# Gadersd/whisper-burn

Hardware: AMD Instinct MI355X
Metric: real-time factor (audio-sec/wall-sec) (higher is better)
Workload: dtype f32; 1 GPU; tiny.en, 30 s of 16 kHz audio per GPU per step, reference windowing (3 windows <= 14.9 s, 3 s overlap), HIP mel + encoder + KV-cached decode, greedy (beam_size 1), max_depth 100; windows=3, beam_size=1, max_depth=100, encoder_gemm_after_the_run=f16x3, parallelism=windows sharded over 1 GPU(s), 1 token all-gather

## Files before the change

profiles/ps_timeline.py:

```python
#!/usr/bin/env python3
import sys

import numpy as np

raw = np.fromfile(sys.argv[1], dtype=np.uint8)
n_steps, n_roles, grid, ns = [int(x) for x in raw[:16].view(np.int32)]
kinds = raw[16:16 + 4 * n_roles].view(np.int32)
n_st = 8 * n_steps * n_roles * ns
st = raw[16 + 4 * n_roles:16 + 4 * n_roles + n_st].view(np.uint64).reshape(n_steps, n_roles, ns).astype(np.float64)
tail = raw[16 + 4 * n_roles + n_st:]
block = None
if len(tail) >= 4 * (grid + 2) and int(tail[:4].view(np.int32)[0]) == 0x66664f52:
    role_off = tail[4:4 * (grid + 2)].view(np.int32)
    block = np.searchsorted(role_off, np.arange(n_roles), side="right") - 1
st[st == 0] = np.nan
names = {0: "attn", 1: "cross", 2: "mlp", 3: "logits", 4: "merge", 5: "finln"}
kind, layer, row = kinds & 0xff, (kinds >> 8) & 0xff, kinds >> 16
ran = ~np.isnan(st[:, :, 6])
last = int(np.nonzero(ran.any(1))[0].max()) + 1 if ran.any() else 0
lo = int(sys.argv[2]) if len(sys.argv) > 2 else min(8, max(last - 1, 0))
hi = int(sys.argv[3]) if len(sys.argv) > 3 else last
live_row = int(sys.argv[4]) if len(sys.argv) > 4 else 0
tick = 0.01
print(f"steps stamped {last} of {n_steps}, roles/step {n_roles}, grid {grid}; statistics over steps [{lo}, {hi}), attention roles of row {live_row}")
sel = st[lo:hi]
merge_done = sel[:, kind == 4, 7]
step_end = np.nanmax(merge_done, axis=1)
step_start = np.concatenate([[np.nan], step_end[:-1]])
hdr = f"{'role':<10}{'n':>4}{'wait':>8}{'w->p2':>8}{'p2->p3':>8}{'p3->p4':>8}{'p4->p5':>8}{'p5->done':>9}{'arrive':>8}{'run':>8}{'done@':>9}{'arrived@':>9}"
print(hdr)
spread = []
for k in (0, 1, 2, 5, 3, 4):
    for l in sorted(set(layer[kind == k])):
        cols = (kind == k) & (layer == l)
        if k in (0, 1, 5):
            cols &= row == live_row
        if not cols.any():
            continue
        s = sel[:, cols, :]
        def d(a, b):
            x = (s[:, :, b] - s[:, :, a]) * tick
            return np.nanmean(x) if np.isfinite(x).any() else float("nan")
        rel_done = np.nanmean((np.nanmax(s[:, :, 6], axis=1) - step_start) * tick)
        rel_arr = np.nanmean((np.nanmax(s[:, :, 7], axis=1) - step_start) * tick)
        nm = names[k] + (f" L{l}" if k < 3 else "")
        if k in (0, 1, 3, 4, 5):
            wp = np.nanmean((s[:, :, 1] - step_start[:, None]) * tick, axis=0)
            dn = np.nanmean((s[:, :, 6] - step_start[:, None]) * tick, axis=0)
            spread.append((nm, wp, dn, block[cols] if block is not None else None))
        print(f"{nm:<10}{int(cols.sum()):>4}{d(0,1):>8.2f}{d(1,2):>8.2f}{d(2,3):>8.2f}{d(3,4):>8.2f}{d(4,5):>8.2f}{d(5,6):>9.2f}{d(6,7):>8.2f}{d(1,6):>8.2f}{rel_done:>9.2f}{rel_arr:>9.2f}")
dd = np.diff(step_end) * tick
print(f"step time (merge arrived -> next merge arrived): mean {np.nanmean(dd):.2f} us, median {np.nanmedian(dd):.2f}, min {np.nanmin(dd):.2f}, max {np.nanmax(dd):.2f}")
a0 = (kind == 0) & (layer == 0) & (row == live_row)
if a0.any() and (kind == 3).any() and hi - lo > 1:
    lg_done = np.nanmax(st[lo:hi - 1][:, kind == 3, 6], axis=1)
    for nm, red in (("first", np.nanmin), ("last", np.nanmax)):
        edge = (red(st[lo + 1:hi][:, a0, 2], axis=1) - lg_done) * tick
        print(f"last logits done -> attn L0 p2 ({nm} block of row {live_row}): mean {np.nanmean(edge):.2f} us, median {np.nanmedian(edge):.2f}, min {np.nanmin(edge):.2f}, max {np.nanmax(edge):.2f}")
print("over the roles of a kind (each role: mean over the steps), us after the step start (merge: of its own step's start):")
print(f"{'role':<10}{'n':>4}  {'wait passed @  min / median / max':<36}{'done @  min / median / max':<34}")
for nm, wp, dn, blk in spread:
    f3 = lambda v: f"{np.nanmin(v):8.2f} /{np.nanmedian(v):8.2f} /{np.nanmax(v):8.2f}"
    print(f"{nm:<10}{len(wp):>4}  {f3(wp):<36}{f3(dn):<34}")
    if nm == "logits" and blk is not None:
        late = np.argsort(-np.nan_to_num(dn))[:12]
        def held(b):
            o = [names[kind[i]] + f" L{layer[i]}" for i in np.nonzero(block == b)[0] if kind[i] < 3]
            return "+".join(o) if o else "-"
        print(f"{'':<10}last to finish (block [its layer roles]: wait passed @ / done @)  " +
              "  ".join(f"b{blk[i]}[{held(blk[i])}]:{wp[i]:.2f}/{dn[i]:.2f}" for i in late))
        behind = np.array([held(b) != "-" for b in blk])
        for lab, m in (("behind a layer role", behind), ("on blocks without one", ~behind)):
            if m.any():
                print(f"{'':<10}{lab}: n {int(m.sum())}, done @ min / median / max {np.nanmin(dn[m]):.2f} / {np.nanmedian(dn[m]):.2f} / {np.nanmax(dn[m]):.2f}")
    if nm in ("attn L0", "merge", "finln"):
        per = "  ".join((f"b{blk[i]}:" if blk is not None else f"#{i}:") + f"{wp[i]:.2f}/{dn[i]:.2f}" for i in range(len(wp)))
        print(f"{'':<10}per role (block: wait passed @ / done @)  {per}")
```

whisper-burn_amd/csrc/decode.h:

```cpp
#pragma once
#include <hip/hip_runtime.h>
#include <hip/hip_ext.h>
#include <stdint.h>

#include <algorithm>
#include <vector>

#include "kernels.h"
#include "wb_internal.h"

namespace wb {

constexpr int MAX_BEAMS = 8;
constexpr int TOPK_MAX = 8;
constexpr int CA_STRIDE = 66;
constexpr int CA_NCH_MAX = 12;
constexpr int TS_STRIDE = 2 + 2 * TOPK_MAX;
constexpr int GV_CT = 128;
constexpr int GV_CT_LOGITS = 128;
constexpr int KS_MAX = 16;

enum { ST_N = 0, ST_STEP = 1, ST_HDR = 4 };
enum { GC_STEP = 0, GC_NDONE = 1, GC_ALLDONE = 2, GC_BAD = 3, GC_HDR = 4 };
struct StepLayout {
  int S = 0, W = 0;
  int tok = 0, parent = 0, len = 0, win = 0;
  int dead = 0;
  int win_nb = 0, win_slots = 0;
  int total = 0;
};
inline StepLayout make_step_layout(int S, int W) {
  StepLayout l;
  l.S = S; l.W = W;
  l.tok = ST_HDR; l.parent = l.tok + S; l.len = l.parent + S; l.win = l.len + S; l.dead = l.win + S;
  l.win_nb = l.dead + S; l.win_slots = l.win_nb + W; l.total = l.win_slots + W * MAX_BEAMS;
  return l;
}

enum { PRO_PLAIN = 0, PRO_GELU = 1, PRO_ATTN = 2, PRO_LN = 3 };
struct GemvArgs {
  const float* W = nullptr; int ldw = 0;
  int K = 0, N = 0, KS = 1, KSL = 0;
  int pro = PRO_PLAIN;
  const float* src = nullptr; int ld_src = 0;
  const float* pend = nullptr; const float* pbias = nullptr; int KSp = 0;
  float* x_out = nullptr;
  const float* ln_g = nullptr; const float* ln_b = nullptr; float ln_eps = 0.f; int ln_inside = 0;
  int n_head = 0, n_chunks = 0;
  float* P = nullptr;
  float* h_tmp = nullptr;
  const float* mask = nullptr; int use_mask = 0, topk = 0; float* tstats = nullptr;
  const int* st = nullptr; int S = 0;
  int ct = 0;
};

void gemv_plan(int K, int N, int* KS, int* KSL);
int cross_attn_chunk();

void launch_dec_prepare(hipStream_t st, const int* state_host_mapped, int* state_dev, const StepLayout& lay, int n,
                        int* tabs, int Lmax, const float* E, const float* pos, int d, float* x, const int* gctl);
void launch_dec_resolve_ln(hipStream_t st, const int* state, int n_max, const float* x_in, float* x_out,
                           const float* P, int KS, int S, const float* bias, int d, const LayerNormW& ln,
                           int eps_inside_sqrt, float* h);
void launch_dec_gemv(hipStream_t st, const GemvArgs& a, int n_rows_hint, bool stats);
bool dec_logits_two_launches(const GemvArgs& a, int n_rows_hint);
void launch_dec_self_attn(hipStream_t st, const int* state, const StepLayout& lay, int n_max, int n_head,
                          const float* Pqkv, int KS, const float* bqkv, int d, float* Kc, float* Vc, const int* tab,
                          int Lmax, float scale, float* att);
struct CaFuse {
  const float* x_in = nullptr;
  const float* pend = nullptr; int KSp = 0; const float* pbias = nullptr;
  float* x_out = nullptr;
  const float* ln_g = nullptr; const float* ln_b = nullptr; float ln_eps = 0.f; int ln_inside = 0;
  const float* Wq = nullptr;
  const float* Wo = nullptr;
  float* rec = nullptr;
};
bool cross_attn_can_fuse_q(int d);
void launch_dec_cross_attn(hipStream_t st, const int* state, const StepLayout& lay, int n_windows, int n_head,
                           int n_chunks, const float* Pq, int KS, const float* bq, int d, const float* ckv, int ldkv,
                           int koff, const int* win_row0, const int* win_C, float scale, float* ca, int max_nb,
                           const CaFuse* fuse = nullptr);
constexpr int CSF_MAX_D = 1280;
struct CaStreamFuse {
  const float* x_in = nullptr; float* x_out = nullptr;
  const float* pend = nullptr; int KSp = 0; const float* pbias = nullptr;
  const float* ln_g = nullptr; const float* ln_b = nullptr; float ln_eps = 0.f; int ln_inside = 0;
  const float* Wq = nullptr;
};
bool cross_stream_can_fuse(int d);
void launch_dec_cross_attn_stream_fused(hipStream_t st, const int* state, const StepLayout& lay, int n_windows, int n_head,
                                        const float* bq, int d, const float* ckv, int ldkv, int koff, const int* win_row0,
                                        const int* win_C, float scale, float* att, const CaStreamFuse& fz);
void launch_dec_cross_attn_stream(hipStream_t st, const int* state, const StepLayout& lay, int n_windows, int n_head,
                                  const float* Pq, int KS, const float* bq, int d, const float* ckv, int ldkv, int koff,
                                  const int* win_row0, const int* win_C, float scale, float* att);
struct NextPrep {
  float* x = nullptr;
  const float* E = nullptr;
  const float* pos = nullptr;
  int* tabs = nullptr;
  int d = 0;
  int* hflags = nullptr;
};
void launch_dec_topk_merge(hipStream_t st, int* state, int n_max, const float* tstats, int n_tiles, int k,
                           int32_t* out_id, float* out_lp, float* row_stats, const StepLayout& lay, int* gctl, int* gtok,
                           int Lmax, int eot, const NextPrep& nx);
void launch_dec_gelu_fold(hipStream_t st, const int* state, int n_max, const float* P, int KS, int S, int K,
                          const float* bias, float* out);
void launch_dec_attn_combine(hipStream_t st, const int* state, int n_max, const float* ca, int n_head, int n_chunks,
                             float* out);
void launch_dec_topk_rows(hipStream_t st, int* state, int n_max, const float* logits, int V, const float* mask,
                          int use_mask, int k, int32_t* out_id, float* out_lp, float* row_stats, const StepLayout& lay,
                          int* gctl, int* gtok, int Lmax, int eot);
void launch_dec_logprob_row(hipStream_t st, const float* x, int KS, int64_t plane, int V, const float* mask,
                            int use_mask, const float* stats, float* out);

constexpr int BEAM_KB = 2 * TOPK_MAX;
enum { BC_DEPTH = 0, BC_ALLDONE = 1, BC_ERR = 2, BC_NLIVE = 3, BC_HDR = 8 };
struct BeamChainLayout {
  int W = 0, max_depth = 0;
  int nb = 0, done = 0, node = 0, fin = 0, prev_slot = 0, slot_now = 0, lp = 0, nodes = 0, total_ints = 0;
};
inline BeamChainLayout make_beam_layout(int W, int max_depth) {
  BeamChainLayout b;
  b.W = W; b.max_depth = max_depth;
  b.nb = BC_HDR; b.done = b.nb + W; b.node = b.done + W; b.fin = b.node + W * BEAM_KB; b.prev_slot = b.fin + W * BEAM_KB;
  b.slot_now = b.prev_slot + W * BEAM_KB;
  b.lp = (b.slot_now + W * BEAM_KB + 1) & ~1;
  b.nodes = b.lp + 2 * W * BEAM_KB;
  b.total_ints = b.nodes + 2 * (max_depth + 1) * W * BEAM_KB;
  return b;
}
struct BeamChainArgs {
  int* ctl = nullptr; BeamChainLayout bl;
  const int32_t* topk_id = nullptr; const float* topk_lp = nullptr;
  int* state_out = nullptr; StepLayout lay;
  int k = 0, eot = 0, first = 0;
  int V = 0;
  int step_pos = 0;
  int* done_flag_host = nullptr;
  int* tabs = nullptr; int Lmax = 0; const float* E = nullptr; const float* pos = nullptr; int d = 0; float* x = nullptr;
};
void launch_dec_beam_update(hipStream_t st, const BeamChainArgs& a);

enum { SC_NDONE = 0, SC_ALLDONE = 1, SC_ERR = 2, SC_NROWS = 3, SC_BEST_OF = 4, SC_ATTEMPT = 5, SC_SEED_LO = 6, SC_SEED_HI = 7,
       SC_INVT = 8, SC_HDR = 16 };
struct SampleChainLayout {
  int S = 0, W = 0, max_depth = 0;
  int stream = 0, fin = 0, ngen = 0, win_fin = 0, sum = 0, tokens = 0, total_ints = 0;
};
inline SampleChainLayout make_sample_layout(int S, int W, int max_depth) {
  SampleChainLayout b;
  b.S = S; b.W = W; b.max_depth = max_depth;
  b.stream = SC_HDR; b.fin = b.stream + S; b.ngen = b.fin + S; b.win_fin = b.ngen + S;
  b.sum = (b.win_fin + W + 1) & ~1;
  b.tokens = b.sum + 2 * S;
  b.total_ints = b.tokens + S * max_depth;
  return b;
}
struct SampleChainArgs {
  int* ctl = nullptr; SampleChainLayout sl;
  const float* logits = nullptr; int V = 0;
  const float* mask = nullptr; int use_mask = 0;
  const float* row_stats = nullptr;
  int* state = nullptr; StepLayout lay;
  int eot = 0;
  int* tabs = nullptr; int Lmax = 0; const float* E = nullptr; const float* pos = nullptr; int d = 0; float* x = nullptr;
};
void launch_dec_sample_update(hipStream_t st, const SampleChainArgs& a, int n_rows);
struct SampleRowsArgs {
  const float* logits = nullptr; int R = 0, ld = 0, V = 0;
  const float* mask = nullptr; const uint8_t* row_masked = nullptr;
  const float* row_stats = nullptr;
  float inv_t = 1.f; uint32_t seed_lo = 0, seed_hi = 0, attempt = 0;
  const int32_t* stream = nullptr; const int32_t* position = nullptr;
  int eot = 0;
  int32_t* out_token = nullptr; float* out_logprob = nullptr; int32_t* out_err = nullptr;
};
void launch_sample_rows(hipStream_t st, const SampleRowsArgs& a);

enum { TC_NDONE = 0, TC_ALLDONE = 1, TC_ERR = 2, TC_NROWS = 3, TC_BEST_OF = 4, TC_ATTEMPT = 5, TC_SEED_LO = 6, TC_SEED_HI = 7,
       TC_INVT = 8,
       TC_TB = 9, TC_NTS = 10, TC_MAX_INIT = 11, TC_MAX_TS = 12, TC_HDR = 16 };
struct TsChainLayout {
  int S = 0, W = 0, max_depth = 0;
  int stream = 0, fin = 0, ngen = 0, last_was = 0, penult_was = 0, last_ts = 0, win_fin = 0, sum = 0, tokens = 0, total_ints = 0;
};
inline TsChainLayout make_ts_layout(int S, int W, int max_depth) {
  TsChainLayout b;
  b.S = S; b.W = W; b.max_depth = max_depth;
  b.stream = TC_HDR; b.fin = b.stream + S; b.ngen = b.fin + S; b.last_was = b.ngen + S; b.penult_was = b.last_was + S;
  b.last_ts = b.penult_was + S; b.win_fin = b.last_ts + S;
  b.sum = (b.win_fin + W + 1) & ~1;
  b.tokens = b.sum + 2 * S;
  b.total_ints = b.tokens + S * max_depth;
  return b;
}
struct TsRowState {
  int n_gen = 0;
  int last_was = 0, penult_was = 0;
  int last_ts = -1;
};
struct TsRules { int tb = 0, n_ts = 0, max_init = -1, max_ts = -1, eot = 0; };
struct TsChainArgs {
  int* ctl = nullptr; TsChainLayout tl;
  const float* logits = nullptr; int V = 0;
  const uint32_t* sup = nullptr; const uint32_t* sup_first = nullptr;
  const float* row_stats = nullptr;
  int* state = nullptr; StepLayout lay;
  int eot = 0;
  int* tabs = nullptr; int Lmax = 0; const float* E = nullptr; const float* pos = nullptr; int d = 0; float* x = nullptr;
};
void launch_dec_ts_update(hipStream_t st, const TsChainArgs& a, int n_rows);
struct TsRowsArgs {
  const float* logits = nullptr; int R = 0, ld = 0, V = 0;
  const uint32_t* sup = nullptr; const uint32_t* sup_first = nullptr;
  const float* row_max = nullptr;
  TsRules rules;
  float inv_t = 0.f; uint32_t seed_lo = 0, seed_hi = 0, attempt = 0;
  const int32_t* n_gen = nullptr; const int32_t* prev1 = nullptr; const int32_t* prev2 = nullptr; const int32_t* last_ts = nullptr;
  const int32_t* stream = nullptr; const int32_t* position = nullptr;
  int32_t* out_token = nullptr; float* out_logprob = nullptr; int32_t* out_forced = nullptr; float* out_stats = nullptr;
  int32_t* out_err = nullptr;
};
void launch_ts_rows(hipStream_t st, const TsRowsArgs& a);

enum { TB_DEPTH = 0, TB_ALLDONE = 1, TB_ERR = 2, TB_NENDED = 3, TB_NWIN = 4, TB_B = 5, TB_C = 6, TB_TB = 7, TB_NTS = 8,
       TB_MAX_INIT = 9, TB_MAX_TS = 10, TB_NLIVE = 11, TB_HDR = 16 };
struct TsBeamLayout {
  int S = 0, W = 0, max_depth = 0;
  int nb = 0, ended = 0, nfin = 0, slot = 0, node = 0, last_was = 0, penult_was = 0, last_ts = 0, fin_node = 0, row_beam = 0,
      tr_n = 0, tr_fin = 0, score = 0, fin_score = 0, tr_score = 0, nodes = 0, total_ints = 0;
};
inline TsBeamLayout make_tsbeam_layout(int S, int W, int max_depth) {
  TsBeamLayout b;
  b.S = S; b.W = W; b.max_depth = max_depth;
  const int WB = W * MAX_BEAMS, DW = max_depth * W;
  b.nb = TB_HDR; b.ended = b.nb + W; b.nfin = b.ended + W; b.slot = b.nfin + W; b.node = b.slot + WB; b.last_was = b.node + WB;
  b.penult_was = b.last_was + WB; b.last_ts = b.penult_was + WB; b.fin_node = b.last_ts + WB; b.row_beam = b.fin_node + W * BEAM_KB;
  b.tr_n = b.row_beam + S; b.tr_fin = b.tr_n + DW;
  b.score = (b.tr_fin + DW + 1) & ~1;
  b.fin_score = b.score + 2 * WB; b.tr_score = b.fin_score + 2 * W * BEAM_KB;
  b.nodes = b.tr_score + 2 * DW * MAX_BEAMS;
  b.total_ints = b.nodes + 2 * DW * MAX_BEAMS;
  return b;
}
enum { TBR_COUNT = 0, TBR_FORCED = 1, TBR_TS_LSE = 2, TBR_MN = 3, TBR_STRIDE = 4 };
struct TsBeamRowsArgs {
  int* ctl = nullptr; TsBeamLayout bl;
  const float* logits = nullptr; int V = 0;
  const uint32_t* sup = nullptr; const uint32_t* sup_first = nullptr;
  const int* state = nullptr; StepLayout lay;
  int eot = 0;
  int32_t* topk_id = nullptr; float* topk_lp = nullptr; int* row_out = nullptr;
};
struct TsBeamUpdateArgs {
  int* ctl = nullptr; TsBeamLayout bl;
  const int32_t* topk_id = nullptr; const float* topk_lp = nullptr; const int* row_out = nullptr;
  int* state = nullptr; StepLayout lay;
  int eot = 0, V = 0;
  int step_pos = 0;
  int* tabs = nullptr; int Lmax = 0; const float* E = nullptr; const float* pos = nullptr; int d = 0; float* x = nullptr;
};
void launch_dec_tsbeam_rows(hipStream_t st, const TsBeamRowsArgs& a, int n_rows);
void launch_dec_tsbeam_update(hipStream_t st, const TsBeamUpdateArgs& a);
struct TsBeamRowsHookArgs {
  const float* logits = nullptr; int R = 0, ld = 0, V = 0, k = 0;
  const uint32_t* sup = nullptr; const uint32_t* sup_first = nullptr;
  TsRules rules;
  const int32_t* n_gen = nullptr; const int32_t* prev1 = nullptr; const int32_t* prev2 = nullptr; const int32_t* last_ts = nullptr;
  int32_t* out_id = nullptr; float* out_lp = nullptr;
  int32_t* out_count = nullptr; int32_t* out_forced = nullptr; float* out_stats = nullptr; int32_t* out_err = nullptr;
};
void launch_tsbeam_rows_hook(hipStream_t st, const TsBeamRowsHookArgs& a);

struct MlpFusedArgs {
  const int* st = nullptr; int S = 0, d = 0;
  const float* x_in = nullptr; const float* pend = nullptr; int KSp = 0; const float* pbias = nullptr; float* x_out = nullptr;
  int n_head = 0, n_chunks = 0;
  const float* ln_g = nullptr; const float* ln_b = nullptr; float ln_eps = 0.f; int ln_inside = 0;
  const float* W1 = nullptr; int ld1 = 0; const float* b1 = nullptr;
  const float* W2 = nullptr;
  float* P = nullptr;
  unsigned long long* stamps = nullptr;
  int row0 = 0;
  const void* g_x_in = nullptr; const void* g_pend = nullptr; void* g_x_out = nullptr; void* g_P = nullptr;
};
struct AttnFusedArgs {
  const int* st = nullptr; StepLayout lay; int S = 0, d = 0, n_head = 0;
  const float* x_in = nullptr; const float* pend = nullptr; int KSp = 0; const float* pbias = nullptr; float* x_out = nullptr;
  const float* ln_g = nullptr; const float* ln_b = nullptr; float ln_eps = 0.f; int ln_inside = 0;
  const float* Wqkv = nullptr; int ldqkv = 0; const float* bqkv = nullptr; float scale = 0.f;
  float* Kc = nullptr; float* Vc = nullptr; const int* tabs = nullptr; int Lmax = 0;
  const float* Wo = nullptr;
  float* P = nullptr;
  unsigned long long* stamps = nullptr;
  const void* g_x_in = nullptr; const void* g_pend = nullptr; void* g_x_out = nullptr; void* g_P = nullptr;
};
struct CrossFusedArgs {
  const int* st = nullptr; StepLayout lay; int S = 0, d = 0, n_head = 0;
  const float* x_in = nullptr; const float* pend = nullptr; int KSp = 0; const float* pbias = nullptr; float* x_out = nullptr;
  const float* ln_g = nullptr; const float* ln_b = nullptr; float ln_eps = 0.f; int ln_inside = 0;
  const float* Wq = nullptr; const float* bq = nullptr; float scale = 0.f;
  const float* ckv = nullptr; int ldkv = 0, koff = 0;
  const int* win_row0 = nullptr; const int* win_C = nullptr;
  int n_pass = 1;
  const float* Wo = nullptr;
  float* P = nullptr;
  unsigned long long* stamps = nullptr;
  const void* g_x_in = nullptr; const void* g_pend = nullptr; void* g_x_out = nullptr; void* g_P = nullptr;
};
struct SkinnyArgs {
  const float* A = nullptr; int lda = 0;
  const float* B = nullptr; int ldb = 0;
  int M = 0, N = 0, K = 0, ksplit = 1;
  float* P = nullptr; int plane = 0;
  const uint16_t* Bh = nullptr; const uint16_t* Bl = nullptr;
  int* range_flag = nullptr;
  const int* st = nullptr;
};
void launch_split_weight_f16_tiles(hipStream_t st, const float* W, int K, int N, uint16_t* hi, uint16_t* lo);
int skinny_ksplit(int K, int N, int max_ks, int max_rows);
bool skinny_supported(int M, int K, int N);
int launch_dec_skinny_gemm(hipStream_t st, const SkinnyArgs& a);

struct PsLayerArgs { AttnFusedArgs attn; CrossFusedArgs cross; MlpFusedArgs mlp; };
enum { PSR_ATTN = 0, PSR_CROSS = 1, PSR_MLP = 2, PSR_LOGITS = 3, PSR_MERGE = 4, PSR_FINLN = 5 };
struct PsRole { int kind, layer, a, b; };
constexpr int PS_MAX_FORCED = 8;
struct PersistArgs {
  const PsLayerArgs* layers = nullptr;
  const PsRole* roles = nullptr; int n_roles = 0;
  const int* role_off = nullptr;
  const int* res_role = nullptr;
  int n_logits_roles = 0;
  int n_layer = 0, n_rows = 0, S = 0, d = 0, n_head = 0, nb_mlp = 0;
  int n_pass = 1;
  int* ctl = nullptr;
  int step0 = 0, n_steps = 0;
  int n_forced = 0; int forced[PS_MAX_FORCED] = {0, 0, 0, 0, 0, 0, 0, 0};
  int mask_until_len = 0;
  const void* x_fin = nullptr; const void* P2 = nullptr; const float* b2_last = nullptr;
  void* g_xn = nullptr;
  unsigned tag_base = 0;
  const float* ln_g = nullptr; const float* ln_b = nullptr; float ln_eps = 0.f; int ln_inside = 0;
  const float* Et = nullptr; int vocab_ld = 0, V = 0; const float* mask = nullptr;
  void* tstats = nullptr; int n_tiles = 0;
  int pick = 1;
  int* gctl = nullptr; int* gtok = nullptr; int Lmax = 0, eot = 0;
  const float* E = nullptr; const float* pos = nullptr; void* x0 = nullptr; int* tabs = nullptr;
  int* dead = nullptr;
  unsigned long long* stamps = nullptr;
};
enum { PS_DEAL_SLACK = 0, PS_DEAL_LEGACY = 1 };
struct PsDeal {
  std::vector<PsRole> roles;
  std::vector<int> role_off;
  std::vector<int> res_role;
  int n_lg = 0, n_res = 0;
};
PsDeal ps_deal_roles(int n_layer, int n_head, int n_rows, int nb_mlp, int n_tiles, int grid, int policy, bool res_on);
int ps_ctl_ints(int S, int n_layer);
bool dec_persist_supported(int d, int n_rows, int max_keys);
int dec_persist_resident_slots(int d, int n_rows, int max_keys);
bool dec_persist_resident_geometry(int d, int n_rows, int max_keys, int out[5]);
int dec_persist_max_grid(int device, int d, int n_rows, int max_keys);
int launch_dec_persist(hipStream_t st, const PersistArgs& a, int grid);
void launch_ps_seed(hipStream_t st, const float* x, int n, void* gx, unsigned tag, int* ctl);
void launch_ps_pick_test(hipStream_t st, const void* rec, int n_tiles, unsigned tag, int* ctl, int* out_id);

#if defined(HIPEMU) && !defined(HIPEMU_PROD_GEOMETRY)
constexpr int CROSS_FUSED_MAX_C = 384;
#else
constexpr int CROSS_FUSED_MAX_C = 768;
#endif
constexpr int CROSS_FUSED_MAX_PASSES = 2;
void launch_dec_cross_fused(hipStream_t st, const CrossFusedArgs& a, int n_rows_hint);
bool dec_fused_supported(int d);
int dec_mlp_fused_planes(int d);
void launch_dec_mlp_fused(hipStream_t st, const MlpFusedArgs& a, int n_rows_hint);
void launch_dec_attn_fused(hipStream_t st, const AttnFusedArgs& a, int n_rows_hint);
int launch_dec_attn_fused_rounds(hipStream_t st, const AttnFusedArgs& a, int n_rows_hint, int n_reg);

}
```

whisper-burn_amd/csrc/decode_chain.cpp:

```cpp
#include <climits>
#include <cstring>
#include <string>

#include "decode_step.h"
#include "handoff.h"
#include "switches.h"

using namespace wb;

namespace wb {

struct PsPin { size_t seed, err, gctl, tok, total, ctl_ints; };
static PsPin ps_pin_layout(size_t ctl_ints, size_t tok_ints) {
  PsPin p;
  p.seed = 0; p.err = (ctl_ints + 3) & ~(size_t)3; p.gctl = p.err + 4; p.tok = p.gctl + ((ctl_ints + 3) & ~(size_t)3);
  p.total = p.tok + tok_ints; p.ctl_ints = ctl_ints;
  return p;
}
static int ps_pin_ensure(wb_session* s, size_t ints) {
  if (s->ps_pin_ints >= ints) return WB_OK;
  if (s->ps_pin_busy) { WB_HIP(hipStreamSynchronize(s->st)); s->ps_pin_busy = false; }
  if (s->ps_pin) { (void)hipHostFree(s->ps_pin); s->ps_pin = nullptr; s->ps_pin_ints = 0; }
  WB_HIP(hipHostMalloc((void**)&s->ps_pin, ints * 4, hipHostMallocDefault));
  s->ps_pin_ints = ints;
  return WB_OK;
}

PsDeal ps_deal_roles(int NL, int H, int W, int NB, int n_tiles, int grid, int policy, bool res_on) {
  std::vector<PsRole> lr;
  for (int l = 0; l < NL; l++) {
    for (int r = 0; r < W; r++) for (int h = 0; h < H; h++) lr.push_back(PsRole{PSR_ATTN, l, h, r});
    for (int r = 0; r < W; r++) for (int h = 0; h < H; h++) lr.push_back(PsRole{PSR_CROSS, l, h, r});
    for (int j = 0; j < NB; j++) lr.push_back(PsRole{PSR_MLP, l, j, 0});
  }
  std::vector<std::vector<PsRole>> deal(grid);
  for (size_t i = 0; i < lr.size(); i++) deal[i % grid].push_back(lr[i]);
  std::vector<char> early(grid, 0);
  std::vector<int> cand;
  for (int b = 0; b < grid; b++) {
    for (const PsRole& r : deal[b]) early[b] |= r.layer == 0 && (r.kind == PSR_ATTN || r.kind == PSR_CROSS);
    if (!early[b]) cand.push_back(b);
  }
  if ((int)cand.size() * 4 < n_tiles) { cand.clear(); for (int b = 0; b < grid; b++) cand.push_back(b); }
  const bool slack = policy != PS_DEAL_LEGACY;
  auto by_load = [&](std::vector<int>& v) {
    std::stable_sort(v.begin(), v.end(), [&](int x, int y) {
      if (slack && early[x] != early[y]) return early[x] < early[y];
      return deal[x].size() < deal[y].size();
    });
  };
  std::vector<int> fin_block(W, 0);
  std::vector<char> is_fin(grid, 0);
  {
    std::vector<int> order(grid);
    for (int b = 0; b < grid; b++) order[b] = b;
    by_load(order);
    for (int r = 0; r < W; r++) { fin_block[r] = order[r % grid]; deal[fin_block[r]].push_back(PsRole{PSR_FINLN, 0, 0, r}); is_fin[fin_block[r]] = 1; }
  }
  if ((int)cand.size() > 2 * W) cand.erase(std::remove_if(cand.begin(), cand.end(), [&](int b) { return is_fin[b] != 0; }), cand.end());
  std::stable_sort(cand.begin(), cand.end(), [&](int x, int y) { return deal[x].size() < deal[y].size(); });
  const int tpb = (n_tiles + (int)cand.size() - 1) / (int)cand.size();
  const int n_lg = (n_tiles + tpb - 1) / tpb;
  std::vector<char> has_lg(grid, 0);
  for (int q = 0; q < n_lg; q++) {
    deal[cand[q]].push_back(PsRole{PSR_LOGITS, q, q * tpb, std::min(tpb, n_tiles - q * tpb)});
    has_lg[cand[q]] = 1;
  }
  {
    std::vector<int> order;
    if (slack) {
      for (int b = 0; b < grid; b++) if (!early[b] && !has_lg[b]) order.push_back(b);
      if (order.empty()) for (int b = 0; b < grid; b++) if (!early[b]) order.push_back(b);
    }
    if (order.empty()) for (int b = 0; b < grid; b++) order.push_back(b);
    by_load(order);
    for (int r = 0; r < W; r++) {
      const int b = slack && !early[fin_block[r]] ? fin_block[r] : order[r % (int)order.size()];
      deal[b].push_back(PsRole{PSR_MERGE, 0, 0, r});
    }
  }
  PsDeal out;
  out.n_lg = n_lg;
  out.role_off.assign(grid + 1, 0);
  for (int b = 0; b < grid; b++) {
    out.role_off[b] = (int)out.roles.size();
    out.roles.insert(out.roles.end(), deal[b].begin(), deal[b].end());
  }
  out.role_off[grid] = (int)out.roles.size();
  out.res_role.assign(grid, -1);
  if (res_on)
    for (int b = 0; b < grid; b++) {
      int n_lr = 0, at = -1;
      for (int i = out.role_off[b]; i < out.role_off[b + 1]; i++)
        if (out.roles[i].kind <= PSR_MLP) { n_lr++; at = i; }
      if (n_lr == 1 && out.roles[at].kind != PSR_MLP) { out.res_role[b] = at; out.n_res++; }
    }
  return out;
}

static void ps_deal_log(const PsDeal& deal, int grid) {
  std::string where[2];
  int n_lg_blocks = 0;
  for (int b = 0; b < grid; b++) {
    bool lg = false;
    for (int i = deal.role_off[b]; i < deal.role_off[b + 1]; i++) {
      const int k = deal.roles[i].kind;
      lg |= k == PSR_LOGITS;
      if (k == PSR_MERGE || k == PSR_FINLN) {
        std::string& w = where[k == PSR_FINLN];
        w += (w.empty() ? "" : ",") + std::to_string(b);
      }
    }
    n_lg_blocks += lg;
  }
  fprintf(stderr, "persist deal: merge on blocks %s; finln on %s; logits blocks %d\n", where[0].c_str(), where[1].c_str(), n_lg_blocks);
}

static int ps_setup_ensure(wb_session* s, bool res_on, bool* built) {
  wb_model* m = s->m;
  const wb_dims& D = m->dims;
  const int d = D.n_text_state, H = D.n_text_head, NL = D.n_text_layer, V = D.n_vocab, S = s->S, W = s->W;
  const StepLayout& L = s->lay;
  hipStream_t st = s->st;
  const int NB = dec_mlp_fused_planes(d);
  const int n_tiles = (V + 127) / 128;
  const size_t pool = (size_t)s->Lmax * S;
  const int ldkv = 2 * d;
  const int n_pass = s->maxC > CROSS_FUSED_MAX_C ? 2 : 1;
  const int n_layer_roles = NL * (2 * W * H + NB);
  const int grid = std::max(1, std::min(s->ps_grid, n_layer_roles + n_tiles + 2 * W));
  const char* deal_sw = sw::persist_deal();
  const int policy = deal_sw && !strcmp(deal_sw, "legacy") ? PS_DEAL_LEGACY : PS_DEAL_SLACK;
  auto up = [](const void* p) { return (uint64_t)reinterpret_cast<uintptr_t>(p); };
  const std::vector<uint64_t> key = {
      s->model_uid, (uint64_t)W, (uint64_t)S, (uint64_t)s->Lmax, (uint64_t)grid, (uint64_t)n_tiles, (uint64_t)n_pass,
      (uint64_t)s->enc_rows, (uint64_t)res_on, (uint64_t)m->ln_eps_inside_sqrt, up(s->state.p), up(s->x.p), up(s->P2.p),
      up(s->Pa.p), up(s->Pc.p), up(s->kc.p), up(s->vc.p), up(s->tabs.p), up(s->ckv.p), up(s->win_meta.p), up(s->ps_gx.p),
      up(s->ps_gpa.p), up(s->ps_gpc.p), up(s->ps_gp2.p), up(s->ps_gxn.p), (uint64_t)policy};
  const char* sw_setup = sw::persist_setup();
  const bool cache_on = !(sw_setup && sw_setup[0] == '0');
  *built = !(cache_on && !s->ps_setup_key.empty() && s->ps_setup_key == key);
  if (sw_setup && strstr(sw_setup, "log")) fprintf(stderr, "persist setup: %s\n", *built ? "built" : "reused");
  if (!*built) return WB_OK;
  s->ps_setup_key.clear();
  char* gxb[2] = {static_cast<char*>(s->ps_gx.p), static_cast<char*>(s->ps_gx.p) + (size_t)S * d * 8};
  std::vector<PsLayerArgs> la(NL);
  float* xb[2] = {s->x.as<float>(), s->x.as<float>() + (size_t)S * d};
  int xi = 0;
  for (int l = 0; l < NL; l++) {
    const DecBlockW& b = m->dec[l];
    AttnFusedArgs& fa = la[l].attn;
    fa.st = s->state.as<int>(); fa.lay = L; fa.S = S; fa.d = d; fa.n_head = H;
    fa.x_in = xb[xi]; fa.pend = l == 0 ? nullptr : s->P2.as<float>(); fa.KSp = l == 0 ? 0 : NB;
    fa.pbias = l == 0 ? nullptr : m->dec[l - 1].mlp2.b; fa.x_out = xb[xi ^ 1];
    fa.ln_g = b.ln1.g; fa.ln_b = b.ln1.b; fa.ln_eps = b.ln1.eps; fa.ln_inside = m->ln_eps_inside_sqrt;
    fa.Wqkv = b.qkv.w; fa.ldqkv = b.qkv.n; fa.bqkv = b.qkv.b; fa.scale = m->qk_scale;
    fa.Kc = s->kc.as<float>() + (size_t)l * pool * d; fa.Vc = s->vc.as<float>() + (size_t)l * pool * d;
    fa.tabs = s->tabs.as<int>(); fa.Lmax = s->Lmax; fa.Wo = b.out.w; fa.P = s->Pa.as<float>();
    fa.g_x_in = gxb[xi]; fa.g_pend = l == 0 ? nullptr : s->ps_gp2.p; fa.g_x_out = gxb[xi ^ 1]; fa.g_P = s->ps_gpa.p;
    xi ^= 1;
    CrossFusedArgs& ca = la[l].cross;
    ca.st = s->state.as<int>(); ca.lay = L; ca.S = S; ca.d = d; ca.n_head = H;
    ca.x_in = xb[xi]; ca.pend = s->Pa.as<float>(); ca.KSp = H; ca.pbias = b.out.b; ca.x_out = xb[xi ^ 1];
    ca.ln_g = b.ln2.g; ca.ln_b = b.ln2.b; ca.ln_eps = b.ln2.eps; ca.ln_inside = m->ln_eps_inside_sqrt;
    ca.Wq = b.cq.w; ca.bq = b.cq.b; ca.scale = m->qk_scale;
    ca.ckv = s->ckv.as<float>() + (size_t)l * s->enc_rows * 2 * d; ca.ldkv = ldkv; ca.koff = 0;
    ca.win_row0 = s->win_meta.as<int>(); ca.win_C = s->win_meta.as<int>() + W;
    ca.Wo = b.cout.w; ca.P = s->Pc.as<float>();
    ca.n_pass = n_pass;
    ca.g_x_in = gxb[xi]; ca.g_pend = s->ps_gpa.p; ca.g_x_out = gxb[xi ^ 1]; ca.g_P = s->ps_gpc.p;
    xi ^= 1;
    MlpFusedArgs& ma = la[l].mlp;
    ma.st = s->state.as<int>(); ma.S = S; ma.d = d;
    ma.x_in = xb[xi]; ma.pend = s->Pc.as<float>(); ma.KSp = H; ma.pbias = b.cout.b; ma.x_out = xb[xi ^ 1];
    ma.ln_g = b.ln3.g; ma.ln_b = b.ln3.b; ma.ln_eps = b.ln3.eps; ma.ln_inside = m->ln_eps_inside_sqrt;
    ma.W1 = b.mlp1.w; ma.ld1 = b.mlp1.n; ma.b1 = b.mlp1.b; ma.W2 = b.mlp2.w; ma.P = s->P2.as<float>();
    ma.g_x_in = gxb[xi]; ma.g_pend = s->ps_gpc.p; ma.g_x_out = gxb[xi ^ 1]; ma.g_P = s->ps_gp2.p;
    xi ^= 1;
  }
  PsDeal deal = ps_deal_roles(NL, H, W, NB, n_tiles, grid, policy, res_on);
  if (deal_sw && !strcmp(deal_sw, "log")) ps_deal_log(deal, grid);
  std::vector<PsRole>& roles = deal.roles;
  const std::vector<int>&role_off = deal.role_off, &res_role = deal.res_role;
  const int n_lg = deal.n_lg, n_res = deal.n_res;
  WB_TRY(s->ps_layers.ensure(la.size() * sizeof(PsLayerArgs)));
  WB_TRY(s->ps_roles.ensure(roles.size() * sizeof(PsRole) + (role_off.size() + res_role.size()) * 4));
  WB_HIP(hipMemcpyAsync(s->ps_layers.p, la.data(), la.size() * sizeof(PsLayerArgs), hipMemcpyHostToDevice, st));
  WB_HIP(hipMemcpyAsync(s->ps_roles.p, roles.data(), roles.size() * sizeof(PsRole), hipMemcpyHostToDevice, st));
  WB_HIP(hipMemcpyAsync(static_cast<char*>(s->ps_roles.p) + roles.size() * sizeof(PsRole), role_off.data(), role_off.size() * 4,
                        hipMemcpyHostToDevice, st));
  WB_HIP(hipMemcpyAsync(static_cast<char*>(s->ps_roles.p) + roles.size() * sizeof(PsRole) + role_off.size() * 4, res_role.data(),
                        res_role.size() * 4, hipMemcpyHostToDevice, st));
  WB_HIP(hipStreamSynchronize(st));
  s->ps_pin_busy = false;
  s->ps_roles_host.swap(roles);
  s->ps_role_off_host = role_off;
  s->ps_setup_grid = grid; s->ps_setup_n_lg = n_lg; s->ps_setup_n_res = n_res;
  s->ps_setup_key = key;
  return WB_OK;
}

static int run_persistent_chain(wb_session* s, int eot, int max_depth, int mask_until_len, const int32_t* forced, int n_forced,
                                const PsPin& pin, int* steps_done, bool* fell_back) {
  *fell_back = false;
  WB_REQUIRE(n_forced >= 0 && n_forced <= PS_MAX_FORCED, WB_ERR_ARG, "persistent decode: %d prompt steps", n_forced);
  const char* inject = sw::persist_inject_fail();
  wb_model* m = s->m;
  const wb_dims& D = m->dims;
  const int d = D.n_text_state, H = D.n_text_head, NL = D.n_text_layer, V = D.n_vocab, S = s->S, W = s->W;
  const StepLayout& L = s->lay;
  hipStream_t st = s->st;
  const int NB = dec_mlp_fused_planes(d);
  const int n_tiles = (V + 127) / 128;
  WB_REQUIRE(NB <= 32 && H <= 8, WB_ERR_SHAPE, "persistent decode: more planes than its folds hold");
  WB_TRY(s->ps_gx.ensure_zeroed(((size_t)2 * S + 8) * d * 8, st));
  WB_TRY(s->ps_gpa.ensure_zeroed(((size_t)H * S + 8) * d * 8, st));
  WB_TRY(s->ps_gpc.ensure_zeroed(((size_t)H * S + 8) * d * 8, st));
  WB_TRY(s->ps_gp2.ensure_zeroed(((size_t)NB * S + 8) * d * 8, st));
  WB_TRY(s->ps_gxn.ensure_zeroed(((size_t)S + 8) * d * 8, st));
  WB_TRY(s->ps_tstats.ensure_zeroed((size_t)2 * S * n_tiles * 16, st));
  if (((s->ps_launches + 1) & 0xffffu) == 0) {
    for (DevMem* b : {&s->ps_gx, &s->ps_gpa, &s->ps_gpc, &s->ps_gp2, &s->ps_gxn, &s->ps_tstats}) WB_HIP(hipMemsetAsync(b->p, 0, b->bytes, st));
    s->ps_launches++;
  }
  const unsigned tag_base = ((++s->ps_launches) & 0xffffu) << 16;
  char* gxb[2] = {static_cast<char*>(s->ps_gx.p), static_cast<char*>(s->ps_gx.p) + (size_t)S * d * 8};
  const char* res_sw = sw::persist_resident();
  const bool res_on = !(res_sw && res_sw[0] == '0') && dec_persist_resident_slots(d, W, s->maxC) > 0;
  bool built = false;
  WB_TRY(ps_setup_ensure(s, res_on, &built));
  const std::vector<PsRole>& roles = s->ps_roles_host;
  const int grid = s->ps_setup_grid, n_res = s->ps_setup_n_res;
  if (res_sw && !strcmp(res_sw, "log")) fprintf(stderr, "persist resident blocks: %d of %d\n", n_res, grid);
  const int n_ctl = ps_ctl_ints(S, NL);
  WB_TRY(s->ps_ctl.ensure((size_t)n_ctl * 4));
  WB_TRY(s->ps_dead.ensure((size_t)S * 4));
  WB_HIP(hipMemsetAsync(s->ps_ctl.p, 0, (size_t)n_ctl * 4, st));
  WB_HIP(hipMemsetAsync(s->ps_dead.p, 0, (size_t)S * 4, st));
  PersistArgs a;
  a.layers = s->ps_layers.as<PsLayerArgs>(); a.roles = s->ps_roles.as<PsRole>(); a.n_roles = (int)roles.size();
  a.role_off = reinterpret_cast<const int*>(static_cast<char*>(s->ps_roles.p) + roles.size() * sizeof(PsRole));
  if (n_res > 0) a.res_role = a.role_off + (grid + 1);
  a.n_logits_roles = s->ps_setup_n_lg;
  a.n_layer = NL; a.n_rows = W; a.S = S; a.d = d; a.n_head = H; a.nb_mlp = NB;
  a.n_pass = s->maxC > CROSS_FUSED_MAX_C ? 2 : 1;
  a.ctl = s->ps_ctl.as<int>(); a.step0 = s->step; a.n_steps = n_forced + max_depth; a.mask_until_len = mask_until_len;
  a.n_forced = n_forced;
  for (int i = 0; i < n_forced; i++) a.forced[i] = forced[i];
  a.g_xn = s->ps_gxn.p;
  a.x_fin = gxb[(3 * NL) & 1]; a.P2 = s->ps_gp2.p; a.b2_last = m->dec[NL - 1].mlp2.b; a.tag_base = tag_base;
  a.ln_g = m->ln_dec.g; a.ln_b = m->ln_dec.b; a.ln_eps = m->ln_dec.eps; a.ln_inside = m->ln_eps_inside_sqrt;
  a.Et = m->tok_emb_t; a.vocab_ld = m->vocab_ld; a.V = V; a.mask = s->mask.as<float>();
  a.tstats = s->ps_tstats.p; a.n_tiles = n_tiles;
  const char* pick_sw = sw::persist_pick();
  a.pick = pick_sw && !strcmp(pick_sw, "merge") ? 0 : 1;
  a.gctl = s->gctl.as<int>(); a.gtok = s->gtok.as<int>(); a.Lmax = s->Lmax; a.eot = eot;
  a.E = m->tok_emb; a.pos = m->dec_pos; a.x0 = gxb[0]; a.tabs = s->tabs.as<int>(); a.dead = s->ps_dead.as<int>();
  const char* stamps_path = sw::ps_stamps();
  const size_t n_stamps = stamps_path ? (size_t)(n_forced + max_depth) * roles.size() * 8 : 0;
  if (n_stamps) {
    WB_TRY(s->ps_stamps.ensure(n_stamps * 8));
    WB_HIP(hipMemsetAsync(s->ps_stamps.p, 0, n_stamps * 8, st));
    a.stamps = s->ps_stamps.as<unsigned long long>();
  }
  WB_REQUIRE(3 * NL * (n_forced + max_depth + 1) + 4 < 0x10000, WB_ERR_SHAPE,
             "persistent decode: %d layers x %d steps do not fit the 16-bit granule tags", NL, max_depth);
  launch_dec_prepare(st, reinterpret_cast<const int*>(s->host_block_dev), s->state.as<int>(), L, W, s->tabs.as<int>(),
                     s->Lmax, m->tok_emb, m->dec_pos, d, s->x.as<float>(), s->gctl.as<int>());
  launch_ps_seed(st, s->x.as<float>(), W * d, gxb[0], tag_base + 1u, s->ps_ctl.as<int>());
  hipEvent_t e0 = nullptr, e1 = nullptr;
  prof_tag(KC_PERSIST, 0.0);
  const bool timed = prof_take_events(&e0, &e1);
  if (timed) WB_HIP(hipEventRecord(e0, st));
  const bool refused = (inject && !strcmp(inject, "launch")) || launch_dec_persist(st, a, grid) != 0;
  if (timed) WB_HIP(hipEventRecord(e1, st));
  if (refused) {
    (void)hipGetLastError();
    s->ps_grid = 0;
    *fell_back = true;
    *steps_done = 0;
    return WB_OK;
  }
  int* hp = s->ps_pin;
  s->ps_pin_busy = true;
  WB_HIP(hipMemcpyAsync(hp + pin.err, s->ps_ctl.as<int>() + HX_ERR, 4, hipMemcpyDeviceToHost, st));
  WB_HIP(hipMemcpyAsync(hp + pin.gctl, s->gctl.p, pin.ctl_ints * 4, hipMemcpyDeviceToHost, st));
  WB_HIP(hipMemcpyAsync(hp + pin.tok, s->gtok.p, (pin.total - pin.tok) * 4, hipMemcpyDeviceToHost, st));
  WB_HIP(hipStreamSynchronize(st));
  s->ps_pin_busy = false;
  const int err = hp[pin.err], gstep = hp[pin.gctl + GC_STEP];
  if (err != 0 && gstep == s->step) {
    s->ps_grid = 0;
    *fell_back = true;
    *steps_done = 0;
    return WB_OK;
  }
  WB_REQUIRE(err == 0, WB_ERR_HIP, "persistent decode: a wait gave up (counter %d) at step %d", err - 1, gstep);
  if (n_stamps) {
    std::vector<unsigned long long> hs(n_stamps);
    WB_HIP(hipMemcpy(hs.data(), s->ps_stamps.p, n_stamps * 8, hipMemcpyDeviceToHost));
    if (FILE* f = fopen(stamps_path, "wb")) {
      const int hdr[4] = {n_forced + max_depth, (int)roles.size(), grid, 8};
      fwrite(hdr, 4, 4, f);
      std::vector<int> kinds(roles.size());
      for (size_t i = 0; i < roles.size(); i++)
        kinds[i] = roles[i].kind | ((roles[i].kind <= PSR_MLP ? roles[i].layer : 0) << 8) |
                   ((roles[i].kind == PSR_LOGITS ? 0 : roles[i].b) << 16);
      fwrite(kinds.data(), 4, kinds.size(), f);
      fwrite(hs.data(), 8, hs.size(), f);
      const int marker = 0x66664f52;
      fwrite(&marker, 4, 1, f);
      fwrite(s->ps_role_off_host.data(), 4, s->ps_role_off_host.size(), f);
      fclose(f);
    }
  }
  *steps_done = std::max(0, std::min(n_forced + max_depth, gstep - s->step));
  return WB_OK;
}

int session_greedy_chain(wb_session* s, const int32_t* prompt, int eot, int max_depth, int mask_until_len, int prompt_len,
                         int32_t* out_tokens, int32_t row_stride, int32_t* out_lens) {
  wb_model* m = s->m;
  const int S = s->S, W = s->W;
  WB_REQUIRE(S == W, WB_ERR_STATE, "chained greedy decode needs max_beams == 1");
  WB_REQUIRE(prompt && prompt_len >= 1, WB_ERR_ARG, "chained greedy decode: empty prompt");
  WB_REQUIRE(s->step == 0 || (s->prev_n == W && s->step == prompt_len - 1), WB_ERR_STATE,
             "chained greedy decode: the session is neither fresh nor prefilled");
  const int n_forced_max = prompt_len - 1;
  auto host_prefill = [&]() -> int {
    std::vector<int32_t> tok(W), par(W), win(W);
    for (int t = s->step; t < prompt_len - 1; t++) {
      for (int w = 0; w < W; w++) { tok[w] = prompt[t]; par[w] = t == 0 ? -1 : w; win[w] = w; }
      WB_TRY(wb_session_step(s, tok.data(), par.data(), win.data(), W, 0, 0, nullptr, nullptr));
    }
    return WB_OK;
  };
  WB_REQUIRE(s->has_mask || mask_until_len < prompt_len || max_depth == 0, WB_ERR_STATE,
             "wb_session_decode: special mask not set");
  const int asked_depth = max_depth;
  max_depth = std::min(max_depth, s->Lmax - (prompt_len - 1));
  WB_HIP(hipSetDevice(m->device));
  hipStream_t st = s->st;
  const size_t ctl_ints = GC_HDR + 3 * (size_t)S;
  WB_TRY(s->gctl.ensure(ctl_ints * 4));
  WB_TRY(s->gtok.ensure(((size_t)S * s->Lmax + 1) * 4));
  std::vector<int> ctl(ctl_ints, 0);
  const PsPin pin = ps_pin_layout(ctl_ints, (size_t)S * s->Lmax + 1);
  WB_TRY(ps_pin_ensure(s, pin.total));
  auto seed_ctl = [&](bool wait) -> int {
    if (s->ps_pin_busy) { WB_HIP(hipStreamSynchronize(st)); s->ps_pin_busy = false; }
    int* seed = s->ps_pin + pin.seed;
    std::fill(seed, seed + ctl_ints, 0);
    seed[GC_STEP] = s->step;
    for (int i = 0; i < W; i++) seed[GC_HDR + i] = prompt[s->step];
    s->ps_pin_busy = true;
    WB_HIP(hipMemcpyAsync(s->gctl.p, seed, ctl_ints * 4, hipMemcpyHostToDevice, st));
    if (wait) { WB_HIP(hipStreamSynchronize(st)); s->ps_pin_busy = false; }
    return WB_OK;
  };
  const StepPlan plan = plan_step(s, W, false);
  const int n_launch = plan.n_launch;
  const bool fuse_ln = plan.fuse_ln;
  const int chunk = 16;
  int depth = 0;
  bool persist = plan.persist && max_depth > 0;
  if (persist) {
    if (s->ps_grid < 0) s->ps_grid = dec_persist_max_grid(m->device, m->dims.n_text_state, W, s->maxC);
    persist = s->ps_grid > 0;
  }
  int n_forced = 0;
  if (s->step == 0 && s->prefill_mode == 1 && sw::prefill_pass() && prompt_len > 1) {
    std::vector<int> win(W);
    for (int w = 0; w < W; w++) win[w] = w;
    WB_TRY(session_prefill(s, prompt, prompt_len - 1, win.data(), W));
  }
  if (persist && sw::persist_prefill() && s->step == 0 && n_forced_max <= PS_MAX_FORCED && s->has_mask) n_forced = n_forced_max;
  if (n_forced == 0) WB_TRY(host_prefill());
  WB_TRY(seed_ctl(!persist));
  ScopedTimer tm(st, 3);
  if (persist) {
    bool fell_back = false;
    WB_TRY(run_persistent_chain(s, eot, max_depth, mask_until_len, prompt + s->step + 1, n_forced, pin, &depth, &fell_back));
    if (fell_back) {
      persist = false;
      depth = 0;
      WB_TRY(host_prefill());
      WB_TRY(seed_ctl(true));
      n_forced = 0;
    } else {
      if (profile().on) profile().ms[4] += depth;
      depth -= n_forced;
      s->step += n_forced;
      s->prev_n = W;
      s->prev_win.resize(W);
      for (int w = 0; w < W; w++) s->prev_win[w] = w;
    }
  }
  if (!persist) {
  if (fuse_ln)
    launch_dec_prepare(st, reinterpret_cast<const int*>(s->host_block_dev), s->state.as<int>(), s->lay, n_launch,
                       s->tabs.as<int>(), s->Lmax, m->tok_emb, m->dec_pos, m->dims.n_text_state, s->x.as<float>(),
                       s->gctl.as<int>());
  const bool speculate = fuse_ln && sw::speculate();
  if (speculate && !s->st2) {
    WB_HIP(hipStreamCreateWithFlags(&s->st2, hipStreamNonBlocking));
    WB_HIP(hipEventCreateWithFlags(&s->ev_seg, hipEventDisableTiming));
  }
  auto enqueue_segment = [&](int* enq) -> int {
    int n = 0;
    while (depth + n < max_depth && n < chunk) {
      const int d0 = depth + n;
      const int use_mask = (prompt_len + d0) <= mask_until_len ? 1 : 0;
      const int run = (!use_mask && max_depth - d0 >= chunk) ? chunk : 1;
      StepCall call;
      call.k = 1; call.use_mask = use_mask; call.chained = true; call.eot = eot; call.reps = run;
      WB_TRY(launch_step(s, plan, call));
      if (profile().on) profile().ms[4] += run;
      n += run;
    }
    *enq = n;
    return WB_OK;
  };
  auto read_flags = [&](bool behind_event) -> int {
    if (behind_event) {
      WB_HIP(hipStreamWaitEvent(s->st2, s->ev_seg, 0));
      WB_HIP(hipMemcpyAsync(ctl.data(), s->gctl.p, ctl_ints * 4, hipMemcpyDeviceToHost, s->st2));
      WB_HIP(hipStreamSynchronize(s->st2));
    } else {
      WB_HIP(hipMemcpyAsync(ctl.data(), s->gctl.p, ctl_ints * 4, hipMemcpyDeviceToHost, st));
      WB_HIP(hipStreamSynchronize(st));
    }
    return WB_OK;
  };
  auto all_done = [&]() {
    bool d = true;
    for (int i = 0; i < W; i++) d = d && ctl[GC_HDR + S + i] != 0;
    return d;
  };
  const bool poll = fuse_ln && sw::poll() && !profile().on;
  volatile int* hfl = reinterpret_cast<volatile int*>(s->host_block + s->chain_flags_off);
  if (poll) for (int i = 0; i < 2 * S; i++) hfl[i] = 0;
  auto wait_flags = [&](int want_step, bool* done) -> int {
    for (long spins = 0;; spins++) {
      bool ready = true;
      for (int i = 0; i < W && ready; i++) ready = hfl[2 * i] >= want_step;
      if (ready) break;
      bool fin = true;
      for (int i = 0; i < W && fin; i++) fin = hfl[2 * i + 1] != 0;
      if (fin) break;
      if ((spins & 0xfff) == 0xfff) {
        const hipError_t q = hipStreamQuery(st);
        if (q == hipSuccess) {
          bool r2 = true;
          for (int i = 0; i < W && r2; i++) r2 = hfl[2 * i] >= want_step;
          if (r2) break;
          bool all = true;
          for (int i = 0; i < W; i++) all = all && hfl[2 * i + 1] != 0;
          if (all) break;
          set_error("chained decode: the device stopped at step %d of %d", (int)hfl[0], want_step);
          return WB_ERR_HIP;
        }
        if (q != hipErrorNotReady) { set_error("chained decode: %s", hipGetErrorString(q)); return WB_ERR_HIP; }
      }
    }
    __atomic_thread_fence(__ATOMIC_ACQUIRE);
    bool all = true;
    for (int i = 0; i < W; i++) all = all && hfl[2 * i + 1] != 0;
    *done = all;
    return WB_OK;
  };
  if (!speculate) {
    while (depth < max_depth) {
      int n = 0;
      WB_TRY(enqueue_segment(&n));
      depth += n;
      if (poll) {
        bool done = false;
        WB_TRY(wait_flags(s->step + depth, &done));
        if (done) break;
      } else {
        WB_TRY(read_flags(false));
        if (all_done()) break;
      }
    }
  } else {
    int n_cur = 0;
    WB_TRY(enqueue_segment(&n_cur));
    depth += n_cur;
    while (true) {
      WB_HIP(hipEventRecord(s->ev_seg, st));
      int n_next = 0;
      if (depth < max_depth) { WB_TRY(enqueue_segment(&n_next)); depth += n_next; }
      WB_TRY(read_flags(true));
      if (all_done() || n_next == 0) break;
    }
    WB_HIP(hipStreamSynchronize(st));
  }
  }
  tm.stop();
  std::vector<int> toks_chain;
  const int* toks = s->ps_pin + pin.tok;
  if (persist) {
    std::copy(s->ps_pin + pin.gctl, s->ps_pin + pin.gctl + ctl_ints, ctl.begin());
  } else {
    toks_chain.resize((size_t)S * s->Lmax + 1);
    WB_HIP(hipMemcpyAsync(ctl.data(), s->gctl.p, ctl_ints * 4, hipMemcpyDeviceToHost, st));
    WB_HIP(hipMemcpyAsync(toks_chain.data(), s->gtok.p, toks_chain.size() * 4, hipMemcpyDeviceToHost, st));
    WB_HIP(hipStreamSynchronize(st));
    s->ps_pin_busy = false;
    toks = toks_chain.data();
  }
  tm.collect();
  WB_TRY(dec_split_check(s));
  WB_REQUIRE(ctl[GC_BAD] == 0, WB_ERR_STATE, "a decode step produced a row without a finite log-prob (NaN logits: non-finite "
             "weights or activations); its window was ended on <|endoftext|> on the device and the rows of this call are invalid");
  for (int w = 0; w < W; w++) {
    int len = ctl[GC_HDR + 2 * S + w];
    if (len < prompt_len) len = prompt_len;
    len = std::min(len, prompt_len + max_depth);
    WB_REQUIRE(len <= row_stride, WB_ERR_ARG, "row_stride too small");
    for (int p = prompt_len; p < len; p++) out_tokens[(size_t)w * row_stride + p] = toks[(size_t)w * s->Lmax + p];
    out_lens[w] = len;
  }
  if (profile().on && !persist && s->prof_cls_cross >= 0 && s->prof_cls_self >= 0) {
    const int dm = m->dims.n_text_state, NL = m->dims.n_text_layer;
    double dead_ckv = 0, dead_self = 0;
    for (int w = 0; w < W; w++) {
      const int live = std::max(0, std::min(out_lens[w] - prompt_len, depth));
      for (int t = live; t < depth; t++) { dead_ckv += 8.0 * s->C[w] * dm; dead_self += 8.0 * (s->step + t + 1) * dm; }
    }
    prof_adjust_bytes(s->prof_cls_cross, -(double)NL * dead_ckv);
    prof_adjust_bytes(s->prof_cls_self, -(double)NL * dead_self);
  }
  if (profile().on && persist) {
    const double dm = m->dims.n_text_state, NL = m->dims.n_text_layer;
    double bytes = (double)(depth + n_forced) * 4.0 * NL * 14.0 * dm * dm + (double)depth * 4.0 * (double)m->dims.n_vocab * dm;
    for (int w = 0; w < W; w++)
      for (int t = 0; t < n_forced; t++) bytes += NL * (8.0 * s->C[w] * dm + 8.0 * (t + 1) * dm);
    for (int w = 0; w < W; w++) {
      const int live = std::max(0, std::min(out_lens[w] - prompt_len, depth));
      for (int t = 0; t < live; t++) bytes += NL * (8.0 * s->C[w] * dm + 8.0 * (s->step + t + 1) * dm);
    }
    prof_adjust_bytes(KC_PERSIST, bytes);
  }
  s->prof_step_off = 0;
  s->step += depth;
  s->prev_len.assign(W, s->step);
  s->last_had_logits = 0;
  if (max_depth < asked_depth)
    for (int w = 0; w < W; w++)
      WB_REQUIRE(ctl[GC_HDR + S + w] != 0, WB_ERR_SHAPE, "Token sequence length %d must not exceed %d.", s->Lmax + 1,
                 s->Lmax);
  return WB_OK;
}
}
```

whisper-burn_amd/csrc/decode_fused_bodies.h:

```cpp
#pragma once
#include <hip/hip_runtime.h>

#include "decode.h"
#include "handoff.h"
#include "wave_ops.h"

namespace wb {
namespace fused {

struct PsStep {
  const unsigned* ctr = nullptr; unsigned target = 0; int ctr_index = 0;
  const int* ctl = nullptr;
  int step = 0;
  int n_rows = 0;
  const int* dead = nullptr;
  int* lds_flag = nullptr;
  unsigned long long* stamp = nullptr;
  int n_ctr = 1;
  unsigned tag_in = 0, tag_out = 0;
  bool known_dead = false;
  mutable bool saw_dead = false;
  const void* pk_rec = nullptr; int pk_n_tiles = 0; unsigned pk_tag = 0;
  const unsigned* pk_go = nullptr; unsigned pk_go_target = 0;
  const float* pk_E = nullptr; const float* pk_pos = nullptr; int pk_eot = 0;
  bool cross_early = false;
};
constexpr int PS_STAMPS = 8;
__device__ __forceinline__ void ps_stamp(const PsStep& ps, int k) {
#ifdef WB_EXP_FINE
  if (k == 4 || k == 5) return;
#endif
  if (ps.stamp && threadIdx.x == 0) ps.stamp[k] = wall_clock64();
}
__device__ __forceinline__ void ps_stamp_fine(const PsStep& ps, int k) {
#ifdef WB_EXP_FINE
  if (ps.stamp && threadIdx.x == 0) ps.stamp[k] = wall_clock64();
#endif
}
__device__ __forceinline__ bool ps_wait(const PsStep& ps) {
  const bool ok = ps.n_ctr > 1 ? hx_wait_same(ps.ctr, ps.target, ps.n_ctr, ps.ctl, ps.step, ps.ctr_index, ps.lds_flag)
                               : hx_wait(ps.ctr, ps.target, ps.ctl, ps.step, ps.ctr_index, ps.lds_flag);
  ps_stamp(ps, 1);
  return ok;
}
__device__ __forceinline__ bool ps_sweep_retry(unsigned& sweeps, const PsStep& ps) {
  if ((sweeps & 31u) == 31u &&
      (__hip_atomic_load(ps.ctl + HX_STOP, __ATOMIC_RELAXED, __HIP_MEMORY_SCOPE_AGENT) <= ps.step ||
       __hip_atomic_load(ps.ctl + HX_ERR, __ATOMIC_RELAXED, __HIP_MEMORY_SCOPE_AGENT) != 0)) return true;
  if (++sweeps > HX_SWEEP_LIMIT) {
    __hip_atomic_store(const_cast<int*>(ps.ctl) + HX_ERR, 5000 + ps.ctr_index, __ATOMIC_RELAXED, __HIP_MEMORY_SCOPE_AGENT);
    return true;
  }
  __builtin_amdgcn_s_sleep(1);
  return false;
}
__device__ __forceinline__ bool ps_sweeps_ok(const PsStep& ps) { return *ps.lds_flag != 0; }
template <int UNITS>
__device__ __forceinline__ void ps_nap() {
#if !defined(WB_PS_DRY) || defined(WB_PS_DRY_NAPS)
#ifndef WB_PS_NAP_ADJ
#define WB_PS_NAP_ADJ 0
#endif
#pragma unroll
  for (int i = 0; i < UNITS + (WB_PS_NAP_ADJ); i++) __builtin_amdgcn_s_sleep(64);
#endif
}

constexpr int PS_PICK_NONE = 0x7fffffff;
#ifdef WB_PS_PICK_NOINLINE
__device__ __attribute__((noinline)) int ps_pick_token(
#else
__device__ __forceinline__ int ps_pick_token(
#endif
const void* rec, const int n_tiles, const unsigned tag, const PsStep& ps,
                                             float* xch, const int tid) {
  const Buf16 rb(rec);
  float bv = -INFINITY; int bi = PS_PICK_NONE;
  unsigned sweeps = 0;
  for (int t = tid; t < n_tiles;) {
    const Rec q = ld_rec(rb, (uint32_t)t);
    if (q.t0 == tag && q.t1 == tag) {
      if (better(q.v, q.id, bv, bi)) { bv = q.v; bi = q.id; }
      t += 512;
    } else if (ps_sweep_retry(sweeps, ps)) {
      *ps.lds_flag = 0;
      break;
    }
  }
  wave_argmax(bv, bi);
  int* xid = reinterpret_cast<int*>(xch) + 8;
  if ((tid & 63) == 0) { xch[tid >> 6] = bv; xid[tid >> 6] = bi; }
  __syncthreads();
  float gv = xch[0]; int gi = xid[0];
#pragma unroll
  for (int j = 1; j < 8; j++)
    if (better(xch[j], xid[j], gv, gi)) { gv = xch[j]; gi = xid[j]; }
  return gi;
}
#ifndef WB_PS_PICK_NAP
#define WB_PS_PICK_NAP 6
#endif
#ifndef WB_PS_CROSS0_NAP
#define WB_PS_CROSS0_NAP 1
#endif

#ifdef WB_STAMPS
#define WB_STAMP_DECL unsigned long long stamp_buf[16];
#define WB_STAMP(i) do { if (threadIdx.x == 0 && blockIdx.x == 0 && blockIdx.y == 0) sm.stamp_buf[i] = wall_clock64(); } while (0)
#define WB_STAMP_FLUSH(a, n) do { if (threadIdx.x == 0 && blockIdx.x == 0 && blockIdx.y == 0 && (a).stamps) for (int _i = 0; _i < (n); _i++) (a).stamps[_i] = sm.stamp_buf[_i]; } while (0)
#else
#define WB_STAMP_DECL
#define WB_STAMP(i) do {} while (0)
#define WB_STAMP_FLUSH(a, n) do {} while (0)
#endif

constexpr int FD_MAX = 512;
constexpr int FA_MAXPOS = 448;


constexpr int ROLE_NT = 512;
template <int MR, int DPL, bool REC>
struct MlpLds {
  static constexpr int d = 64 * DPL, HS = 64, G = d / 4 <= 32 ? 8 : 4;
  alignas(16) float hs[MR][d];
  alignas(16) float red[8][MR][HS];
  alignas(16) float hid[MR][HS];
  alignas(16) float obuf[(G - 1) * MR * d];
  float mlb[REC ? MR : 1][48][2];
  float coef[REC ? MR : 1][48];
  WB_STAMP_DECL
};
template <int DPL>
struct AttnLds {
  static constexpr int d = 64 * DPL, G = d / 4 <= 32 ? 8 : 4;
  static constexpr int RED = (8 * 192 > (G - 1) * d) ? 8 * 192 : (G - 1) * d;
  alignas(16) float hs[d];
  alignas(16) float red[RED];
  alignas(16) float qkv[192];
  int tbs[FA_MAXPOS];
  float sc[FA_MAXPOS];
  alignas(16) float part[32][64];
  alignas(16) float att[64];
  WB_STAMP_DECL
};
template <int DPL, int NP>
struct CrossLds {
  static constexpr int d = 64 * DPL, G = d / 4 <= 32 ? 8 : 4, CMAX = NP * CROSS_FUSED_MAX_C;
  alignas(16) float hs[d];
  alignas(16) float red[8][64];
  alignas(16) float qv[64];
  float sc[CMAX];
  float pbuf[CMAX];
  alignas(16) float part[32][64];
  alignas(16) float att[64];
  alignas(16) float wmax[8];
  alignas(16) float obuf[(G - 1) * d];
};

template <int DPL, int NP, int RS>
struct ResGeom {
  static constexpr int d = 64 * DPL, G = d / 4 <= 32 ? 8 : 4, RPG = 64 / G;
  static constexpr int KW = d / 8, RK = DPL >= 6 ? 8 : 16, NIT = KW / RK;
  static constexpr int CAP = RS * ROLE_NT;
  static constexpr int QL = 8 * 48;
  static constexpr int WL = G * (d / 4) < ROLE_NT ? G * (d / 4) : ROLE_NT;
  static constexpr int NRND_MAX = DPL == 6 ? 2 : 1;
  static constexpr int NRND_FIT = CAP / (RK * QL) < NIT - 2 ? CAP / (RK * QL) : NIT - 2;
  static constexpr int NRND = NRND_FIT <= 0 ? 0 : (NRND_FIT < NRND_MAX ? NRND_FIT : NRND_MAX);
  static constexpr int WO_A = NRND * RK * QL;
  static constexpr int NWO_A = (CAP - WO_A) / WL < RPG ? (CAP - WO_A) / WL : RPG;
  static constexpr int SL = 4, NTILE = CROSS_FUSED_MAX_C / 128;
  static constexpr int NVT = NP > 1 ? 0 : (RS / SL < NTILE ? RS / SL : NTILE);
  static constexpr int WO_X = NVT * SL * ROLE_NT;
  static constexpr int NWO_X = NP > 1 ? 0 : ((CAP - WO_X) / WL < RPG ? (CAP - WO_X) / WL : RPG);
  static_assert(RS >= 0 && WO_A + NWO_A * WL <= CAP && WO_X + NWO_X * WL <= CAP, "resident region");
  static __device__ __forceinline__ int q_holder(int wave, int lane) { return wave * 48 + (lane < 47 ? lane : 47); }
  static __device__ __forceinline__ int wo_holder(int tid) { return tid < WL - 1 ? tid : WL - 1; }
};
__device__ __forceinline__ float4 res_ld(const float4* res, int base, int NH, int slot, int k) { return res[base + slot * NH + k]; }
__device__ __forceinline__ void res_st(float4* res, int base, int NH, int slot, int k, const float4& v) { res[base + slot * NH + k] = v; }

__device__ __forceinline__ float gelu_erf_f(float x) {
  return 0.5f * x * (1.0f + erff(x * 0.70710678118654752440f));
}

template <int DPL>
__device__ __forceinline__ void fold_ln_row(const float* __restrict__ x_in, const float* __restrict__ pend, int KSp,
                                            int64_t plane, const float* __restrict__ pbias, float* __restrict__ x_out,
                                            const float* __restrict__ g, const float* __restrict__ b, float eps,
                                            int eps_inside, int d, int row, int lane, float* __restrict__ out) {
  int co[DPL];
#pragma unroll
  for (int i = 0; i < DPL; i++) co[i] = lane + (64 * i < d ? 64 * i : 0);
  float gv[DPL], bv[DPL], v[DPL];
  const float* xr = x_in + (int64_t)row * d;
#pragma unroll
  for (int i = 0; i < DPL; i++) { gv[i] = g[co[i]]; bv[i] = b[co[i]]; v[i] = xr[co[i]]; }
  if (KSp > 0) {
    float acc[DPL];
#pragma unroll
    for (int i = 0; i < DPL; i++) acc[i] = pbias[co[i]];
    const float* pp = pend + (int64_t)row * d;
    constexpr int CH = DPL <= 6 ? 8 : 4;
    for (int sp = 0; sp < KSp; sp += CH) {
      float t[CH][DPL];
#pragma unroll
      for (int j = 0; j < CH; j++) {
        const float* pj = pp + (int64_t)min(sp + j, KSp - 1) * plane;
#pragma unroll
        for (int i = 0; i < DPL; i++) t[j][i] = pj[co[i]];
      }
#pragma unroll
      for (int j = 0; j < CH; j++) {
        const bool live = sp + j < KSp;
#pragma unroll
        for (int i = 0; i < DPL; i++) acc[i] += live ? t[j][i] : 0.f;
      }
    }
#pragma unroll
    for (int i = 0; i < DPL; i++) v[i] = v[i] + acc[i];
  }
  float s = 0.f;
#pragma unroll
  for (int i = 0; i < DPL; i++) {
    if (64 * i < d) { s += v[i]; if (x_out) x_out[(int64_t)row * d + co[i]] = v[i]; }
  }
  const float mean = wave_sum(s) / (float)d;
  float q = 0.f;
#pragma unroll
  for (int i = 0; i < DPL; i++) {
    if (64 * i < d) { const float t = v[i] - mean; q += t * t; }
  }
  const float var = wave_sum(q) / (float)d;
  const float denom = eps_inside ? sqrtf(var + eps) : (sqrtf(var) + eps);
#pragma unroll
  for (int i = 0; i < DPL; i++) {
    const int c = lane + 64 * i;
    if (c < d) out[c] = (v[i] - mean) / denom * gv[i] + bv[i];
  }
}

template <int NT, int MR, int EPT, int PCH>
__device__ __forceinline__ void fold_rows(const float* __restrict__ x_in, const float* __restrict__ pend, int KSp,
                                          int64_t plane, const float* __restrict__ pbias, int d, int tid,
                                          float (&v)[EPT]) {
  int off[EPT], col[EPT];
#pragma unroll
  for (int i = 0; i < EPT; i++) {
    int e = tid + NT * i;
    if (e >= MR * d) e = tid;
    off[i] = e; col[i] = e % d;
  }
#pragma unroll
  for (int i = 0; i < EPT; i++) v[i] = x_in[off[i]];
  if (KSp > 0) {
    float acc[EPT];
#pragma unroll
    for (int i = 0; i < EPT; i++) acc[i] = pbias[col[i]];
    for (int sp = 0; sp < KSp; sp += PCH) {
      float t[PCH][EPT];
#pragma unroll
      for (int j = 0; j < PCH; j++) {
        const float* pj = pend + (int64_t)min(sp + j, KSp - 1) * plane;
#pragma unroll
        for (int i = 0; i < EPT; i++) t[j][i] = pj[off[i]];
      }
#pragma unroll
      for (int j = 0; j < PCH; j++) {
        const bool live = sp + j < KSp;
#pragma unroll
        for (int i = 0; i < EPT; i++) acc[i] += live ? t[j][i] : 0.f;
      }
    }
#pragma unroll
    for (int i = 0; i < EPT; i++) v[i] = v[i] + acc[i];
  }
}

template <int DPL>
__device__ __forceinline__ void ln_row_lds(float* __restrict__ row, int d, int lane, const float (&gv)[DPL],
                                           const float (&bv)[DPL], float eps, int eps_inside) {
  float v[DPL];
  float s = 0.f;
#pragma unroll
  for (int i = 0; i < DPL; i++) { v[i] = row[lane + 64 * i]; s += v[i]; }
  const float mean = wave_sum(s) / (float)d;
  float q = 0.f;
#pragma unroll
  for (int i = 0; i < DPL; i++) { const float t = v[i] - mean; q += t * t; }
  const float var = wave_sum(q) / (float)d;
  const float denom = eps_inside ? sqrtf(var + eps) : (sqrtf(var) + eps);
#pragma unroll
  for (int i = 0; i < DPL; i++) row[lane + 64 * i] = (v[i] - mean) / denom * gv[i] + bv[i];
}

template <int DPL>
__device__ __forceinline__ void ln_stats_lds(const float* __restrict__ row, int d, int lane, float eps, int eps_inside,
                                             float& mean, float& denom) {
  float v[DPL];
  float s = 0.f;
#pragma unroll
  for (int i = 0; i < DPL; i++) { v[i] = row[lane + 64 * i]; s += v[i]; }
  mean = wave_sum(s) / (float)d;
  float q = 0.f;
#pragma unroll
  for (int i = 0; i < DPL; i++) { const float t = v[i] - mean; q += t * t; }
  const float var = wave_sum(q) / (float)d;
  denom = eps_inside ? sqrtf(var + eps) : (sqrtf(var) + eps);
}
__device__ __forceinline__ float lane_get(float v, int src) { return __shfl(v, src, 64); }

template <int MR, int DPL, bool REC, bool PS>
__device__ __forceinline__ bool dec_mlp_body(const MlpFusedArgs& a, const int jblk, const PsStep& ps, MlpLds<MR, DPL, REC>& sm) {
  constexpr int HS = 64, NT = 512;
  constexpr int d = 64 * DPL;
  constexpr int CF = d / 4;
  constexpr int G = CF <= 32 ? 8 : 4;
  constexpr int RPG = HS / G;
  constexpr int EPT = (MR * d + NT - 1) / NT;
  constexpr int PCH = EPT <= 3 ? 8 : EPT <= 6 ? 6 : 3;
  static_assert(G == MlpLds<MR, DPL, REC>::G, "LDS struct geometry");
  auto& hs = sm.hs; auto& red = sm.red; auto& hid = sm.hid; auto& obuf = sm.obuf; auto& mlb = sm.mlb; auto& coef = sm.coef;
  WB_STAMP(0);
  const int tid = role_tid<PS>(), lane = tid & 63, wave = tid >> 6;
  const int j0 = jblk * HS;
  const int rg = tid >> 4, c4 = (tid & 15) * 4;
  float xv_fold[EPT];
  constexpr int NW1 = d / 32;
  float4 w1[NW1];
  const int cf = tid % CF, jg = tid / CF;
  const bool p2 = jg < G;
  const int jb = (p2 ? jg : 0) * RPG;
  float4 w2[RPG];
  constexpr int NOWN = 4 * NW1;
  const int own_col = 4 * wave + (lane & 3) + 32 * ((lane < NOWN ? lane : 0) >> 2);
  float g_own = 0.f, b_own = 0.f;
  float b1v;
  int deadm = 0;
  {
    int off[EPT], col[EPT];
#pragma unroll
    for (int i = 0; i < EPT; i++) {
      int e = tid + NT * i;
      if (e >= MR * d) e = tid;
      off[i] = e; col[i] = e % d;
    }
    float acc0[EPT];
    constexpr bool rec = REC;
    const int64_t plane = rec ? (int64_t)a.S * (d + 2) : (int64_t)a.S * d;
    int poff[EPT];
#pragma unroll
    for (int i = 0; i < EPT; i++) poff[i] = rec ? (off[i] / d) * (d + 2) + 2 + col[i] : off[i];
    constexpr int PCHR = EPT <= 3 ? 18 : EPT <= 4 ? 16 : EPT <= 6 ? 12 : 8;
    constexpr int PC = REC ? PCHR : PCH;
    float t[PC][EPT];
    const int npl = a.KSp;
    const int ch = rec ? PCHR : PCH;
    auto load_weights = [&]() {
      g_own = gld(a.ln_g + own_col); b_own = gld(a.ln_b + own_col);
      b1v = gld(a.b1 + j0 + (tid & 63));
      {
        const float* wp = a.W1 + (int64_t)rg * a.ld1 + j0 + c4;
#pragma unroll
        for (int i = 0; i < NW1; i++) w1[i] = ld_w4(wp + (int64_t)(32 * i) * a.ld1);
      }
      {
        const float* wp = a.W2 + (int64_t)(j0 + jb) * d + cf * 4;
#pragma unroll
        for (int i = 0; i < RPG; i++) w2[i] = ld_w4(wp + (int64_t)i * d);
      }
    };
    if constexpr (PS) {
#if !defined(WB_PS_DRY)
      load_weights();
#endif
      if (!ps_wait(ps)) return false;
#pragma unroll
      for (int r = 0; r < MR; r++)
        if (r >= ps.n_rows || ld_i<true>(ps.dead + min(r, ps.n_rows - 1)) != 0) deadm |= 1 << r;
      const Buf16 xgb(a.g_x_in), pgb(a.g_pend);
      const int iplane = a.S * d;
      ps_nap<3>();
      bool rdead[EPT];
#pragma unroll
      for (int i = 0; i < EPT; i++) { rdead[i] = ((deadm >> (off[i] / d)) & 1) != 0; acc0[i] = gld(a.pbias + col[i]); xv_fold[i] = 0.f; }
      constexpr int GP = EPT <= 3 ? 8 : 4;
      unsigned sweeps = 0;
      bool bad = false;
      for (int sp = 0; sp < npl && !bad; sp += GP) {
        Gran gx[EPT], g[GP][EPT];
#pragma unroll
        for (int i = 0; i < EPT; i++) {
          gx[i] = Gran{0u, 0.f};
#pragma unroll
          for (int j = 0; j < GP; j++) g[j][i] = Gran{0u, 0.f};
        }
        for (;;) {
          if (sp == 0) {
#pragma unroll
            for (int i = 0; i < EPT; i++)
              if (!rdead[i] && gx[i].tag != ps.tag_in) gx[i] = ld_gran(xgb, (uint32_t)off[i], 0u);
          }
#pragma unroll
          for (int j = 0; j < GP; j++)
#pragma unroll
            for (int i = 0; i < EPT; i++)
              if (!rdead[i] && sp + j < npl && g[j][i].tag != ps.tag_in)
                g[j][i] = ld_gran(pgb, (uint32_t)off[i], (uint32_t)((sp + j) * iplane));
          bool ok = true;
#pragma unroll
          for (int i = 0; i < EPT; i++) {
            if (sp == 0) ok &= rdead[i] || gx[i].tag == ps.tag_in;
#pragma unroll
            for (int j = 0; j < GP; j++) ok &= rdead[i] || sp + j >= npl || g[j][i].tag == ps.tag_in;
          }
          if (ok) {
#pragma unroll
            for (int i = 0; i < EPT; i++) {
              if (sp == 0) xv_fold[i] = gx[i].v;
#pragma unroll
              for (int j = 0; j < GP; j++) acc0[i] += (sp + j < npl) ? g[j][i].v : 0.f;
            }
            break;
          }
          if (ps_sweep_retry(sweeps, ps)) { *ps.lds_flag = 0; bad = true; break; }
        }
      }
#pragma unroll
      for (int i = 0; i < EPT; i++) {
        xv_fold[i] = rdead[i] ? 0.f : xv_fold[i] + acc0[i];
        const int e = tid + NT * i;
        if (e < MR * d) (&hs[0][0])[e] = xv_fold[i];
      }
    } else {
#pragma unroll
    for (int i = 0; i < EPT; i++) { xv_fold[i] = a.x_in[off[i]]; acc0[i] = npl > 0 ? gld(a.pbias + col[i]) : 0.f; }
    float mlv0 = -1.0e30f, mlv1 = 0.f;
    if (rec && tid < MR * npl) {
      const float* rp = a.pend + (int64_t)(tid % npl) * plane + (int64_t)(tid / npl) * (d + 2);
      mlv0 = rp[0]; mlv1 = rp[1];
    }
    if (npl > 0) {
#pragma unroll
      for (int j = 0; j < PC; j++)
        if (j < ch) {
#pragma unroll
          for (int i = 0; i < EPT; i++) t[j][i] = a.pend[(int64_t)min(j, npl - 1) * plane + poff[i]];
        }
    }
    load_weights();
    if constexpr (REC) {
      if (tid < MR * npl) { mlb[tid / npl][tid % npl][0] = mlv0; mlb[tid / npl][tid % npl][1] = mlv1; }
      __syncthreads();
      if (tid < MR * a.n_head) {
        const int r = tid / a.n_head, hh = tid % a.n_head;
        float M = -1.0e30f;
        for (int c = 0; c < a.n_chunks; c++) M = fmaxf(M, mlb[r][hh * a.n_chunks + c][0]);
        float den = 0.f;
        for (int c = 0; c < a.n_chunks; c++) den += expf(mlb[r][hh * a.n_chunks + c][0] - M) * mlb[r][hh * a.n_chunks + c][1];
        for (int c = 0; c < a.n_chunks; c++)
          coef[r][hh * a.n_chunks + c] = den > 0.f ? expf(mlb[r][hh * a.n_chunks + c][0] - M) / den : 0.f;
      }
      __syncthreads();
    }
    if (npl > 0) {
      int rowi[EPT];
#pragma unroll
      for (int i = 0; i < EPT; i++) rowi[i] = off[i] / d;
      for (int sp = 0; sp < npl; sp += ch) {
        if (sp > 0) {
#pragma unroll
          for (int j = 0; j < PC; j++)
            if (j < ch) {
#pragma unroll
              for (int i = 0; i < EPT; i++) t[j][i] = a.pend[(int64_t)min(sp + j, npl - 1) * plane + poff[i]];
            }
        }
#pragma unroll
        for (int j = 0; j < PC; j++)
          if (j < ch) {
#pragma unroll
            for (int i = 0; i < EPT; i++) {
              const bool live = sp + j < npl;
              float wgt = 1.f;
              if constexpr (REC) wgt = coef[rowi[i]][min(sp + j, npl - 1)];
              acc0[i] += live ? wgt * t[j][i] : 0.f;
            }
          }
      }
#pragma unroll
      for (int i = 0; i < EPT; i++) xv_fold[i] += acc0[i];
    }
#pragma unroll
    for (int i = 0; i < EPT; i++) {
      const int e = tid + NT * i;
      if (e < MR * d) (&hs[0][0])[e] = xv_fold[i];
    }
    }
  }
  int n_rows;
  if constexpr (PS) n_rows = ps.n_rows; else n_rows = min(MR, a.st[ST_N] - a.row0);
  if (n_rows <= 0) return true;
  WB_STAMP(1);
  __syncthreads();
  if constexpr (PS) { if (!ps_sweeps_ok(ps)) return false; }
#if defined(WB_PS_DRY)
  if constexpr (PS) {
    if (jg == 0) {
      const Buf16 pgo(a.g_P);
#pragma unroll
      for (int r = 0; r < MR; r++)
        if (r < n_rows && !((deadm >> r) & 1)) st_gran4(pgo, (uint32_t)((jblk * a.S + r) * d + cf * 4), ps.tag_out, make_float4(0.f, 0.f, 0.f, 0.f));
    }
    if (jblk == 0) {
      const Buf16 xgo(a.g_x_out);
#pragma unroll
      for (int i = 0; i < EPT; i++) {
        const int e = tid + NT * i;
        if (e < n_rows * d && !((deadm >> (e / d)) & 1)) st_gran(xgo, (uint32_t)e, ps.tag_out, xv_fold[i]);
      }
    }
    return true;
  }
#endif
  float xn_own[MR];
#pragma unroll
  for (int r = 0; r < MR; r++) {
    xn_own[r] = 0.f;
    bool skip = r >= n_rows;
    if constexpr (PS) skip = skip || ((deadm >> r) & 1);
    if (skip) continue;
    float mean, denom;
    ln_stats_lds<DPL>(hs[r], d, lane, a.ln_eps, a.ln_inside, mean, denom);
    xn_own[r] = (hs[r][own_col] - mean) / denom * g_own + b_own;
  }
  WB_STAMP(2);
  float acc[MR][4];
#pragma unroll
  for (int r = 0; r < MR; r++) { acc[r][0] = acc[r][1] = acc[r][2] = acc[r][3] = 0.f; }
  {
    const int q4 = lane >> 4;
#pragma unroll
    for (int r = 0; r < MR; r++) {
      bool skip = r >= n_rows;
      if constexpr (PS) skip = skip || ((deadm >> r) & 1);
      if (skip) continue;
#pragma unroll
      for (int i = 0; i < NW1; i++) {
        const float xv = lane_get(xn_own[r], 4 * i + q4);
        acc[r][0] += xv * w1[i].x; acc[r][1] += xv * w1[i].y; acc[r][2] += xv * w1[i].z; acc[r][3] += xv * w1[i].w;
      }
    }
  }
#pragma unroll
  for (int r = 0; r < MR; r++)
#pragma unroll
    for (int c = 0; c < 4; c++) { acc[r][c] = xor16_sum(acc[r][c]); acc[r][c] = xor32_sum(acc[r][c]); }
  if (lane < 16) {
#pragma unroll
    for (int r = 0; r < MR; r++)
      *reinterpret_cast<float4*>(&red[wave][r][c4]) = make_float4(acc[r][0], acc[r][1], acc[r][2], acc[r][3]);
  }
  __syncthreads();
  if (tid < MR * HS) {
    const int r = tid >> 6, c = tid & 63;
    float v = 0.f;
#pragma unroll
    for (int w8 = 0; w8 < 8; w8++) v += red[w8][r][c];
    hid[r][c] = gelu_erf_f(v + b1v);
  }
  __syncthreads();
  WB_STAMP(3);
  float o[MR][4];
#pragma unroll
  for (int r = 0; r < MR; r++) { o[r][0] = o[r][1] = o[r][2] = o[r][3] = 0.f; }
  if constexpr (PS) {
#pragma unroll
    for (int r = 0; r < MR; r++) {
      if ((deadm >> r) & 1) continue;
#pragma unroll
      for (int i = 0; i < RPG; i++) {
        const float hv = hid[r][jb + i];
        o[r][0] += hv * w2[i].x; o[r][1] += hv * w2[i].y; o[r][2] += hv * w2[i].z; o[r][3] += hv * w2[i].w;
      }
    }
  } else {
#pragma unroll
  for (int i = 0; i < RPG; i++) {
#pragma unroll
    for (int r = 0; r < MR; r++) {
      const float hv = hid[r][jb + i];
      o[r][0] += hv * w2[i].x; o[r][1] += hv * w2[i].y; o[r][2] += hv * w2[i].z; o[r][3] += hv * w2[i].w;
    }
  }
  }
  if (p2 && jg > 0) {
#pragma unroll
    for (int r = 0; r < MR; r++)
      *reinterpret_cast<float4*>(&obuf[((jg - 1) * MR + r) * d + cf * 4]) = make_float4(o[r][0], o[r][1], o[r][2], o[r][3]);
  }
  __syncthreads();
  if (jg == 0) {
#pragma unroll
    for (int g2 = 1; g2 < G; g2++) {
#pragma unroll
      for (int r = 0; r < MR; r++) {
        const float4 t = *reinterpret_cast<const float4*>(&obuf[((g2 - 1) * MR + r) * d + cf * 4]);
        o[r][0] += t.x; o[r][1] += t.y; o[r][2] += t.z; o[r][3] += t.w;
      }
    }
    if constexpr (PS) {
      const Buf16 pgo(a.g_P);
#pragma unroll
      for (int r = 0; r < MR; r++)
        if (r < n_rows && !((deadm >> r) & 1))
          st_gran4(pgo, (uint32_t)((jblk * a.S + r) * d + cf * 4), ps.tag_out, make_float4(o[r][0], o[r][1], o[r][2], o[r][3]));
    } else {
#pragma unroll
      for (int r = 0; r < MR; r++)
        if (r < n_rows)
          *reinterpret_cast<float4*>(&a.P[((int64_t)jblk * a.S + r) * d + cf * 4]) = make_float4(o[r][0], o[r][1], o[r][2], o[r][3]);
    }
  }
  if (jblk == 0) {
    if constexpr (PS) {
      const Buf16 xgo(a.g_x_out);
#pragma unroll
      for (int i = 0; i < EPT; i++) {
        const int e = tid + NT * i;
        if (e < n_rows * d && !((deadm >> (e / d)) & 1)) st_gran(xgo, (uint32_t)e, ps.tag_out, xv_fold[i]);
      }
    } else {
#pragma unroll
      for (int i = 0; i < EPT; i++) {
        const int e = tid + NT * i;
        if (e < n_rows * d) a.x_out[e] = xv_fold[i];
      }
    }
  }
  WB_STAMP(4);
  WB_STAMP_FLUSH(a, 5);
  return true;
}

#ifndef WB_ATTN_NREG_PS6
#define WB_ATTN_NREG_PS6 4
#endif
template <int DPL, bool PS, int RS>
constexpr int attn_nreg() { return (PS && DPL == 6 && RS > 0) ? (WB_ATTN_NREG_PS6) : 2; }
template <int DPL, bool PS, int RS = 0, int NREG = attn_nreg<DPL, PS, RS>()>
__device__ __forceinline__ bool dec_attn_body(const AttnFusedArgs& a, const int h, const int r, const PsStep& ps, AttnLds<DPL>& sm,
                                              const float4* res = nullptr) {
  constexpr int NT = 512;
  constexpr int d = 64 * DPL;
  constexpr int KW = d / 8;
  constexpr int RK = DPL >= 6 ? 8 : 16;
  constexpr int NIT = KW / RK;
  constexpr int CF = d / 4;
  constexpr int G = CF <= 32 ? 8 : 4;
  constexpr int RPG = 64 / G;
  constexpr int PT = 128, PSL = PT * 16 / NT;
  using RG = ResGeom<DPL, 1, PS ? RS : 0>;
  static_assert(G == AttnLds<DPL>::G && RG::RK == RK && RG::NIT == NIT && RG::RPG == RPG && NT == ROLE_NT, "LDS struct / resident geometry");
  auto& hs = sm.hs; auto& red = sm.red; auto& qkv = sm.qkv; auto& tbs = sm.tbs; auto& sc = sm.sc; auto& part = sm.part; auto& att = sm.att;
  WB_STAMP(0);
  const int tid = role_tid<PS>(), lane = tid & 63, wave = tid >> 6;
  if (h >= a.n_head) return true;
  int n_rows, len, step_par, dead;
  if constexpr (PS) { n_rows = ps.n_rows; len = ps.step + 1; step_par = 0; dead = 0; }
  else {
    n_rows = a.st[ST_N]; len = a.st[a.lay.len + r]; step_par = a.st[ST_STEP] & 1;
    dead = a.st[a.lay.dead + r];
  }
  const int seg = lane >> 4, c4 = (lane & 15) * 4;
  const bool seg_ok = seg < 3;
  const float* wq = a.Wqkv + (int64_t)(wave * KW) * a.ldqkv + (seg_ok ? seg : 0) * d + h * 64 + c4;
  static_assert(NREG == 2 || (NREG == 4 && NIT == 6 && (RG::NRND == 0 || RG::NRND == 2)), "register rounds: 2, or 4 of the 6 at d = 384");
  float4 wr[NREG][RK];
  auto load_round =[&](float4 (&w)[RK], int it) {
#pragma unroll
    for (int j = 0; j < RK; j++) w[j] = ld_w4(wq + (int64_t)(RK * it + j) * a.ldqkv);
  };
  float xfold;
  const int own_col = wave * KW + (lane < KW ? lane : 0);
  float g_own = 0.f, b_own = 0.f;
  float qbias = 0.f;
  const int npast = len - 1;
  const int rg = tid >> 4, pq4 = (tid & 15) * 4;
  const int* tb = a.tabs + (size_t)step_par * a.lay.S * a.Lmax + r * a.Lmax;
  auto slot_of = [&](int p) { if constexpr (PS) return p * a.lay.S + r; else return tb[p]; };
  int slot_new = 0;
  const Buf16 kbuf(a.Kc), vbuf(a.Vc);
  float4 kc[PSL], vc[PSL];
  auto load_cache_tile = [&]() {
    int slot[PSL];
#pragma unroll
    for (int i = 0; i < PSL; i++) slot[i] = slot_of(rg + 32 * i < npast ? rg + 32 * i : 0);
    slot_new = slot_of(npast);
    if constexpr (!PS) {
      if (npast > PT)
        for (int p = tid; p < npast; p += NT) tbs[p] = tb[p];
    }
#pragma unroll
    for (int i = 0; i < PSL; i++) kc[i] = ld_f4<PS>(a.Kc, kbuf, (uint32_t)(slot[i] * d + h * 64 + pq4));
#pragma unroll
    for (int i = 0; i < PSL; i++) vc[i] = ld_f4<PS>(a.Vc, vbuf, (uint32_t)(slot[i] * d + h * 64 + pq4));
  };
  {
    const int c = tid < d ? tid : 0;
    const float* pp = a.pend + (int64_t)r * d + c;
    const int64_t plane = (int64_t)a.S * d;
    auto load_weights = [&]() {
      g_own = gld(a.ln_g + own_col); b_own = gld(a.ln_b + own_col);
      load_round(wr[0], 0);
      if (NIT > 1) load_round(wr[1], 1);
      if constexpr (NREG == 4) {
        const int it2 = (RG::NRND > 0 && res != nullptr) ? 2 + RG::NRND : 2;
        load_round(wr[2], it2);
        load_round(wr[3], it2 + 1);
      }
      if constexpr (PS && NREG == 2) { if (tid < 192) qbias = gld(a.bqkv + (tid >> 6) * d + h * 64 + (tid & 63)); }
    };
    if constexpr (PS) {
#if !defined(WB_PS_DRY)
      if (!ps.known_dead) {
        load_weights();
        if constexpr (NREG == 2) load_cache_tile();
      }
#endif
      float v = 0.f;
      bool picked = false;
      if (ps.pk_rec != nullptr && !ps.known_dead) {
        const int go = hx_wait_two(ps.pk_go, ps.pk_go_target, ps.ctr, ps.target - 1u, ps.ctl, ps.step, ps.ctr_index, ps.lds_flag,
                                   ps.dead + (r < n_rows ? r : 0));
        if (go == 0) return false;
        ps_stamp(ps, 1);
        if (r < n_rows && go == 1) {
          ps_nap<WB_PS_PICK_NAP>();
          const int tok = ps_pick_token(ps.pk_rec, ps.pk_n_tiles, ps.pk_tag, ps, red, tid);
          if (!ps_sweeps_ok(ps)) return false;
          if (tok != PS_PICK_NONE && tok != ps.pk_eot) {
            v = gld(ps.pk_E + (int64_t)tok * d + c) + gld(ps.pk_pos + c);
            picked = true;
          }
        }
      }
      if (!picked) {
      if (!ps_wait(ps)) return false;
      dead = ps.known_dead ? 1 : ld_i<true>(ps.dead + r);
      if (r >= n_rows || dead) { ps.saw_dead = true; return true; }
      const Buf16 xgb(a.g_x_in), pgb(a.g_pend);
      const uint32_t pvo = (uint32_t)(r * d + c);
      const int iplane = a.S * d;
      if (a.KSp > 0) ps_nap<2>();
      constexpr int FP = 4 * DPL;
      float accp = a.KSp > 0 ? gld(a.pbias + c) : 0.f;
      unsigned sweeps = 0;
      Gran gx{0u, 0.f}, g[FP];
#pragma unroll
      for (int j = 0; j < FP; j++) g[j] = Gran{0u, 0.f};
      for (;;) {
        if (gx.tag != ps.tag_in) gx = ld_gran(xgb, pvo, 0u);
        if (a.KSp > 0) {
#pragma unroll
          for (int j = 0; j < FP; j++)
            if (j < a.KSp && g[j].tag != ps.tag_in) g[j] = ld_gran(pgb, pvo, (uint32_t)(j * iplane));
        }
        bool ok = gx.tag == ps.tag_in;
        if (a.KSp > 0) {
#pragma unroll
          for (int j = 0; j < FP; j++) ok &= (j >= a.KSp) || g[j].tag == ps.tag_in;
        }
        if (ok) {
          v = gx.v;
          if (a.KSp > 0) {
#pragma unroll
            for (int j = 0; j < FP; j++) accp += (j < a.KSp) ? g[j].v : 0.f;
            v += accp;
          }
          break;
        }
        if (ps_sweep_retry(sweeps, ps)) { *ps.lds_flag = 0; break; }
      }
      }
      xfold = v;
      if (tid < d) hs[tid] = v;
#if !defined(WB_PS_DRY)
      if constexpr (NREG == 4) {
        load_cache_tile();
        if (tid < 192) qbias = gld(a.bqkv + (tid >> 6) * d + h * 64 + (tid & 63));
      }
#endif
    } else {
    float v = a.x_in[(int64_t)r * d + c];
    constexpr int FP = 32;
    float t[FP];
    float accp = 0.f;
    if (a.KSp > 0) {
      accp = gld(a.pbias + c);
#pragma unroll
      for (int j = 0; j < FP; j++) t[j] = pp[(int64_t)min(j, a.KSp - 1) * plane];
    }
    load_weights();
    if (r >= n_rows || dead) return true;
    if (a.KSp > 0) {
#pragma unroll
      for (int j = 0; j < FP; j++) accp += (j < a.KSp) ? t[j] : 0.f;
      for (int sp = FP; sp < a.KSp; sp += FP) {
#pragma unroll
        for (int j = 0; j < FP; j++) t[j] = pp[(int64_t)min(sp + j, a.KSp - 1) * plane];
#pragma unroll
        for (int j = 0; j < FP; j++) accp += (sp + j < a.KSp) ? t[j] : 0.f;
      }
      v += accp;
    }
    xfold = v;
    if (tid < d) hs[tid] = v;
    }
  }
  if constexpr (!PS) qbias = tid < 192 ? a.bqkv[(tid >> 6) * d + h * 64 + (tid & 63)] : 0.f;
  if constexpr (!PS) load_cache_tile();
  WB_STAMP(1);
  if constexpr (PS) ps_stamp(ps, 2);
  __syncthreads();
  if constexpr (PS) { if (!ps_sweeps_ok(ps)) return false; }
#if defined(WB_PS_DRY)
  if constexpr (PS) {
    if (tid < d / 4) { const Buf16 pgo(a.g_P); st_gran4(pgo, (uint32_t)((h * a.S + r) * d + tid * 4), ps.tag_out, make_float4(0.f, 0.f, 0.f, 0.f)); }
    if (h == 0 && tid < d) { const Buf16 xgo(a.g_x_out); st_gran(xgo, (uint32_t)(r * d + tid), ps.tag_out, xfold); }
    return true;
  }
#endif
  float xn_own;
  {
    float mean, denom;
    ln_stats_lds<DPL>(hs, d, lane, a.ln_eps, a.ln_inside, mean, denom);
    xn_own = (hs[own_col] - mean) / denom * g_own + b_own;
  }
  if constexpr (PS) ps_stamp_fine(ps, 4);
  WB_STAMP(2);
  const int nres = (RG::NRND > 0 && res != nullptr) ? RG::NRND : 0;
  const int nreg = NIT - nres;
  float acc[4] = {0.f, 0.f, 0.f, 0.f};
  if constexpr (NREG == 4) {
    auto fma_round = [&](const float4 (&w)[RK], const int kb) {
#pragma unroll
      for (int j = 0; j < RK; j++) {
        const float xv = __int_as_float(__builtin_amdgcn_readlane(__float_as_int(xn_own), kb + j));
        acc[0] += xv * w[j].x; acc[1] += xv * w[j].y; acc[2] += xv * w[j].z; acc[3] += xv * w[j].w;
      }
    };
    fma_round(wr[0], 0);
    if (nres == 0) load_round(wr[0], 4);
    fma_round(wr[1], RK);
    if (nres == 0) load_round(wr[1], 5);
    if (nres > 0) {
      if constexpr (RG::NRND > 0) {
#pragma unroll 1
        for (int q = 0; q < RG::NRND; q++) {
          float4 wl[RK];
#pragma unroll
          for (int j = 0; j < RK; j++) wl[j] = res_ld(res, 0, RG::QL, q * RK + j, RG::q_holder(wave, lane));
          fma_round(wl, RK * (2 + q));
        }
      }
      fma_round(wr[2], 4 * RK);
      fma_round(wr[3], 5 * RK);
    } else {
      fma_round(wr[2], 2 * RK);
      fma_round(wr[3], 3 * RK);
      fma_round(wr[0], 4 * RK);
      fma_round(wr[1], 5 * RK);
    }
  } else {
#pragma unroll 1
  for (int n = 0; n < nreg; n += 2) {
#pragma unroll
    for (int b = 0; b < 2; b++) {
      if (n + b < nreg) {
        const int kb = RK * (n + b < 2 ? n + b : n + b + nres);
#pragma unroll
        for (int j = 0; j < RK; j++) {
          const float xv = __int_as_float(__builtin_amdgcn_readlane(__float_as_int(xn_own), kb + j));
          acc[0] += xv * wr[b][j].x; acc[1] += xv * wr[b][j].y; acc[2] += xv * wr[b][j].z; acc[3] += xv * wr[b][j].w;
        }
        if (n + b + 2 < nreg) load_round(wr[b], n + b + 2 + nres);
      }
      if constexpr (RG::NRND > 0) {
        if (b == 1 && n == 0 && nres > 0) {
#pragma unroll 1
          for (int q = 0; q < RG::NRND; q++) {
            float4 wl[RK];
#pragma unroll
            for (int j = 0; j < RK; j++) wl[j] = res_ld(res, 0, RG::QL, q * RK + j, RG::q_holder(wave, lane));
            const int kb = RK * (2 + q);
#pragma unroll
            for (int j = 0; j < RK; j++) {
              const float xv = __int_as_float(__builtin_amdgcn_readlane(__float_as_int(xn_own), kb + j));
              acc[0] += xv * wl[j].x; acc[1] += xv * wl[j].y; acc[2] += xv * wl[j].z; acc[3] += xv * wl[j].w;
            }
          }
        }
      }
    }
  }
  }
  WB_STAMP(3);
  if constexpr (PS) ps_stamp(ps, 3);
  __syncthreads();
  const int cf = tid % CF, jg = tid / CF;
  const bool p5 = jg < G;
  const int jb = (p5 ? jg : 0) * RPG;
  float4 wo[RPG];
  {
    const float* wp = a.Wo + (int64_t)(h * 64 + jb) * d + cf * 4;
    if (RG::NWO_A == 0 || res == nullptr) {
#pragma unroll
      for (int i = 0; i < RG::NWO_A; i++) wo[i] = ld_w4(wp + (int64_t)i * d);
    }
#pragma unroll
    for (int i = RG::NWO_A; i < RPG; i++) wo[i] = ld_w4(wp + (int64_t)i * d);
  }
  if (seg_ok) *reinterpret_cast<float4*>(&red[wave * 192 + seg * 64 + c4]) = make_float4(acc[0], acc[1], acc[2], acc[3]);
  __syncthreads();
  if (tid < 192) {
    float v = 0.f;
#pragma unroll
    for (int w8 = 0; w8 < 8; w8++) v += red[w8 * 192 + tid];
    v += qbias;
    if (tid < 128) v *= a.scale;
    qkv[tid] = v;
  }
  __syncthreads();
  if constexpr (PS) ps_stamp_fine(ps, 5);
  WB_STAMP(4);
  {
    const float4 q4 = *reinterpret_cast<const float4*>(&qkv[pq4]);
    auto row_dot = [&](const float4& k4) {
      float s = q4.x * k4.x + q4.y * k4.y + q4.z * k4.z + q4.w * k4.w;
      s += dpp_f<DPP_QUAD_XOR1, 0xF>(0.f, s);
      s += dpp_f<DPP_QUAD_XOR2, 0xF>(0.f, s);
      s += dpp_f<DPP_ROW_HALF_MIRROR, 0xF>(0.f, s);
      s += dpp_f<DPP_ROW_MIRROR, 0xF>(0.f, s);
      return s;
    };
#pragma unroll
    for (int i = 0; i < PSL; i++) {
      const int p = rg + 32 * i;
      const float s = row_dot(kc[i]);
      if ((tid & 15) == 0 && p < npast) sc[p] = s;
    }
    for (int t0 = PT; t0 < npast; t0 += PT) {
      float4 kt[PSL];
#pragma unroll
      for (int i = 0; i < PSL; i++) {
        const int p = min(t0 + rg + 32 * i, npast - 1);
        int sl;
        if constexpr (PS) sl = p * a.lay.S + r; else sl = tbs[p];
        kt[i] = ld_f4<PS>(a.Kc, kbuf, (uint32_t)(sl * d + h * 64 + pq4));
      }
#pragma unroll
      for (int i = 0; i < PSL; i++) {
        const int p = t0 + rg + 32 * i;
        const float s = row_dot(kt[i]);
        if ((tid & 15) == 0 && p < npast) sc[p] = s;
      }
    }
    if (wave == 7) {
      const float s = wave_sum(qkv[lane] * qkv[64 + lane]);
      if (lane == 0) sc[npast] = s;
    }
  }
  __syncthreads();
  WB_STAMP(5);
  if constexpr (PS) ps_stamp(ps, 4);
  float m = -INFINITY;
  for (int p = lane; p < len; p += 64) m = fmaxf(m, sc[p]);
  m = wave_max(m);
  float l = 0.f;
  for (int p = lane; p < len; p += 64) l += expf(sc[p] - m);
  l = wave_sum(l);
  {
    float4 o = make_float4(0.f, 0.f, 0.f, 0.f);
#pragma unroll
    for (int i = 0; i < PSL; i++) {
      const int p = rg + 32 * i;
      const float pk = p < npast ? expf(sc[p] - m) : 0.f;
      o.x += pk * vc[i].x; o.y += pk * vc[i].y; o.z += pk * vc[i].z; o.w += pk * vc[i].w;
    }
    for (int t0 = PT; t0 < npast; t0 += PT) {
      float4 vt[PSL];
#pragma unroll
      for (int i = 0; i < PSL; i++) {
        const int p = min(t0 + rg + 32 * i, npast - 1);
        int sl;
        if constexpr (PS) sl = p * a.lay.S + r; else sl = tbs[p];
        vt[i] = ld_f4<PS>(a.Vc, vbuf, (uint32_t)(sl * d + h * 64 + pq4));
      }
#pragma unroll
      for (int i = 0; i < PSL; i++) {
        const int p = t0 + rg + 32 * i;
        const float pk = p < npast ? expf(sc[p] - m) : 0.f;
        o.x += pk * vt[i].x; o.y += pk * vt[i].y; o.z += pk * vt[i].z; o.w += pk * vt[i].w;
      }
    }
    *reinterpret_cast<float4*>(&part[rg][pq4]) = o;
  }
  __syncthreads();
  if (tid < 64) {
    float v = 0.f;
#pragma unroll
    for (int g2 = 0; g2 < 32; g2++) v += part[g2][tid];
    v += expf(sc[npast] - m) * qkv[128 + tid];
    att[tid] = v / l;
  }
  __syncthreads();
  WB_STAMP(6);
  if constexpr (PS) ps_stamp(ps, 5);
  if constexpr (RG::NWO_A > 0) {
    if (res != nullptr) {
#pragma unroll
      for (int i = 0; i < RG::NWO_A; i++) wo[i] = res_ld(res, RG::WO_A, RG::WL, i, RG::wo_holder(tid));
    }
  }
  float ov[4] = {0.f, 0.f, 0.f, 0.f};
#pragma unroll
  for (int i = 0; i < RPG; i++) {
    const float av = att[jb + i];
    ov[0] += av * wo[i].x; ov[1] += av * wo[i].y; ov[2] += av * wo[i].z; ov[3] += av * wo[i].w;
  }
  if (p5 && jg > 0)
    *reinterpret_cast<float4*>(&red[(jg - 1) * d + cf * 4]) = make_float4(ov[0], ov[1], ov[2], ov[3]);
  __syncthreads();
  if (jg == 0) {
#pragma unroll
    for (int g2 = 1; g2 < G; g2++) {
      const float4 t = *reinterpret_cast<const float4*>(&red[(g2 - 1) * d + cf * 4]);
      ov[0] += t.x; ov[1] += t.y; ov[2] += t.z; ov[3] += t.w;
    }
    if constexpr (PS) {
      const Buf16 pgo(a.g_P);
      st_gran4(pgo, (uint32_t)((h * a.S + r) * d + cf * 4), ps.tag_out, make_float4(ov[0], ov[1], ov[2], ov[3]));
    } else {
      *reinterpret_cast<float4*>(&a.P[((int64_t)h * a.S + r) * d + cf * 4]) = make_float4(ov[0], ov[1], ov[2], ov[3]);
    }
  }
  if (tid >= 64 && tid < 192) {
    float* dst = (tid < 128 ? a.Kc : a.Vc) + (int64_t)slot_new * d + h * 64 + (tid & 63);
    st_f<PS>(dst, qkv[tid]);
  }
  if (h == 0 && tid < d) {
    if constexpr (PS) { const Buf16 xgo(a.g_x_out); st_gran(xgo, (uint32_t)(r * d + tid), ps.tag_out, xfold); }
    else a.x_out[(int64_t)r * d + tid] = xfold;
  }
  WB_STAMP(7);
  WB_STAMP_FLUSH(a, 8);
  return true;
}

template <int DPL, int RS>
__device__ __forceinline__ void dec_attn_res_fill(const AttnFusedArgs& a, const int h, float4* res) {
  using RG = ResGeom<DPL, 1, RS>;
  constexpr int d = 64 * DPL, KW = d / 8, RK = RG::RK, CF = d / 4, G = RG::G, RPG = RG::RPG;
  const int tid = role_tid<true>(), lane = tid & 63, wave = tid >> 6;
  const int seg = lane >> 4, c4 = (lane & 15) * 4;
  const float* wq = a.Wqkv + (int64_t)(wave * KW) * a.ldqkv + (seg < 3 ? seg : 0) * d + h * 64 + c4;
#pragma unroll 1
  for (int q = 0; q < RG::NRND; q++) {
    float4 w[RK];
#pragma unroll
    for (int j = 0; j < RK; j++) w[j] = ld_w4(wq + (int64_t)(RK * (2 + q) + j) * a.ldqkv);
#pragma unroll
    for (int j = 0; j < RK; j++)
      if (seg < 3) res_st(res, 0, RG::QL, q * RK + j, RG::q_holder(wave, lane), w[j]);
  }
  if constexpr (RG::NWO_A > 0) {
    const int cf = tid % CF, jg = tid / CF;
    const int jb = (jg < G ? jg : 0) * RPG;
    const float* wp = a.Wo + (int64_t)(h * 64 + jb) * d + cf * 4;
    float4 w[RG::NWO_A];
#pragma unroll
    for (int i = 0; i < RG::NWO_A; i++) w[i] = ld_w4(wp + (int64_t)i * d);
#pragma unroll
    for (int i = 0; i < RG::NWO_A; i++)
      if (jg < G) res_st(res, RG::WO_A, RG::WL, i, tid, w[i]);
  }
}

template <int DPL, bool PS, int NP = 1, int RS = 0>
__device__ __forceinline__ bool dec_cross_body(const CrossFusedArgs& a, const int h, const int r, const PsStep& ps,
                                               CrossLds<DPL, NP>& sm, const float4* res = nullptr) {
  constexpr int NT = 512;
  constexpr int PASS_C = CROSS_FUSED_MAX_C, CMAX = NP * PASS_C;
  constexpr int d = 64 * DPL;
  constexpr int NWQ = d / 32;
  constexpr int CF = d / 4;
  constexpr int G = CF <= 32 ? 8 : 4;
  constexpr int RPG = 64 / G;
  constexpr int KT = 128, NTILE = CROSS_FUSED_MAX_C / KT, SL = KT * 16 / NT;
  static_assert(CROSS_FUSED_MAX_C % KT == 0 && SL * NT == KT * 16, "tile geometry");
  using RG = ResGeom<DPL, NP, PS ? RS : 0>;
  static_assert(G == CrossLds<DPL, NP>::G && CMAX == CrossLds<DPL, NP>::CMAX && RG::SL == SL && RG::NTILE == NTILE && RG::RPG == RPG &&
                NT == ROLE_NT, "LDS struct / resident geometry");
  auto& hs = sm.hs; auto& red = sm.red; auto& qv = sm.qv; auto& sc = sm.sc; auto& pbuf = sm.pbuf; auto& part = sm.part; auto& att = sm.att;
  auto& obuf = sm.obuf; auto& wmax = sm.wmax;
  const bool res_v = RG::NVT > 0 && res != nullptr;
  const int tid = role_tid<PS>(), lane = tid & 63, wave = tid >> 6;
  if (h >= a.n_head) return true;
  int n_live, w_row, dead;
  if constexpr (PS) { n_live = ps.n_rows; w_row = r; dead = 0; }
  else {
    n_live = a.st[ST_N]; w_row = a.st[a.lay.win + r];
    dead = a.st[a.lay.dead + r];
  }
  const int wi8 = min(lane & 7, a.lay.W - 1);
  const int vC8 = gld(a.win_C + wi8), vR8 = gld(a.win_row0 + wi8);
  float xfold;
  const int rg = tid >> 4, c4 = (tid & 15) * 4;
  constexpr int NOWN = 4 * NWQ;
  const int own_col = 4 * wave + (lane & 3) + 32 * ((lane < NOWN ? lane : 0) >> 2);
  float g_own = 0.f, b_own = 0.f;
  float4 wqr[NWQ];
  float4 kv[NTILE][SL];
  const float* Kh; const float* Vh; int C;
  float qbias = 0.f;
  auto load_weights = [&]() {
    g_own = gld(a.ln_g + own_col); b_own = gld(a.ln_b + own_col);
    if constexpr (PS) { if (tid < 64) qbias = gld(a.bq + h * 64 + tid); }
    {
      const float* wp = a.Wq + (int64_t)rg * d + h * 64 + c4;
#pragma unroll
      for (int i = 0; i < NWQ; i++) wqr[i] = ld_w4(wp + (int64_t)(32 * i) * d);
    }
  };
  auto load_keys = [&]() {
    int C_w, row0_w;
    {
      const int ws = __builtin_amdgcn_readfirstlane(w_row);
      if (ws < 8) { C_w = __builtin_amdgcn_readlane(vC8, ws); row0_w = __builtin_amdgcn_readlane(vR8, ws); }
      else { C_w = gld(a.win_C + ws); row0_w = gld(a.win_row0 + ws); }
    }
    C = min(C_w, CMAX);
    Kh = a.ckv + (int64_t)row0_w * a.ldkv + a.koff + h * 64;
    Vh = Kh + d;
#pragma unroll
    for (int t = 0; t < NTILE; t++)
#pragma unroll
      for (int i = 0; i < SL; i++) {
        const int key = min(t * KT + rg + 32 * i, C - 1);
        kv[t][i] = gld4(Kh + (key * a.ldkv + c4));
      }
  };
  {
    const int c = tid < d ? tid : 0;
    const float* pp = a.pend + (int64_t)r * d + c;
    const int64_t plane = (int64_t)a.S * d;
    if constexpr (PS) {
#if !defined(WB_PS_DRY)
      if (!ps.known_dead) {
        load_weights();
        load_keys();
      }
#endif
      if (!ps_wait(ps)) return false;
      dead = ps.known_dead ? 1 : ld_i<true>(ps.dead + r);
      if (r >= n_live || dead) { ps.saw_dead = true; return true; }
      const Buf16 xgb(a.g_x_in), pgb(a.g_pend);
      const uint32_t pvo = (uint32_t)(r * d + c);
      const int iplane = a.S * d;
      if (ps.cross_early) ps_nap<WB_PS_CROSS0_NAP>(); else ps_nap<4>();
      constexpr int FP = 8;
      float v = 0.f, accp = gld(a.pbias + c);
      unsigned sweeps = 0;
      Gran gx{0u, 0.f}, g[FP];
#pragma unroll
      for (int j = 0; j < FP; j++) g[j] = Gran{0u, 0.f};
      for (;;) {
        if (gx.tag != ps.tag_in) gx = ld_gran(xgb, pvo, 0u);
#pragma unroll
        for (int j = 0; j < FP; j++)
          if (j < a.KSp && g[j].tag != ps.tag_in) g[j] = ld_gran(pgb, pvo, (uint32_t)(j * iplane));
        bool ok = gx.tag == ps.tag_in;
#pragma unroll
        for (int j = 0; j < FP; j++) ok &= (j >= a.KSp) || g[j].tag == ps.tag_in;
        if (ok) {
#pragma unroll
          for (int j = 0; j < FP; j++) accp += (j < a.KSp) ? g[j].v : 0.f;
          v = gx.v + accp;
          break;
        }
        if (ps_sweep_retry(sweeps, ps)) { *ps.lds_flag = 0; break; }
      }
      xfold = v;
      if (tid < d) hs[tid] = v;
    } else {
    float v = a.x_in[(int64_t)r * d + c];
    constexpr int FP = 16;
    float t[FP];
    float accp = 0.f;
    if (a.KSp > 0) {
      accp = gld(a.pbias + c);
#pragma unroll
      for (int j = 0; j < FP; j++) t[j] = pp[(int64_t)min(j, a.KSp - 1) * plane];
    }
    load_weights();
    if (r >= n_live || dead) return true;
    if (a.KSp > 0) {
#pragma unroll
      for (int j = 0; j < FP; j++) accp += (j < a.KSp) ? t[j] : 0.f;
      for (int sp = FP; sp < a.KSp; sp += FP) {
#pragma unroll
        for (int j = 0; j < FP; j++) t[j] = pp[(int64_t)min(sp + j, a.KSp - 1) * plane];
#pragma unroll
        for (int j = 0; j < FP; j++) accp += (sp + j < a.KSp) ? t[j] : 0.f;
      }
      v += accp;
    }
    xfold = v;
    if (tid < d) hs[tid] = v;
    }
  }
  if constexpr (!PS) qbias = tid < 64 ? a.bq[h * 64 + tid] : 0.f;
  if constexpr (!PS) load_keys();
  if constexpr (PS) ps_stamp(ps, 2);
  __syncthreads();
  if constexpr (PS) { if (!ps_sweeps_ok(ps)) return false; }
#if defined(WB_PS_DRY)
  if constexpr (PS) {
    if (tid < d / 4) { const Buf16 pgo(a.g_P); st_gran4(pgo, (uint32_t)((h * a.S + r) * d + tid * 4), ps.tag_out, make_float4(0.f, 0.f, 0.f, 0.f)); }
    if (h == 0 && tid < d) { const Buf16 xgo(a.g_x_out); st_gran(xgo, (uint32_t)(r * d + tid), ps.tag_out, xfold); }
    return true;
  }
#endif
  float xn_own;
  {
    float mean, denom;
    ln_stats_lds<DPL>(hs, d, lane, a.ln_eps, a.ln_inside, mean, denom);
    xn_own = (hs[own_col] - mean) / denom * g_own + b_own;
  }
  if constexpr (PS) ps_stamp_fine(ps, 4);
  {
    float acc[4] = {0.f, 0.f, 0.f, 0.f};
    const int q4 = lane >> 4;
#pragma unroll
    for (int i = 0; i < NWQ; i++) {
      const float xv = lane_get(xn_own, 4 * i + q4);
      acc[0] += xv * wqr[i].x; acc[1] += xv * wqr[i].y; acc[2] += xv * wqr[i].z; acc[3] += xv * wqr[i].w;
    }
#pragma unroll
    for (int c = 0; c < 4; c++) { acc[c] = xor16_sum(acc[c]); acc[c] = xor32_sum(acc[c]); }
    if (lane < 16) *reinterpret_cast<float4*>(&red[wave][c4]) = make_float4(acc[0], acc[1], acc[2], acc[3]);
  }
  __syncthreads();
  if constexpr (PS) ps_stamp_fine(ps, 5);
  const int cf = tid % CF, jg = tid / CF;
  const bool p5 = jg < G;
  const int jb = (p5 ? jg : 0) * RPG;
  float4 wo[RPG];
  {
    const float* wp = a.Wo + (int64_t)(h * 64 + jb) * d + cf * 4;
    if (RG::NWO_X == 0 || res == nullptr) {
#pragma unroll
      for (int i = 0; i < RG::NWO_X; i++) wo[i] = ld_w4(wp + (int64_t)i * d);
    }
#pragma unroll
    for (int i = RG::NWO_X; i < RPG; i++) wo[i] = ld_w4(wp + (int64_t)i * d);
  }
  if (tid < 64) {
    float v = 0.f;
#pragma unroll
    for (int w8 = 0; w8 < 8; w8++) v += red[w8][tid];
    qv[tid] = (v + qbias) * a.scale;
  }
  __syncthreads();
  if constexpr (PS) ps_stamp(ps, 3);
  {
    const float4 q4 = *reinterpret_cast<const float4*>(&qv[c4]);
#pragma unroll
    for (int p = 0; p < NP; p++) {
      const float* nxt = p + 1 < NP ? Kh + (p + 1) * PASS_C * a.ldkv : Vh;
      int rgp = rg;
      if constexpr (NP > 1) WB_LAUNDER_V(rgp);
#pragma unroll
      for (int t = 0; t < NTILE; t++) {
        if constexpr (NP > 1) __builtin_amdgcn_sched_barrier(0);
#pragma unroll
        for (int i = 0; i < SL; i++) {
          const int k0 = t * KT + rgp + 32 * i, key = p * PASS_C + k0;
          float s = q4.x * kv[t][i].x + q4.y * kv[t][i].y + q4.z * kv[t][i].z + q4.w * kv[t][i].w;
          s += dpp_f<DPP_QUAD_XOR1, 0xF>(0.f, s);
          s += dpp_f<DPP_QUAD_XOR2, 0xF>(0.f, s);
          s += dpp_f<DPP_ROW_HALF_MIRROR, 0xF>(0.f, s);
          s += dpp_f<DPP_ROW_MIRROR, 0xF>(0.f, s);
          if ((tid & 15) == 0 && key < C) sc[key] = s;
          const int lim = p + 1 < NP ? max(C - 1 - (p + 1) * PASS_C, -(p + 1) * PASS_C) : C - 1;
          if (t >= RG::NVT || !res_v) kv[t][i] = gld4(nxt + (min(k0, lim) * a.ldkv + c4));
        }
      }
    }
  }
  __syncthreads();
  if constexpr (PS) ps_stamp(ps, 4);
  constexpr int KPT = (CMAX + NT - 1) / NT;
  float m;
  {
    float sv[KPT];
#pragma unroll
    for (int i = 0; i < KPT; i++) sv[i] = sc[min(tid + NT * i, CMAX - 1)];
    float mt = -INFINITY;
#pragma unroll
    for (int i = 0; i < KPT; i++) mt = fmaxf(mt, tid + NT * i < C ? sv[i] : -INFINITY);
    mt = wave_max(mt);
    if (lane == 0) wmax[wave] = mt;
    __syncthreads();
    const float4 m0 = *reinterpret_cast<const float4*>(&wmax[0]), m1 = *reinterpret_cast<const float4*>(&wmax[4]);
    m = fmaxf(fmaxf(fmaxf(m0.x, m0.y), fmaxf(m0.z, m0.w)), fmaxf(fmaxf(m1.x, m1.y), fmaxf(m1.z, m1.w)));
#pragma unroll
    for (int i = 0; i < KPT; i++)
      if (tid + NT * i < C) pbuf[tid + NT * i] = expf(sv[i] - m);
  }
  __syncthreads();
  float l = 0.f;
  if (tid < 64) {
    constexpr int KPL = CMAX / 64;
    float pv[KPL];
#pragma unroll
    for (int i = 0; i < KPL; i++) pv[i] = pbuf[lane + 64 * i];
#pragma unroll
    for (int i = 0; i < KPL; i++) l += lane + 64 * i < C ? pv[i] : 0.f;
    l = wave_sum(l);
  }
  {
    float4 o = make_float4(0.f, 0.f, 0.f, 0.f);
#pragma unroll
    for (int p = 0; p < NP; p++) {
      int rgp = rg;
      if constexpr (NP > 1) WB_LAUNDER_V(rgp);
#pragma unroll
      for (int t = 0; t < NTILE; t++) {
        if constexpr (NP > 1) WB_PIN_F4(o);
#pragma unroll
        for (int i = 0; i < SL; i++) {
          const int k0 = t * KT + rgp + 32 * i, key = p * PASS_C + k0;
          const float pk = key < C ? pbuf[key] : 0.f;
          if (t < RG::NVT) { if (res_v) kv[t][i] = res_ld(res, 0, ROLE_NT, t * SL + i, tid); }
          o.x += pk * kv[t][i].x; o.y += pk * kv[t][i].y; o.z += pk * kv[t][i].z; o.w += pk * kv[t][i].w;
          if (p + 1 < NP)
            kv[t][i] = gld4(Vh + (min(key + PASS_C, C - 1) * a.ldkv + c4));
        }
      }
    }
    *reinterpret_cast<float4*>(&part[rg][c4]) = o;
  }
  __syncthreads();
  if (tid < 64) {
    float v = 0.f;
#pragma unroll
    for (int g2 = 0; g2 < 32; g2++) v += part[g2][tid];
    att[tid] = v / l;
  }
  __syncthreads();
  if constexpr (PS) ps_stamp(ps, 5);
  if constexpr (RG::NWO_X > 0) {
    if (res != nullptr) {
#pragma unroll
      for (int i = 0; i < RG::NWO_X; i++) wo[i] = res_ld(res, RG::WO_X, RG::WL, i, RG::wo_holder(tid));
    }
  }
  float ov[4] = {0.f, 0.f, 0.f, 0.f};
#pragma unroll
  for (int i = 0; i < RPG; i++) {
    const float av = att[jb + i];
    ov[0] += av * wo[i].x; ov[1] += av * wo[i].y; ov[2] += av * wo[i].z; ov[3] += av * wo[i].w;
  }
  if (p5 && jg > 0) *reinterpret_cast<float4*>(&obuf[(jg - 1) * d + cf * 4]) = make_float4(ov[0], ov[1], ov[2], ov[3]);
  __syncthreads();
  if (jg == 0) {
#pragma unroll
    for (int g2 = 1; g2 < G; g2++) {
      const float4 t = *reinterpret_cast<const float4*>(&obuf[(g2 - 1) * d + cf * 4]);
      ov[0] += t.x; ov[1] += t.y; ov[2] += t.z; ov[3] += t.w;
    }
    if constexpr (PS) {
      const Buf16 pgo(a.g_P);
      st_gran4(pgo, (uint32_t)((h * a.S + r) * d + cf * 4), ps.tag_out, make_float4(ov[0], ov[1], ov[2], ov[3]));
    } else {
      *reinterpret_cast<float4*>(&a.P[((int64_t)h * a.S + r) * d + cf * 4]) = make_float4(ov[0], ov[1], ov[2], ov[3]);
    }
  }
  if (h == 0 && tid < d) {
    if constexpr (PS) { const Buf16 xgo(a.g_x_out); st_gran(xgo, (uint32_t)(r * d + tid), ps.tag_out, xfold); }
    else a.x_out[(int64_t)r * d + tid] = xfold;
  }
  return true;
}

template <int DPL, int NP, int RS>
__device__ __forceinline__ void dec_cross_res_fill(const CrossFusedArgs& a, const int h, const int r, float4* res) {
  using RG = ResGeom<DPL, NP, RS>;
  constexpr int d = 64 * DPL, CF = d / 4, G = RG::G, RPG = RG::RPG, KT = 128, SL = RG::SL;
  const int tid = role_tid<true>();
  const int rg = tid >> 4, c4 = (tid & 15) * 4;
  if constexpr (RG::NVT > 0) {
    const int C = min(gld(a.win_C + r), CROSS_FUSED_MAX_C), row0 = gld(a.win_row0 + r);
    const float* Vh = a.ckv + (int64_t)row0 * a.ldkv + a.koff + h * 64 + d;
#pragma unroll 1
    for (int t = 0; t < RG::NVT; t++) {
      float4 v[SL];
#pragma unroll
      for (int i = 0; i < SL; i++) v[i] = gld4(Vh + (min(t * KT + rg + 32 * i, C - 1) * a.ldkv + c4));
#pragma unroll
      for (int i = 0; i < SL; i++) res_st(res, 0, ROLE_NT, t * SL + i, tid, v[i]);
    }
  }
  if constexpr (RG::NWO_X > 0) {
    const int cf = tid % CF, jg = tid / CF;
    const int jb = (jg < G ? jg : 0) * RPG;
    const float* wp = a.Wo + (int64_t)(h * 64 + jb) * d + cf * 4;
    float4 w[RG::NWO_X];
#pragma unroll
    for (int i = 0; i < RG::NWO_X; i++) w[i] = ld_w4(wp + (int64_t)i * d);
#pragma unroll
    for (int i = 0; i < RG::NWO_X; i++)
      if (jg < G) res_st(res, RG::WO_X, RG::WL, i, tid, w[i]);
  }
}


}
}
```

whisper-burn_amd/csrc/decode_persist.hip:

```cpp
#include <hip/hip_runtime.h>

#include <climits>
#include <vector>

#include "decode.h"
#include "decode_fused_bodies.h"
#include "handoff.h"
#include "wave_ops.h"

namespace wb {
namespace {

using namespace fused;

constexpr int PS_NT = 512;
constexpr int PS_CT = 128;
constexpr int PS_NGO = 16;

template <int DPL>
struct FinLnLds { alignas(16) float hs[64 * DPL]; };
template <int DPL>
__device__ __forceinline__ bool ps_finln_role(const PersistArgs& a, const int r, const PsStep& ps, FinLnLds<DPL>& sm) {
  constexpr int d = 64 * DPL, FP = 4 * DPL;
  auto& hs = sm.hs;
  const int tid = role_tid<true>(), lane = tid & 63, wave = tid >> 6;
  const int c = tid < d ? tid : 0;
  const float g_own = a.ln_g[c], b_own = a.ln_b[c];
  float accp = a.b2_last[c];
  if (!ps_wait(ps)) return false;
  if (ld_i<true>(ps.dead + r) != 0) return true;
  ps_nap<2>();
  const Buf16 xgb(a.x_fin), pgb(a.P2);
  const uint32_t pvo = (uint32_t)(r * d + c);
  const int iplane = a.S * d;
  float v = 0.f;
  unsigned sweeps = 0;
  Gran gx{0u, 0.f}, g[FP];
#pragma unroll
  for (int j = 0; j < FP; j++) g[j] = Gran{0u, 0.f};
  for (;;) {
    if (gx.tag != ps.tag_in) gx = ld_gran(xgb, pvo, 0u);
#pragma unroll
    for (int j = 0; j < FP; j++)
      if (j < a.nb_mlp && g[j].tag != ps.tag_in) g[j] = ld_gran(pgb, pvo, (uint32_t)(j * iplane));
    bool ok = gx.tag == ps.tag_in;
#pragma unroll
    for (int j = 0; j < FP; j++) ok &= (j >= a.nb_mlp) || g[j].tag == ps.tag_in;
    if (ok) {
#pragma unroll
      for (int j = 0; j < FP; j++) accp += (j < a.nb_mlp) ? g[j].v : 0.f;
      v = gx.v + accp;
      break;
    }
    if (ps_sweep_retry(sweeps, ps)) { *ps.lds_flag = 0; break; }
  }
  if (tid < d) hs[tid] = v;
  ps_stamp(ps, 2);
  __syncthreads();
  if (!ps_sweeps_ok(ps)) return false;
  if (wave < DPL) {
    float mean, denom;
    ln_stats_lds<DPL>(hs, d, lane, a.ln_eps, a.ln_inside, mean, denom);
    const Buf16 xo(a.g_xn);
    st_gran(xo, (uint32_t)(r * d + tid), ps.tag_out, (v - mean) / denom * g_own + b_own);
  }
  return true;
}

template <int MR, int DPL>
struct LogitsLds {
  alignas(16) float xs[MR][64 * DPL];
  alignas(16) float red[8][MR][PS_CT];
  float tilev[MR][PS_CT];
};
template <int MR, int DPL>
__device__ __forceinline__ bool ps_logits_role(const PersistArgs& a, const int tile0, const int n_t, const PsStep& ps,
                                               const bool forced, const int par, LogitsLds<MR, DPL>& sm) {
  constexpr int d = 64 * DPL, NT = PS_NT, CT = PS_CT;
  constexpr int NR = d / 16;
  constexpr int EPT = (MR * d + NT - 1) / NT;
  constexpr int PCH = EPT <= 3 ? 8 : EPT <= 6 ? 4 : 2;
  constexpr int NQ = MR * CT / NT;
  constexpr bool TWO = DPL <= 6;
  auto& xs = sm.xs; auto& red = sm.red; auto& tilev = sm.tilev;
  const int tid = role_tid<true>(), lane = tid & 63, wave = tid >> 6;
  const int hh = lane >> 5, c4 = (lane & 31) * 4;
  const Buf16 etb(a.Et);
  auto load_tile = [&](float4 (&w)[NR], int tile) {
    const int n0 = tile * CT;
    const bool col_ok = n0 + c4 < a.vocab_ld;
    const uint32_t vo = (uint32_t)((2 * wave + hh) * NR * a.vocab_ld + n0 + (col_ok ? c4 : 0));
#pragma unroll
    for (int i = 0; i < NR; i++) w[i] = ld_f4_plain(etb, vo, (uint32_t)(i * a.vocab_ld));
  };
  float4 w0[NR], w1[TWO ? NR : 1];
  if (!forced) {
#if !defined(WB_PS_DRY)
    load_tile(w0, tile0);
    if constexpr (TWO) { if (n_t > 1) load_tile(w1, tile0 + 1); }
#endif
  }
  const int use_mask = (ps.step + 1 <= a.mask_until_len) ? 1 : 0;
  int deadm = 0;
  if (!ps_wait(ps)) return false;
  {
    int off[EPT];
#pragma unroll
    for (int i = 0; i < EPT; i++) {
      int e = tid + NT * i;
      if (e >= MR * d) e = tid;
      off[i] = e;
    }
#pragma unroll
    for (int r = 0; r < MR; r++)
      if (r >= ps.n_rows || ld_i<true>(ps.dead + min(r, ps.n_rows - 1)) != 0) deadm |= 1 << r;
    const Buf16 xgb(a.g_xn);
    float v[EPT];
    unsigned sweeps = 0;
    for (;;) {
      Gran gx[EPT];
#pragma unroll
      for (int i = 0; i < EPT; i++) gx[i] = ld_gran(xgb, (uint32_t)off[i], 0u);
      bool ok = true;
#pragma unroll
      for (int i = 0; i < EPT; i++) ok &= ((deadm >> (off[i] / d)) & 1) != 0 || gx[i].tag == ps.tag_in;
      if (ok) {
#pragma unroll
        for (int i = 0; i < EPT; i++) v[i] = ((deadm >> (off[i] / d)) & 1) ? 0.f : gx[i].v;
        break;
      }
      if (ps_sweep_retry(sweeps, ps)) { *ps.lds_flag = 0; break; }
    }
#pragma unroll
    for (int i = 0; i < EPT; i++) {
      const int e = tid + NT * i;
      if (e < MR * d) (&xs[0][0])[e] = v[i];
    }
  }
  ps_stamp(ps, 2);
  __syncthreads();
  if (!ps_sweeps_ok(ps)) return false;
  ps_stamp(ps, 3);
  if (forced) return true;
#if defined(WB_PS_DRY)
  for (int t = 0; t < n_t; t++)
    if (wave < MR && !((deadm >> wave) & 1)) {
      const int r_u = __builtin_amdgcn_readfirstlane(wave);
      if (lane == 0) st_rec(Buf16(a.tstats), (uint32_t)((par * a.S + r_u) * a.n_tiles + tile0 + t), ps.tag_in, 0.f, (tile0 + t) * CT);
    }
  return true;
#endif
  auto run_tile = [&](const float4 (&w)[NR], int tile) {
    const int n0 = tile * CT;
    float mk[NQ];
#pragma unroll
    for (int q = 0; q < NQ; q++) {
      const int col = n0 + ((tid + NT * q) & (CT - 1));
      mk[q] = (use_mask && col < a.V) ? a.mask[col] : 0.f;
    }
    float acc[MR][4];
#pragma unroll
    for (int r = 0; r < MR; r++) { acc[r][0] = acc[r][1] = acc[r][2] = acc[r][3] = 0.f; }
#pragma unroll
    for (int r = 0; r < MR; r++) {
      if ((deadm >> r) & 1) continue;
#pragma unroll
      for (int i4 = 0; i4 < NR; i4 += 4) {
        const float4 xv = *reinterpret_cast<const float4*>(&xs[r][(2 * wave + hh) * NR + i4]);
        acc[r][0] += xv.x * w[i4].x; acc[r][1] += xv.x * w[i4].y; acc[r][2] += xv.x * w[i4].z; acc[r][3] += xv.x * w[i4].w;
        acc[r][0] += xv.y * w[i4 + 1].x; acc[r][1] += xv.y * w[i4 + 1].y; acc[r][2] += xv.y * w[i4 + 1].z; acc[r][3] += xv.y * w[i4 + 1].w;
        acc[r][0] += xv.z * w[i4 + 2].x; acc[r][1] += xv.z * w[i4 + 2].y; acc[r][2] += xv.z * w[i4 + 2].z; acc[r][3] += xv.z * w[i4 + 2].w;
        acc[r][0] += xv.w * w[i4 + 3].x; acc[r][1] += xv.w * w[i4 + 3].y; acc[r][2] += xv.w * w[i4 + 3].z; acc[r][3] += xv.w * w[i4 + 3].w;
      }
    }
#pragma unroll
    for (int r = 0; r < MR; r++)
#pragma unroll
      for (int c = 0; c < 4; c++) acc[r][c] = xor32_sum(acc[r][c]);
    __syncthreads();
    if (hh == 0) {
#pragma unroll
      for (int r = 0; r < MR; r++)
        *reinterpret_cast<float4*>(&red[wave][r][c4]) = make_float4(acc[r][0], acc[r][1], acc[r][2], acc[r][3]);
    }
    __syncthreads();
#pragma unroll
    for (int q = 0; q < NQ; q++) {
      const int e = tid + NT * q, r = e / CT, c = e & (CT - 1);
      float v = 0.f;
#pragma unroll
      for (int w8 = 0; w8 < 8; w8++) v += red[w8][r][c];
      v += mk[q];
      if (n0 + c >= a.V) v = -INFINITY;
      tilev[r][c] = v;
    }
    __syncthreads();
    if (wave < MR && !((deadm >> wave) & 1)) {
      const int r = wave;
      const float v0 = tilev[r][lane], v1 = tilev[r][lane + 64];
      float bvv; int bi;
      if (better(v0, lane, v1, lane + 64)) { bvv = v0; bi = lane; } else { bvv = v1; bi = lane + 64; }
      wave_argmax(bvv, bi);
      const int r_u = __builtin_amdgcn_readfirstlane(r);
      if (lane == 0) st_rec(Buf16(a.tstats), (uint32_t)((par * a.S + r_u) * a.n_tiles + tile), ps.tag_in, bvv, n0 + bi);
    }
  };
  run_tile(w0, tile0);
  ps_stamp(ps, 4);
  if constexpr (TWO) {
    if (n_t > 1) run_tile(w1, tile0 + 1);
    ps_stamp(ps, 5);
    for (int t = 2; t < n_t; t++) { load_tile(w0, tile0 + t); run_tile(w0, tile0 + t); }
  } else {
    for (int t = 1; t < n_t; t++) { load_tile(w0, tile0 + t); run_tile(w0, tile0 + t); }
  }
  return true;
}

struct MergeLds { float redv[8]; int redi[8]; unsigned tgt[8]; };
__device__ __forceinline__ bool ps_merge_role(const PersistArgs& a, const int r, const int e, const PsStep& ps0,
                                              const unsigned* clog, const int* n_per_ctr, MergeLds& sm) {
  auto& redv = sm.redv; auto& redi = sm.redi;
  const int tid = role_tid<true>(), lane = tid & 63, wave = tid >> 6;
  const PsStep& ps = ps0;
  {
    auto& tgt = sm.tgt;
    if (tid < 8) tgt[tid] = (unsigned)(e + 1) * (unsigned)n_per_ctr[tid];
    __syncthreads();
    if (!hx_wait_many(clog, tgt, 8, ps.ctl, ps.step, 1000, ps.lds_flag)) return false;
  }
  ps_stamp(ps, 1);
  const int len = ps.step + 1;
  const int fin_now = ld_i<true>(a.dead + r);
  const int tok_prev = ld_i<true>(a.gctl + GC_HDR + r);
  int gi;
  if (e < a.n_forced) {
    gi = a.forced[e];
  } else {
    float bv = -INFINITY; int bi = 0x7fffffff;
    const Buf16 recb(a.tstats);
    for (int t = tid; t < a.n_tiles; t += PS_NT) {
      const Rec q = ld_rec(recb, (uint32_t)(((e & 1) * a.S + r) * a.n_tiles + t));
      if (better(q.v, q.id, bv, bi)) { bv = q.v; bi = q.id; }
    }
    wave_argmax(bv, bi);
    if (lane == 0) { redv[wave] = bv; redi[wave] = bi; }
    __syncthreads();
    float gv = redv[0]; gi = redi[0];
#pragma unroll
    for (int j = 1; j < 8; j++)
      if (better(redv[j], redi[j], gv, gi)) { gv = redv[j]; gi = redi[j]; }
    if ((unsigned)gi >= 0x7fffffffu) { gi = a.eot; if (tid == 0) a.gctl[GC_BAD] = 1; }
  }
  const int finished = fin_now || (gi == a.eot && e >= a.n_forced);
  const int tok_next = fin_now ? tok_prev : gi;
  if (tid == 0 && !fin_now) {
    st_i_sc1(a.gctl + GC_HDR + r, gi);
    a.gtok[r * a.Lmax + len] = gi;
    a.gctl[GC_HDR + 2 * a.S + r] = len + 1;
    if (gi == a.eot && e >= a.n_forced) {
      a.gctl[GC_HDR + a.S + r] = 1;
      st_i_sc1(a.dead + r, 1);
      const unsigned n = __hip_atomic_fetch_add(reinterpret_cast<unsigned*>(a.ctl + HX_NDONE), 1u, __ATOMIC_RELAXED,
                                                __HIP_MEMORY_SCOPE_AGENT) + 1u;
      if ((int)n == ps.n_rows) st_i_sc1(a.ctl + HX_STOP, ps.step + 1);
    }
  }
  if (tid == 0 && r == 0) a.gctl[GC_STEP] = ps.step + 1;
  if (len < a.Lmax) {
    const Buf16 xb(a.x0);
    const float4* ev = reinterpret_cast<const float4*>(a.E + (int64_t)tok_next * a.d);
    const float4* pp = reinterpret_cast<const float4*>(a.pos + (int64_t)len * a.d);
    const unsigned tag_x = a.tag_base + 1u + 3u * (unsigned)((e + 1) * a.n_layer);
    for (int c = tid; c < (a.d >> 2); c += PS_NT) {
      const float4 x = ev[c], y = pp[c];
      st_gran4(xb, (uint32_t)(r * a.d + 4 * c), tag_x, make_float4(x.x + y.x, x.y + y.y, x.z + y.z, x.w + y.w));
    }
    const int nstep = ps.step + 1;
    int* tab_new = a.tabs + (size_t)(nstep & 1) * a.S * a.Lmax;
    for (int p = tid; p <= len; p += PS_NT) tab_new[r * a.Lmax + p] = p * a.S + r;
  }
  (void)finished;
  return true;
}

template <int DPL, int MR, int NP>
union PsRoleLds {
  MlpLds<MR, DPL, false> mlp; AttnLds<DPL> attn; CrossLds<DPL, NP> cross;
  FinLnLds<DPL> finln; LogitsLds<MR, DPL> logits; MergeLds merge;
};
constexpr int PS_LDS_BYTES = 160 * 1024;
constexpr bool ps_resident_instance(int DPL, int MR, int NP) { return !(DPL >= 6 && (MR == 8 || NP == 2)); }
template <int DPL, int MR, int NP>
struct PsArena {
  static constexpr int ROLE_BYTES = (int)((sizeof(PsRoleLds<DPL, MR, NP>) + 15) / 16 * 16);
  static constexpr int FLAG_BYTES = 16;
  static constexpr int RS = ps_resident_instance(DPL, MR, NP) ? (PS_LDS_BYTES - ROLE_BYTES - FLAG_BYTES) / (PS_NT * 16) : 0;
  static constexpr int BYTES = ROLE_BYTES + FLAG_BYTES + RS * PS_NT * 16;
  static_assert(RS >= 0 && BYTES <= PS_LDS_BYTES, "the persistent kernel's LDS arena exceeds 160 KB");
  static constexpr bool USEFUL = ResGeom<DPL, NP, RS>::WO_A + ResGeom<DPL, NP, RS>::NWO_A + ResGeom<DPL, NP, RS>::WO_X +
                                 ResGeom<DPL, NP, RS>::NWO_X > 0;
};
static_assert(PS_NT == ROLE_NT, "block size");
#define WB_PS_INSTANCES(X) X(2, 4, 1) X(2, 8, 1) X(6, 4, 1) X(6, 8, 1) X(8, 4, 1) X(2, 4, 2) X(6, 4, 2) X(8, 4, 2)
#define WB_PS_CHECK(DPL_, MR_, NP_) static_assert(PsArena<DPL_, MR_, NP_>::BYTES <= 160 * 1024, "LDS arena of an instance");
WB_PS_INSTANCES(WB_PS_CHECK)
#undef WB_PS_CHECK

template <int DPL, int MR, int NP>
__global__ __launch_bounds__(PS_NT) void dec_persist_kernel(PersistArgs a) {
  using AR = PsArena<DPL, MR, NP>;
  constexpr int RS = AR::RS;
  __shared__ PsRoleLds<DPL, MR, NP> lds;
  __shared__ __attribute__((aligned(16))) int wait_flag[AR::FLAG_BYTES / 4];
  __shared__ __attribute__((aligned(16))) float4 res_buf[RS > 0 ? RS * PS_NT : 1];
  static_assert(sizeof(lds) <= AR::ROLE_BYTES && sizeof(wait_flag) == AR::FLAG_BYTES && sizeof(res_buf) <= (RS > 0 ? RS : 1) * PS_NT * 16 &&
                AR::BYTES + (RS > 0 ? 0 : 16) <= PS_LDS_BYTES, "the three LDS objects are what PsArena accounts for");
  const int NL = a.n_layer, S = a.S, R = a.n_rows, H = a.n_head, NB = a.nb_mlp;
  auto cptr = [&](int c) { return reinterpret_cast<unsigned*>(a.ctl + HX_HDR + c * HX_LINE); };
  const int C_X = 0, C_ATTN = S, C_CROSS = S + NL * S, C_MLP = C_CROSS + NL, C_LOG = C_MLP + NL, C_GO = C_LOG + 8;
  int n_per_ctr[8];
#pragma unroll
  for (int k = 0; k < 8; k++) n_per_ctr[k] = (a.n_logits_roles + 7 - k) / 8;
  const int i_lo = a.role_off[blockIdx.x], i_hi = a.role_off[blockIdx.x + 1];
#if defined(WB_PS_DRY)
  constexpr bool RES = false;
#else
  constexpr bool RES = RS > 0;
#endif
  int res_i = -1;
  if (RES && a.res_role != nullptr) res_i = a.res_role[blockIdx.x];
  if (res_i >= i_lo && res_i < i_hi) {
    const PsRole role = a.roles[res_i];
    if (role.kind == PSR_ATTN) dec_attn_res_fill<DPL, RS>(a.layers[role.layer].attn, role.a, res_buf);
    else if (role.kind == PSR_CROSS) dec_cross_res_fill<DPL, NP, RS>(a.layers[role.layer].cross, role.a, role.b, res_buf);
  }
  unsigned long long dead_seen = 0;
  for (int e = 0; e < a.n_steps; e++) {
    for (int i = i_lo; i < i_hi; i++) {
      const PsRole role = a.roles[i];
      PsStep ps;
      ps.known_dead = i - i_lo < 64 && ((dead_seen >> (i - i_lo)) & 1ull) != 0;
      ps.ctl = a.ctl; ps.step = a.step0 + e; ps.n_rows = R; ps.dead = a.dead; ps.lds_flag = &wait_flag[0];
      unsigned long long* stp = a.stamps ? a.stamps + ((size_t)e * a.n_roles + i) * PS_STAMPS : nullptr;
      if (stp && threadIdx.x == 0) stp[0] = wall_clock64();
      ps.stamp = stp;
      int out;
      bool ok;
      const unsigned tag_l = a.tag_base + 2u + 3u * (unsigned)(e * NL + (role.kind <= PSR_MLP ? role.layer : NL - 1));
      const bool pick_e = a.pick != 0 && e >= 1 && e - 1 >= a.n_forced && ps.step < a.Lmax;
      if (role.kind == PSR_ATTN) {
        const AttnFusedArgs la = a.layers[role.layer].attn;
        if (role.layer == 0) { ps.ctr_index = C_X + role.b; ps.target = (unsigned)e; }
        else { ps.ctr_index = C_CROSS + role.layer - 1; ps.target = (unsigned)(e + 1) * H * R; }
        ps.ctr = cptr(ps.ctr_index);
        ps.tag_out = tag_l; ps.tag_in = tag_l - 1u;
        if (role.layer == 0 && pick_e) {
          ps.pk_rec = static_cast<const char*>(a.tstats) + ((size_t)((e - 1) & 1) * S + role.b) * a.n_tiles * sizeof(Rec);
          ps.pk_n_tiles = a.n_tiles;
          ps.pk_tag = a.tag_base + 4u + 3u * (unsigned)((e - 1) * NL + NL - 1);
          ps.pk_go = cptr(C_GO + (role.b * H + role.a) % PS_NGO); ps.pk_go_target = (unsigned)e;
          ps.pk_E = a.E; ps.pk_pos = a.pos + (int64_t)ps.step * a.d; ps.pk_eot = a.eot;
        }
        ok = dec_attn_body<DPL, true, RS>(la, role.a, role.b, ps, lds.attn, i == res_i ? res_buf : nullptr);
        out = C_ATTN + role.layer * S + role.b;
      } else if (role.kind == PSR_CROSS) {
        const CrossFusedArgs la = a.layers[role.layer].cross;
        if (role.layer == 0) { ps.ctr_index = C_X + role.b; ps.target = (unsigned)e; }
        else { ps.ctr_index = C_MLP + role.layer - 1; ps.target = (unsigned)(e + 1) * NB; }
        ps.ctr = cptr(ps.ctr_index);
        ps.tag_out = tag_l + 1u; ps.tag_in = tag_l;
        ps.cross_early = role.layer == 0 && pick_e;
        ok = dec_cross_body<DPL, true, NP, RS>(la, role.a, role.b, ps, lds.cross, i == res_i ? res_buf : nullptr);
        out = C_CROSS + role.layer;
      } else if (role.kind == PSR_MLP) {
        const MlpFusedArgs la = a.layers[role.layer].mlp;
        ps.ctr_index = C_ATTN + role.layer * S; ps.target = (unsigned)(e + 1) * H; ps.n_ctr = R;
        ps.ctr = cptr(ps.ctr_index);
        ps.tag_out = tag_l + 2u; ps.tag_in = tag_l + 1u;
        ok = dec_mlp_body<MR, DPL, false, true>(la, role.a, ps, lds.mlp);
        out = C_MLP + role.layer;
      } else if (role.kind == PSR_FINLN) {
        ps.ctr_index = C_CROSS + NL - 1; ps.target = (unsigned)(e + 1) * H * R;
        ps.ctr = cptr(ps.ctr_index);
        ps.tag_in = tag_l + 2u; ps.tag_out = tag_l + 2u;
        ok = ps_finln_role<DPL>(a, role.b, ps, lds.finln);
        out = C_GO + PS_NGO;
      } else if (role.kind == PSR_LOGITS) {
        ps.ctr_index = C_GO + (role.layer % PS_NGO); ps.target = (unsigned)(e + 1);
        ps.ctr = cptr(ps.ctr_index);
        ps.tag_in = tag_l + 2u;
        ok = ps_logits_role<MR, DPL>(a, role.a, role.b, ps, e < a.n_forced, e & 1, lds.logits);
        out = C_LOG + (role.layer & 7);
      } else {
        ok = ps_merge_role(a, role.b, e, ps, cptr(C_LOG), n_per_ctr, lds.merge);
        out = C_X + role.b;
      }
      if (!ok) return;
      if (ps.saw_dead && i - i_lo < 64) dead_seen |= 1ull << (i - i_lo);
      if (stp && threadIdx.x == 0) stp[6] = wall_clock64();
      if (role.kind == PSR_CROSS && role.layer == NL - 1)
        hx_arrive_broadcast(cptr(out), (unsigned)(e + 1) * H * R, cptr(C_GO), PS_NGO, (unsigned)(e + 1));
      else
        hx_arrive(cptr(out));
      if (stp && threadIdx.x == 0) stp[7] = wall_clock64();
    }
  }
}

__global__ void ps_seed_kernel(const float* __restrict__ x, int n, void* gx, unsigned tag, int* ctl) {
  if (blockIdx.x == 0 && threadIdx.x == 0) ctl[HX_STOP] = INT_MAX;
  const Buf16 b(gx);
  for (int i = blockIdx.x * blockDim.x + threadIdx.x; i < n; i += gridDim.x * blockDim.x) st_gran(b, (uint32_t)i, tag, x[i]);
}

__global__ __launch_bounds__(PS_NT) void ps_pick_test_kernel(const void* rec, int n_tiles, unsigned tag, int* ctl, int* out_id) {
  __shared__ float xch[16];
  __shared__ int flag;
  PsStep ps;
  ps.ctl = ctl; ps.step = -1; ps.lds_flag = &flag;
  if (threadIdx.x == 0) flag = 1;
  __syncthreads();
  const int tok = ps_pick_token(rec, n_tiles, tag, ps, xch, role_tid<true>());
  if (threadIdx.x == 0) *out_id = ps_sweeps_ok(ps) ? tok : -1;
}

template <int DPL, int MR, int NP>
int max_blocks_per_cu() {
  int nb = 0;
  if (hipOccupancyMaxActiveBlocksPerMultiprocessor(&nb, (dec_persist_kernel<DPL, MR, NP>), PS_NT, 0) != hipSuccess) return 0;
  return nb;
}

}

int dec_persist_resident_slots(int d, int n_rows, int max_keys) {
  if (!dec_persist_supported(d, n_rows, max_keys)) return 0;
  const int dpl = d / 64, mr = n_rows > 4 ? 8 : 4, np = max_keys > CROSS_FUSED_MAX_C ? 2 : 1;
#define WB_PS_SLOTS(DPL_, MR_, NP_) \
  if (dpl == DPL_ && mr == MR_ && np == NP_) return PsArena<DPL_, MR_, NP_>::USEFUL ? PsArena<DPL_, MR_, NP_>::RS : 0;
  WB_PS_INSTANCES(WB_PS_SLOTS)
#undef WB_PS_SLOTS
  return 0;
}

bool dec_persist_resident_geometry(int d, int n_rows, int max_keys, int out[5]) {
  if (!dec_persist_supported(d, n_rows, max_keys)) return false;
  const int dpl = d / 64, mr = n_rows > 4 ? 8 : 4, np = max_keys > CROSS_FUSED_MAX_C ? 2 : 1;
#define WB_PS_GEOM(DPL_, MR_, NP_)                                                            \
  if (dpl == DPL_ && mr == MR_ && np == NP_) {                                                \
    using RG = ResGeom<DPL_, NP_, PsArena<DPL_, MR_, NP_>::RS>;                               \
    out[0] = PsArena<DPL_, MR_, NP_>::RS; out[1] = RG::NRND; out[2] = RG::NWO_A; out[3] = RG::NVT; out[4] = RG::NWO_X; \
    if (PsArena<DPL_, MR_, NP_>::RS == 0) out[1] = out[2] = out[3] = out[4] = 0;              \
    return true;                                                                              \
  }
  WB_PS_INSTANCES(WB_PS_GEOM)
#undef WB_PS_GEOM
  return false;
}

int ps_ctl_ints(int S, int n_layer) { return HX_HDR + (S + n_layer * S + 2 * n_layer + 8 + PS_NGO + 1) * HX_LINE; }

bool dec_persist_supported(int d, int n_rows, int max_keys) {
  if (n_rows < 1 || n_rows > 8) return false;
  if (max_keys > CROSS_FUSED_MAX_PASSES * CROSS_FUSED_MAX_C) return false;
  if (max_keys > CROSS_FUSED_MAX_C && n_rows > 4) return false;
  if (d == 128 || d == 384) return true;
  return d == 512 && n_rows <= 4;
}

int dec_persist_max_grid(int device, int d, int n_rows, int max_keys) {
  if (!dec_persist_supported(d, n_rows, max_keys)) return 0;
  int cus = 0, coop = 0;
  if (hipDeviceGetAttribute(&coop, hipDeviceAttributeCooperativeLaunch, device) != hipSuccess || !coop) return 0;
  if (hipDeviceGetAttribute(&cus, hipDeviceAttributeMultiprocessorCount, device) != hipSuccess || cus <= 0) return 0;
  int per = 0;
  const bool big = n_rows > 4;
  if (max_keys > CROSS_FUSED_MAX_C)
    per = d == 128 ? max_blocks_per_cu<2, 4, 2>() : d == 384 ? max_blocks_per_cu<6, 4, 2>() : max_blocks_per_cu<8, 4, 2>();
  else if (d == 128) per = big ? max_blocks_per_cu<2, 8, 1>() : max_blocks_per_cu<2, 4, 1>();
  else if (d == 384) per = big ? max_blocks_per_cu<6, 8, 1>() : max_blocks_per_cu<6, 4, 1>();
  else per = max_blocks_per_cu<8, 4, 1>();
  if (per <= 0) return 0;
  return cus * 1;
}

void launch_ps_seed(hipStream_t st, const float* x, int n, void* gx, unsigned tag, int* ctl) {
  hipLaunchKernelGGL(ps_seed_kernel, dim3((n + 255) / 256), dim3(256), 0, st, x, n, gx, tag, ctl);
}

void launch_ps_pick_test(hipStream_t st, const void* rec, int n_tiles, unsigned tag, int* ctl, int* out_id) {
  hipLaunchKernelGGL(ps_pick_test_kernel, dim3(1), dim3(PS_NT), 0, st, rec, n_tiles, tag, ctl, out_id);
}

int launch_dec_persist(hipStream_t st, const PersistArgs& a, int grid) {
  const dim3 g(grid), b(PS_NT);
  const bool big = a.n_rows > 4;
  hipError_t e = hipErrorInvalidValue;
#define WB_PS(DPL_, MR_, NP_) e = WB_LAUNCH_COOP((dec_persist_kernel<DPL_, MR_, NP_>), g, b, 0, st, a)
  if (a.n_pass > 1) {
    if (big) return -1;
    if (a.d == 128) WB_PS(2, 4, 2); else if (a.d == 384) WB_PS(6, 4, 2); else if (a.d == 512) WB_PS(8, 4, 2);
  }
  else if (a.d == 128) { if (big) WB_PS(2, 8, 1); else WB_PS(2, 4, 1); }
  else if (a.d == 384) { if (big) WB_PS(6, 8, 1); else WB_PS(6, 4, 1); }
  else if (a.d == 512 && !big) WB_PS(8, 4, 1);
#undef WB_PS
  return e == hipSuccess ? 0 : -1;
}

}
```

whisper-burn_amd/csrc/session.h:

```cpp
#pragma once
#include <vector>

#include "decode.h"
#include "engine.h"

namespace wb {
struct TsBeamResult {
  int W = 0, depth = 0;
  std::vector<int> n_cand, best, n_steps;
  std::vector<std::vector<std::vector<int32_t>>> cand_tokens;
  std::vector<std::vector<double>> cand_score, cand_rank;
  std::vector<int> tr_n, tr_fin;
  std::vector<int32_t> tr_tok, tr_par;
  std::vector<double> tr_score;
};
}

struct wb_session {
  wb_model* m = nullptr;
  uint64_t model_uid = 0;
  int device = 0;
  hipStream_t st = nullptr;
  hipStream_t st2 = nullptr;
  hipEvent_t ev_seg = nullptr;
  int W = 0, max_beams = 0, S = 0, padding = 0;
  double sample_rate = 16000.0;
  int Lmax = 0;
  std::vector<int> T, C, row0;
  std::vector<wb::MelWindow> wins_host; void* wins_dev_ptr = nullptr;
  std::vector<int> meta_host; void* meta_dev_ptr = nullptr;
  std::vector<uint8_t> mask_host; void* mask_dev_ptr = nullptr;
  int enc_rows = 0, maxC = 0, n_chunks = 0;
  wb::Workspace ws;
  wb::DevMem pcm, mel, wins, gmax, enc_out, ckv, win_meta;
  float* pcm_stage = nullptr; size_t pcm_stage_bytes = 0;
  wb::DevMem kc, vc, tabs, state;
  wb::StepLayout lay;
  char* host_block = nullptr;
  char* host_block_dev = nullptr;
  size_t host_bytes = 0;
  size_t chain_flags_off = 0;
  int* state_host = nullptr;
  int32_t* topk_id_host = nullptr;
  float* topk_lp_host = nullptr;
  wb::DevMem x, h, att, Pqkv, Po, Pq, P1, P2, Pa, Pc, carec, ca, logits, tstats, row_stats, mask, lp_tmp, gctl, gtok, hm;
  int sk_qkv = 0, sk_o = 0, sk_1 = 0, sk_2 = 0;
  wb::DevMem ps_layers, ps_roles, ps_ctl, ps_dead, ps_tstats, ps_stamps;
  wb::DevMem ps_gx, ps_gpa, ps_gpc, ps_gp2, ps_gxn;
  unsigned ps_launches = 0;
  int ps_grid = -1;
  std::vector<uint64_t> ps_setup_key;
  std::vector<wb::PsRole> ps_roles_host;
  std::vector<int> ps_role_off_host;
  int ps_setup_grid = 0, ps_setup_n_lg = 0, ps_setup_n_res = 0;
  int* ps_pin = nullptr; size_t ps_pin_ints = 0;
  bool ps_pin_busy = false;
  int n_tiles_v = 0, ct_v = 128;
  int ks_qkv = 1, ksl_qkv = 0, ks_o = 1, ksl_o = 0, ks_1 = 1, ksl_1 = 0, ks_2 = 1, ksl_2 = 0, ks_v = 1, ksl_v = 0;
  wb::DevMem bc_ctl, bc_topk;
  wb::DevMem sc_ctl, sc_topk;
  uint64_t sample_sig = 0;
  std::vector<int32_t> smp_tokens, smp_len; int smp_best_of = 0, smp_depth = 0;
  wb::DevMem ts_ctl, ts_topk, ts_sup;
  std::vector<uint8_t> ts_sup_host; void* ts_sup_dev_ptr = nullptr;
  bool has_suppress = false;
  uint64_t ts_sig = 0;
  wb::DevMem tb_ctl, tb_topk;
  uint64_t tsbeam_sig = 0;
  wb::TsBeamResult tb_last;
  std::vector<int> prev_len, prev_win;
  int prev_n = 0, step = 0;
  bool has_mask = false, decode_ready = false;
  int last_use_mask = 0, last_had_logits = 0;
  wb::PrefillJob prefill_job;
  int prefill_mode = 0;
  int prof_cls_cross = -1, prof_cls_self = -1, prof_step_off = 0;
  int* guard_host = nullptr; int* guard_dev = nullptr;
  bool enc_guard_pending = false;
  wb::MelBatch enc_mb;
  std::unordered_map<uint64_t, hipGraphExec_t> graphs;
  int64_t n_captures = 0;
  uint64_t buf_sig = 0;
  uint64_t beam_sig = 0;
  void clear_graphs();
  ~wb_session();
};

namespace wb {
struct Profile {
  bool on = false;
  double ms[8] = {0, 0, 0, 0, 0, 0, 0, 0};
};
Profile& profile();
struct KernelStat { int64_t calls = 0; double ms = 0, bytes = 0; };
void prof_adjust_bytes(int cls, double delta);
void prof_collect();
struct ScopedTimer {
  hipStream_t st; int slot; hipEvent_t a = nullptr, b = nullptr; bool on;
  ScopedTimer(hipStream_t s, int slot_);
  void stop();
  void collect();
  ~ScopedTimer();
};

void session_pool_register(wb_model* m);
void session_pool_purge(wb_model* m);
int session_create(wb_model* m, int n_windows, int max_beams, int padding, wb_session** out);
int session_encode_pcm(wb_session* s, const float* pcm, int64_t n_pcm, const int64_t* starts, const int64_t* lens,
                       bool pcm_on_device, bool defer_guard = false);
int session_enc_guard_resolve(wb_session* s, bool* reencoded);
void session_rewind(wb_session* s);
int session_reserve(wb_session* s, int max_len);
int session_prefill(wb_session* s, const int32_t* tokens, int n, const int* wa, int nA);
int session_prefill_prompt(wb_session* s, const int32_t* prompt, int P, const int* wa, int nA);
int session_beam_chain(wb_session* s, const int32_t* prompt, int prompt_len, int beam_size, int eot, int max_depth,
                       int mask_until_len, int32_t* out_tokens, int32_t row_stride, int32_t* out_lens, bool* handled);
struct SampleCall { float temperature; int best_of; uint64_t seed; int attempt; };
int session_sample_chain(wb_session* s, const int32_t* prompt, int prompt_len, const SampleCall& sp, const uint8_t* active,
                         const int32_t* stream_ids, int eot, int max_depth, int mask_until_len, int32_t* out_tokens,
                         int32_t row_stride, int32_t* out_lens, double* out_sum, int32_t* out_best);
int session_ts_chain(wb_session* s, const wb_timestamp_params& tp, const int32_t* prompt, int prompt_len, const uint8_t* active,
                     const int32_t* stream_ids, int eot, int max_depth, int32_t* out_tokens, int32_t row_stride,
                     int32_t* out_lens, double* out_sum, int32_t* out_best);
void pack_suppress(const uint8_t* a, const uint8_t* b, int V, uint32_t* out);
int check_ts_params(const wb_timestamp_params& tp, int V, int eot, const char* who);
int check_beam_params(const wb_timestamp_params& tp, const wb_beam_params& bp, int max_beams, int* max_candidates);
int session_tsbeam_chain(wb_session* s, const wb_timestamp_params& tp, const wb_beam_params& bp, const int32_t* prompt, int prompt_len,
                         const uint8_t* active, int eot, int max_depth, int32_t* out_tokens, int32_t row_stride, int32_t* out_lens,
                         double* out_score, int32_t* out_n_candidates);
int session_greedy_chain(wb_session* s, const int32_t* prompt, int eot, int max_depth, int mask_until_len, int prompt_len,
                         int32_t* out_tokens, int32_t row_stride, int32_t* out_lens);
int session_align(wb_session* s, const int32_t* tokens, int32_t row_stride, const int32_t* lens, const int32_t* heads,
                  int32_t n_heads, int32_t n_prefix, int32_t drop_last, int32_t filter_width, int32_t* start_pos,
                  float* matrix, const int32_t* drop_last_rows);
int session_score(wb_session* s, const int32_t* tokens, int32_t row_stride, const int32_t* lens, int32_t mask_until_len,
                  const int32_t* probe_ids, int32_t n_probe, int32_t probe_pos, float* token_logprobs,
                  float* probe_logprobs);
}
```

whisper-burn_amd/csrc/switches.h:

```cpp
#pragma once

namespace wb {
namespace sw {

enum Kind { DEFAULT_ON, OPT_IN, UNSET_OR_1, TRI, INT, STR };

#define WB_BOOL_SWITCHES(X)                                                                                                          \
  X(graph, "WHISPER_HIP_GRAPH", DEFAULT_ON, "on", "replay captured hipGraphs of the decode steps; 0: enqueue every step eagerly")    \
  X(chain, "WHISPER_HIP_CHAIN", DEFAULT_ON, "on", "device-chained greedy decode; 0: one host round trip per step")                   \
  X(beam_chain, "WHISPER_HIP_BEAM_CHAIN", DEFAULT_ON, "on", "beam bookkeeping on the device; 0: host-driven beam search")            \
  X(persist, "WHISPER_HIP_PERSIST", DEFAULT_ON, "on", "persistent flag-chained greedy kernel; 0: one launch per sublayer")           \
  X(persist_prefill, "WHISPER_HIP_PERSIST_PREFILL", DEFAULT_ON, "on", "the persistent launch runs the prompt itself; 0: host prefill") \
  X(prefill_pass, "WHISPER_HIP_PREFILL_PASS", DEFAULT_ON, "on", "a session's prefill mode 1 is honoured (one-pass prompt prefill); 0: steps everywhere") \
  X(poll, "WHISPER_HIP_POLL", DEFAULT_ON, "on", "chained greedy: spin on mapped progress flags; 0: copy + synchronise per chunk")    \
  X(speculate, "WHISPER_HIP_SPECULATE", OPT_IN, "off", "chained greedy: enqueue one segment ahead of the finished flags")            \
  X(fuse_sub, "WHISPER_HIP_FUSE_SUB", DEFAULT_ON, "on", "fused self-attention and MLP sublayer kernels; 0: per-matrix GEMVs")        \
  X(fuse_x, "WHISPER_HIP_FUSE_X", DEFAULT_ON, "on", "fused cross-attention sublayer kernel; 0: chunked cross-attention + GEMV")      \
  X(fuse_q, "WHISPER_HIP_FUSE_Q", DEFAULT_ON, "on", "chunked cross-attention blocks project their own queries")                      \
  X(fuse_co, "WHISPER_HIP_FUSE_CO", OPT_IN, "off", "chunked cross-attention blocks apply the out-projection too")                    \
  X(fuse16, "WHISPER_HIP_FUSE16", DEFAULT_ON, "on", "9 - 16 live rows stay on the fused sublayer kernels; 0: batch mode")            \
  X(batch_skinny, "WHISPER_HIP_BATCH_SKINNY", DEFAULT_ON, "on", "batch mode: skinny weight-stream GEMM up to 64 rows; 0: tiled GEMM") \
  X(cross_stream, "WHISPER_HIP_CROSS_STREAM", DEFAULT_ON, "on", "batch mode, one beam per window: streaming cross-attention")        \
  X(sk_pair, "WHISPER_HIP_SK_PAIR", OPT_IN, "off", "skinny GEMM: the waves' partial tiles meet pairwise")                            \
  X(mlp16_mfma, "WHISPER_HIP_MLP16_MFMA", DEFAULT_ON, "on", "9 - 16-row fused MLP on the matrix cores; 0: two row groups of 8")      \
  X(logits_mfma, "WHISPER_HIP_LOGITS_MFMA", DEFAULT_ON, "on", "9 - 16-row logits product on the matrix cores")                       \
  X(logits_preln, "WHISPER_HIP_LOGITS_PRELN", DEFAULT_ON, "on", "9 - 16-row logits: fold + LayerNorm once, in its own launch")       \
  X(logits_mr16, "WHISPER_HIP_LOGITS_MR16", DEFAULT_ON, "on", "9 - 16-row logits GEMV as one 16-row tile")                           \
  X(encoder_split, "WHISPER_HIP_ENCODER_SPLIT", UNSET_OR_1, "on", "split-precision (fp16 hi / lo) encoder-side GEMMs; 0: exact f32") \
  X(decoder_split, "WHISPER_HIP_DECODER_SPLIT", DEFAULT_ON, "on", "split-precision batch-mode decoder GEMM; 0: exact f32")           \
  X(encoder_pieces, "WHISPER_HIP_ENCODER_PIECES", DEFAULT_ON, "on", "encoder activations travel as fp16 pieces between split GEMMs") \
  X(attn_f16, "WHISPER_HIP_ATTN_F16", DEFAULT_ON, "on", "encoder attention on fp16 pieces; 0: the f32 kernels")                      \
  X(attn_kvsplit, "WHISPER_HIP_ATTN_KVSPLIT", DEFAULT_ON, "on", "encoder attention splits long key ranges across blocks")            \
  X(gpu_turn, "WHISPER_HIP_GPU_TURN", DEFAULT_ON, "on", "one entry point at a time per device and process (developer: 0 drops it)")  \
  X(session_pool, "WHISPER_HIP_SESSION_POOL", DEFAULT_ON, "on", "released sessions are parked for reuse; 0: freed (developer A/B)")  \
  X(pcm_stage, "WHISPER_HIP_PCM_STAGE", OPT_IN, "off", "host PCM is uploaded through a pinned per-session buffer")
#define WB_INT_SWITCHES(X)                                                                                                           \
  X(cross_stream_fuse, "WHISPER_HIP_CROSS_STREAM_FUSE", TRI, -1, "streaming cross-attention folds / projects its query; unset: d <= 768") \
  X(sk_max_blocks, "WHISPER_HIP_SK_MAX_BLOCKS", INT, 256, "skinny GEMM: most blocks a K-split may launch")                           \
  X(split_tile, "WHISPER_HIP_SPLIT_TILE", INT, 0, "split-precision GEMM: force a tile shape (developer A/B; 0: choose)")             \
  X(enc_trace_extra, "WHISPER_HIP_ENC_TRACE_EXTRA", INT, 0, "bit mask of extra stages in the encoder trace (1 pcm, 2 mel, 4 maxima)")
#define WB_STR_SWITCHES(X)                                                                                                           \
  X(enc_trace, "WHISPER_HIP_ENC_TRACE", STR, nullptr, "directory for per-thread dumps of the encoder stages (developer)")            \
  X(ps_stamps, "WHISPER_HIP_PS_STAMPS", STR, nullptr, "file for the persistent kernel's role timeline (developer)")                  \
  X(persist_resident, "WHISPER_HIP_PERSIST_RESIDENT", STR, nullptr, "persistent kernel: step-invariant operands stay in LDS (on); 0: off; log: on + report") \
  X(persist_setup, "WHISPER_HIP_PERSIST_SETUP", STR, nullptr, "persistent kernel: launch setup cached on the session (on); 0: built per call; log: on + report; 0log: both") \
  X(persist_deal, "WHISPER_HIP_PERSIST_DEAL", STR, nullptr, "persistent kernel: merge / final-LN roles kept off the first-layer attention blocks (on); legacy: the least loaded blocks; log: on + report") \
  X(persist_pick, "WHISPER_HIP_PERSIST_PICK", STR, nullptr, "persistent kernel: first-layer self-attention picks the next token from the tile records itself (on); merge: it waits for the merge role's row") \
  X(persist_inject_fail, "WHISPER_HIP_PERSIST_INJECT_FAIL", STR, nullptr, "test hook: \"launch\" = the cooperative launch is refused")

#define WB_SW_DECL(fn, name, kind, dflt, what) bool fn();
WB_BOOL_SWITCHES(WB_SW_DECL)
#undef WB_SW_DECL
#define WB_SW_DECL(fn, name, kind, dflt, what) int fn();
WB_INT_SWITCHES(WB_SW_DECL)
#undef WB_SW_DECL
#define WB_SW_DECL(fn, name, kind, dflt, what) const char* fn();
WB_STR_SWITCHES(WB_SW_DECL)
#undef WB_SW_DECL

}
}
```

Measured before the change: 2609 x real-time.

## Two-phase MLP in persistent decoder with final LayerNorm folded into logits roles

In the persistent decode kernel, each MLP role now publishes its GELU hidden columns to a global buffer, then reads all of them back and finishes whole residual output columns with the second bias. This replaces the partial-sum planes that later consumers had to reduce. The separate final-LN role is dropped: logits roles normalise the residual row themselves, and blocks holding last-layer MLP work get fewer logits tiles. The aim is to remove a reduction and a dependency hop on the per-token critical path, at the cost of an extra global exchange and spin-wait inside the MLP role. A switch keeps the old plane form, test kernels are added, and the profiling script gains MLP-to-consumer latency stats.

```diff
diff --git a/profiles/ps_timeline.py b/profiles/ps_timeline.py
--- a/profiles/ps_timeline.py
+++ b/profiles/ps_timeline.py
@@ -44,7 +44,7 @@
         rel_done = np.nanmean((np.nanmax(s[:, :, 6], axis=1) - step_start) * tick)
         rel_arr = np.nanmean((np.nanmax(s[:, :, 7], axis=1) - step_start) * tick)
         nm = names[k] + (f" L{l}" if k < 3 else "")
-        if k in (0, 1, 3, 4, 5):
+        if k in (0, 1, 2, 3, 4, 5):
             wp = np.nanmean((s[:, :, 1] - step_start[:, None]) * tick, axis=0)
             dn = np.nanmean((s[:, :, 6] - step_start[:, None]) * tick, axis=0)
             spread.append((nm, wp, dn, block[cols] if block is not None else None))
@@ -76,3 +76,32 @@
     if nm in ("attn L0", "merge", "finln"):
         per = "  ".join((f"b{blk[i]}:" if blk is not None else f"#{i}:") + f"{wp[i]:.2f}/{dn[i]:.2f}" for i in range(len(wp)))
         print(f"{'':<10}per role (block: wait passed @ / done @)  {per}")
+def stats(v):
+    return f"mean {np.nanmean(v):.2f} us, median {np.nanmedian(v):.2f}, min {np.nanmin(v):.2f}, max {np.nanmax(v):.2f}"
+n_layer = int(layer[kind == 2].max()) + 1 if (kind == 2).any() else 0
+for l in range(n_layer):
+    m = (kind == 2) & (layer == l)
+    mdone = sel[:, m, 6]
+    if not np.isfinite(mdone).any():
+        continue
+    last_done = np.nanmax(mdone, axis=1)
+    print(f"mlp L{l} done, last - first role inside a step ({int(m.sum())} roles): {stats((last_done - np.nanmin(mdone, axis=1)) * tick)}")
+    if l + 1 < n_layer:
+        cons, cn = (kind == 0) & (layer == l + 1) & (row == live_row), f"attn L{l + 1} p2"
+    elif (kind == 5).any():
+        cons, cn = (kind == 5) & (row == live_row), "finln p2"
+    else:
+        cons, cn = kind == 3, "logits p2"
+    if cons.any() and np.isfinite(sel[:, cons, 2]).any():
+        for nm, red in (("first", np.nanmin), ("last", np.nanmax)):
+            print(f"last mlp L{l} done -> {cn} ({nm} block): {stats((red(sel[:, cons, 2], axis=1) - last_done) * tick)}")
+a0all = (kind == 0) & (layer == 0)
+if a0all.any() and hi - lo > 1:
+    rows = sorted(set(row[a0all]))
+    n_live = np.zeros(hi - lo, dtype=int)
+    for r in rows:
+        n_live += np.isfinite(sel[:, a0all & (row == r), 2]).any(axis=1)
+    for n in sorted(set(n_live[1:]), reverse=True):
+        v = dd[n_live[1:] == n]
+        if len(v) and np.isfinite(v).any():
+            print(f"step time with {n} live row(s) ({len(v)} steps): {stats(v)}")
diff --git a/whisper-burn_amd/csrc/decode.h b/whisper-burn_amd/csrc/decode.h
--- a/whisper-burn_amd/csrc/decode.h
+++ b/whisper-burn_amd/csrc/decode.h
@@ -325,7 +325,10 @@
 bool skinny_supported(int M, int K, int N);
 int launch_dec_skinny_gemm(hipStream_t st, const SkinnyArgs& a);
 
-struct PsLayerArgs { AttnFusedArgs attn; CrossFusedArgs cross; MlpFusedArgs mlp; };
+struct PsLayerArgs {
+  AttnFusedArgs attn; CrossFusedArgs cross; MlpFusedArgs mlp;
+  const float* mlp_b2 = nullptr;
+};
 enum { PSR_ATTN = 0, PSR_CROSS = 1, PSR_MLP = 2, PSR_LOGITS = 3, PSR_MERGE = 4, PSR_FINLN = 5 };
 struct PsRole { int kind, layer, a, b; };
 constexpr int PS_MAX_FORCED = 8;
@@ -348,6 +351,8 @@
   const float* Et = nullptr; int vocab_ld = 0, V = 0; const float* mask = nullptr;
   void* tstats = nullptr; int n_tiles = 0;
   int pick = 1;
+  int mlp2 = 1;
+  void* g_hid = nullptr;
   int* gctl = nullptr; int* gtok = nullptr; int Lmax = 0, eot = 0;
   const float* E = nullptr; const float* pos = nullptr; void* x0 = nullptr; int* tabs = nullptr;
   int* dead = nullptr;
@@ -359,8 +364,10 @@
   std::vector<int> role_off;
   std::vector<int> res_role;
   int n_lg = 0, n_res = 0;
-};
-PsDeal ps_deal_roles(int n_layer, int n_head, int n_rows, int nb_mlp, int n_tiles, int grid, int policy, bool res_on);
+  std::vector<int> tail_block;
+};
+PsDeal ps_deal_roles(int n_layer, int n_head, int n_rows, int nb_mlp, int n_tiles, int grid, int policy, bool res_on,
+                     bool finln = true);
 int ps_ctl_ints(int S, int n_layer);
 bool dec_persist_supported(int d, int n_rows, int max_keys);
 int dec_persist_resident_slots(int d, int n_rows, int max_keys);
@@ -369,6 +376,12 @@
 int launch_dec_persist(hipStream_t st, const PersistArgs& a, int grid);
 void launch_ps_seed(hipStream_t st, const float* x, int n, void* gx, unsigned tag, int* ctl);
 void launch_ps_pick_test(hipStream_t st, const void* rec, int n_tiles, unsigned tag, int* ctl, int* out_id);
+struct PsMlp2TestArgs {
+  MlpFusedArgs a; int n_rows = 0; const int* dead = nullptr; void* g_hid = nullptr; const float* b2 = nullptr; unsigned tag_in = 0;
+  int* ctl = nullptr;
+};
+int launch_ps_mlp2_test(hipStream_t st, const PsMlp2TestArgs& t);
+int launch_ps_logits_test(hipStream_t st, const PersistArgs& a, unsigned tag, int n_t);
 
 #if defined(HIPEMU) && !defined(HIPEMU_PROD_GEOMETRY)
 constexpr int CROSS_FUSED_MAX_C = 384;
diff --git a/whisper-burn_amd/csrc/decode_chain.cpp b/whisper-burn_amd/csrc/decode_chain.cpp
--- a/whisper-burn_amd/csrc/decode_chain.cpp
+++ b/whisper-burn_amd/csrc/decode_chain.cpp
@@ -26,7 +26,7 @@
   return WB_OK;
 }
 
-PsDeal ps_deal_roles(int NL, int H, int W, int NB, int n_tiles, int grid, int policy, bool res_on) {
+PsDeal ps_deal_roles(int NL, int H, int W, int NB, int n_tiles, int grid, int policy, bool res_on, bool finln) {
   std::vector<PsRole> lr;
   for (int l = 0; l < NL; l++) {
     for (int r = 0; r < W; r++) for (int h = 0; h < H; h++) lr.push_back(PsRole{PSR_ATTN, l, h, r});
@@ -55,16 +55,32 @@
     std::vector<int> order(grid);
     for (int b = 0; b < grid; b++) order[b] = b;
     by_load(order);
-    for (int r = 0; r < W; r++) { fin_block[r] = order[r % grid]; deal[fin_block[r]].push_back(PsRole{PSR_FINLN, 0, 0, r}); is_fin[fin_block[r]] = 1; }
+    for (int r = 0; r < W; r++) {
+      fin_block[r] = order[r % grid];
+      if (finln) deal[fin_block[r]].push_back(PsRole{PSR_FINLN, 0, 0, r});
+      is_fin[fin_block[r]] = 1;
+    }
   }
   if ((int)cand.size() > 2 * W) cand.erase(std::remove_if(cand.begin(), cand.end(), [&](int b) { return is_fin[b] != 0; }), cand.end());
   std::stable_sort(cand.begin(), cand.end(), [&](int x, int y) { return deal[x].size() < deal[y].size(); });
-  const int tpb = (n_tiles + (int)cand.size() - 1) / (int)cand.size();
-  const int n_lg = (n_tiles + tpb - 1) / tpb;
+  int tpb = (n_tiles + (int)cand.size() - 1) / (int)cand.size();
+  std::vector<char> late(grid, 0);
+  int n_late = 0;
+  if (!finln && tpb > 1) {
+    for (int b : cand) {
+      for (const PsRole& r : deal[b]) late[b] |= r.kind == PSR_MLP && r.layer == NL - 1;
+      n_late += late[b];
+    }
+    const int n_other = (int)cand.size() - n_late;
+    if (n_late == 0 || n_other <= 0 || (n_tiles - n_late + n_other - 1) / n_other > tpb) { std::fill(late.begin(), late.end(), 0); n_late = 0; }
+  }
   std::vector<char> has_lg(grid, 0);
-  for (int q = 0; q < n_lg; q++) {
-    deal[cand[q]].push_back(PsRole{PSR_LOGITS, q, q * tpb, std::min(tpb, n_tiles - q * tpb)});
+  int n_lg = 0;
+  for (int q = 0, t0 = 0; q < (int)cand.size() && t0 < n_tiles; q++) {
+    const int n = std::min(late[cand[q]] ? 1 : tpb, n_tiles - t0);
+    deal[cand[q]].push_back(PsRole{PSR_LOGITS, n_lg++, t0, n});
     has_lg[cand[q]] = 1;
+    t0 += n;
   }
   {
     std::vector<int> order;
@@ -81,6 +97,7 @@
   }
   PsDeal out;
   out.n_lg = n_lg;
+  out.tail_block = fin_block;
   out.role_off.assign(grid + 1, 0);
   for (int b = 0; b < grid; b++) {
     out.role_off[b] = (int)out.roles.size();
@@ -98,9 +115,17 @@
   return out;
 }
 
-static void ps_deal_log(const PsDeal& deal, int grid) {
+static int ps_grid_blocks(const wb_session* s) {
+  const wb_dims& D = s->m->dims;
+  const int NB = dec_mlp_fused_planes(D.n_text_state), n_tiles = (D.n_vocab + 127) / 128;
+  const int n_layer_roles = D.n_text_layer * (2 * s->W * D.n_text_head + NB);
+  return std::max(1, std::min(s->ps_grid, n_layer_roles + n_tiles + 2 * s->W));
+}
+
+static void ps_deal_log(const PsDeal& deal, int grid, bool finln) {
   std::string where[2];
   int n_lg_blocks = 0;
+  if (!finln) for (int b : deal.tail_block) where[1] += (where[1].empty() ? "" : ",") + std::to_string(b);
   for (int b = 0; b < grid; b++) {
     bool lg = false;
     for (int i = deal.role_off[b]; i < deal.role_off[b + 1]; i++) {
@@ -113,10 +138,11 @@
     }
     n_lg_blocks += lg;
   }
-  fprintf(stderr, "persist deal: merge on blocks %s; finln on %s; logits blocks %d\n", where[0].c_str(), where[1].c_str(), n_lg_blocks);
-}
-
-static int ps_setup_ensure(wb_session* s, bool res_on, bool* built) {
+  fprintf(stderr, "persist deal: merge on blocks %s; finln on %s; logits blocks %d; mlp form %s\n", where[0].c_str(), where[1].c_str(),
+          n_lg_blocks, finln ? "planes (final-LN roles)" : "two-phase (no final-LN role: final LayerNorm inside the logits roles)");
+}
+
+static int ps_setup_ensure(wb_session* s, bool res_on, bool mlp2, bool* built) {
   wb_model* m = s->m;
   const wb_dims& D = m->dims;
   const int d = D.n_text_state, H = D.n_text_head, NL = D.n_text_layer, V = D.n_vocab, S = s->S, W = s->W;
@@ -127,8 +153,7 @@
   const size_t pool = (size_t)s->Lmax * S;
   const int ldkv = 2 * d;
   const int n_pass = s->maxC > CROSS_FUSED_MAX_C ? 2 : 1;
-  const int n_layer_roles = NL * (2 * W * H + NB);
-  const int grid = std::max(1, std::min(s->ps_grid, n_layer_roles + n_tiles + 2 * W));
+  const int grid = ps_grid_blocks(s);
   const char* deal_sw = sw::persist_deal();
   const int policy = deal_sw && !strcmp(deal_sw, "legacy") ? PS_DEAL_LEGACY : PS_DEAL_SLACK;
   auto up = [](const void* p) { return (uint64_t)reinterpret_cast<uintptr_t>(p); };
@@ -136,7 +161,7 @@
       s->model_uid, (uint64_t)W, (uint64_t)S, (uint64_t)s->Lmax, (uint64_t)grid, (uint64_t)n_tiles, (uint64_t)n_pass,
       (uint64_t)s->enc_rows, (uint64_t)res_on, (uint64_t)m->ln_eps_inside_sqrt, up(s->state.p), up(s->x.p), up(s->P2.p),
       up(s->Pa.p), up(s->Pc.p), up(s->kc.p), up(s->vc.p), up(s->tabs.p), up(s->ckv.p), up(s->win_meta.p), up(s->ps_gx.p),
-      up(s->ps_gpa.p), up(s->ps_gpc.p), up(s->ps_gp2.p), up(s->ps_gxn.p), (uint64_t)policy};
+      up(s->ps_gpa.p), up(s->ps_gpc.p), up(s->ps_gp2.p), up(s->ps_gxn.p), (uint64_t)policy, (uint64_t)mlp2};
   const char* sw_setup = sw::persist_setup();
   const bool cache_on = !(sw_setup && sw_setup[0] == '0');
   *built = !(cache_on && !s->ps_setup_key.empty() && s->ps_setup_key == key);
@@ -176,10 +201,11 @@
     ma.ln_g = b.ln3.g; ma.ln_b = b.ln3.b; ma.ln_eps = b.ln3.eps; ma.ln_inside = m->ln_eps_inside_sqrt;
     ma.W1 = b.mlp1.w; ma.ld1 = b.mlp1.n; ma.b1 = b.mlp1.b; ma.W2 = b.mlp2.w; ma.P = s->P2.as<float>();
     ma.g_x_in = gxb[xi]; ma.g_pend = s->ps_gpc.p; ma.g_x_out = gxb[xi ^ 1]; ma.g_P = s->ps_gp2.p;
+    la[l].mlp_b2 = b.mlp2.b;
     xi ^= 1;
   }
-  PsDeal deal = ps_deal_roles(NL, H, W, NB, n_tiles, grid, policy, res_on);
-  if (deal_sw && !strcmp(deal_sw, "log")) ps_deal_log(deal, grid);
+  PsDeal deal = ps_deal_roles(NL, H, W, NB, n_tiles, grid, policy, res_on, !mlp2);
+  if (deal_sw && !strcmp(deal_sw, "log")) ps_deal_log(deal, grid, !mlp2);
   std::vector<PsRole>& roles = deal.roles;
   const std::vector<int>&role_off = deal.role_off, &res_role = deal.res_role;
   const int n_lg = deal.n_lg, n_res = deal.n_res;
@@ -216,11 +242,18 @@
   WB_TRY(s->ps_gx.ensure_zeroed(((size_t)2 * S + 8) * d * 8, st));
   WB_TRY(s->ps_gpa.ensure_zeroed(((size_t)H * S + 8) * d * 8, st));
   WB_TRY(s->ps_gpc.ensure_zeroed(((size_t)H * S + 8) * d * 8, st));
-  WB_TRY(s->ps_gp2.ensure_zeroed(((size_t)NB * S + 8) * d * 8, st));
-  WB_TRY(s->ps_gxn.ensure_zeroed(((size_t)S + 8) * d * 8, st));
+  const char* mlp_sw = sw::persist_mlp();
+  const bool mlp2 = !(mlp_sw && !strcmp(mlp_sw, "planes")) && ps_grid_blocks(s) >= NB;
+  if (mlp2) {
+    WB_TRY(s->ps_ghid.ensure_zeroed(((size_t)S + 2) * 4 * d * 8, st));
+  } else {
+    WB_TRY(s->ps_gp2.ensure_zeroed(((size_t)NB * S + 8) * d * 8, st));
+    WB_TRY(s->ps_gxn.ensure_zeroed(((size_t)S + 8) * d * 8, st));
+  }
   WB_TRY(s->ps_tstats.ensure_zeroed((size_t)2 * S * n_tiles * 16, st));
   if (((s->ps_launches + 1) & 0xffffu) == 0) {
-    for (DevMem* b : {&s->ps_gx, &s->ps_gpa, &s->ps_gpc, &s->ps_gp2, &s->ps_gxn, &s->ps_tstats}) WB_HIP(hipMemsetAsync(b->p, 0, b->bytes, st));
+    for (DevMem* b : {&s->ps_gx, &s->ps_gpa, &s->ps_gpc, &s->ps_gp2, &s->ps_gxn, &s->ps_ghid, &s->ps_tstats})
+      if (b->p && b->bytes) WB_HIP(hipMemsetAsync(b->p, 0, b->bytes, st));
     s->ps_launches++;
   }
   const unsigned tag_base = ((++s->ps_launches) & 0xffffu) << 16;
@@ -228,7 +261,7 @@
   const char* res_sw = sw::persist_resident();
   const bool res_on = !(res_sw && res_sw[0] == '0') && dec_persist_resident_slots(d, W, s->maxC) > 0;
   bool built = false;
-  WB_TRY(ps_setup_ensure(s, res_on, &built));
+  WB_TRY(ps_setup_ensure(s, res_on, mlp2, &built));
   const std::vector<PsRole>& roles = s->ps_roles_host;
   const int grid = s->ps_setup_grid, n_res = s->ps_setup_n_res;
   if (res_sw && !strcmp(res_sw, "log")) fprintf(stderr, "persist resident blocks: %d of %d\n", n_res, grid);
@@ -248,6 +281,7 @@
   a.n_forced = n_forced;
   for (int i = 0; i < n_forced; i++) a.forced[i] = forced[i];
   a.g_xn = s->ps_gxn.p;
+  a.mlp2 = mlp2 ? 1 : 0; a.g_hid = s->ps_ghid.p;
   a.x_fin = gxb[(3 * NL) & 1]; a.P2 = s->ps_gp2.p; a.b2_last = m->dec[NL - 1].mlp2.b; a.tag_base = tag_base;
   a.ln_g = m->ln_dec.g; a.ln_b = m->ln_dec.b; a.ln_eps = m->ln_dec.eps; a.ln_inside = m->ln_eps_inside_sqrt;
   a.Et = m->tok_emb_t; a.vocab_ld = m->vocab_ld; a.V = V; a.mask = s->mask.as<float>();
diff --git a/whisper-burn_amd/csrc/decode_fused_bodies.h b/whisper-burn_amd/csrc/decode_fused_bodies.h
--- a/whisper-burn_amd/csrc/decode_fused_bodies.h
+++ b/whisper-burn_amd/csrc/decode_fused_bodies.h
@@ -1,5 +1,7 @@
 #pragma once
 #include <hip/hip_runtime.h>
+
+#include <cstddef>
 
 #include "decode.h"
 #include "handoff.h"
@@ -24,6 +26,8 @@
   const unsigned* pk_go = nullptr; unsigned pk_go_target = 0;
   const float* pk_E = nullptr; const float* pk_pos = nullptr; int pk_eot = 0;
   bool cross_early = false;
+  void* mlp_hid = nullptr; const float* mlp_b2 = nullptr;
+  bool x_late = false;
 };
 constexpr int PS_STAMPS = 8;
 __device__ __forceinline__ void ps_stamp(const PsStep& ps, int k) {
@@ -337,6 +341,12 @@
   float g_own = 0.f, b_own = 0.f;
   float b1v;
   int deadm = 0;
+  constexpr int NB2 = 4 * DPL, NCH = NB2 * G, CB = d / NB2, HD = 4 * d;
+  static_assert(!PS || (CB == 16 && 4 * NCH <= NT && (MR * HD) % NT == 0 && (MR & (MR - 1)) == 0), "two-phase geometry");
+  bool two = false;
+  if constexpr (PS) two = ps.mlp_hid != nullptr;
+  const int ch2 = min(tid >> 2, NCH - 1), cq = tid & 3;
+  float b2v = 0.f, xown = 0.f;
   {
     int off[EPT], col[EPT];
 #pragma unroll
@@ -366,6 +376,9 @@
       }
       {
         const float* wp = a.W2 + (int64_t)(j0 + jb) * d + cf * 4;
+        if constexpr (PS) {
+          if (two) { wp = a.W2 + (int64_t)(ch2 * RPG) * d + jblk * CB + cq * 4; b2v = gld(ps.mlp_b2 + jblk * CB + (tid & (CB - 1))); }
+        }
 #pragma unroll
         for (int i = 0; i < RPG; i++) w2[i] = ld_w4(wp + (int64_t)i * d);
       }
@@ -502,10 +515,17 @@
   if constexpr (PS) n_rows = ps.n_rows; else n_rows = min(MR, a.st[ST_N] - a.row0);
   if (n_rows <= 0) return true;
   WB_STAMP(1);
+  if constexpr (PS) ps_stamp(ps, 2);
   __syncthreads();
   if constexpr (PS) { if (!ps_sweeps_ok(ps)) return false; }
+  if constexpr (PS) { if (two) xown = hs[(tid >> 4) & (MR - 1)][jblk * CB + (tid & (CB - 1))]; }
 #if defined(WB_PS_DRY)
   if constexpr (PS) {
+    if (two) {
+      if (tid < MR * CB && (tid >> 4) < n_rows && !((deadm >> (tid >> 4)) & 1))
+        st_gran(Buf16(a.g_x_out), (uint32_t)((tid >> 4) * d + jblk * CB + (tid & (CB - 1))), ps.tag_out, xown);
+      return true;
+    }
     if (jg == 0) {
       const Buf16 pgo(a.g_P);
 #pragma unroll
@@ -561,16 +581,108 @@
     for (int r = 0; r < MR; r++)
       *reinterpret_cast<float4*>(&red[wave][r][c4]) = make_float4(acc[r][0], acc[r][1], acc[r][2], acc[r][3]);
   }
+  if constexpr (PS) ps_stamp(ps, 3);
   __syncthreads();
   if (tid < MR * HS) {
     const int r = tid >> 6, c = tid & 63;
     float v = 0.f;
 #pragma unroll
     for (int w8 = 0; w8 < 8; w8++) v += red[w8][r][c];
-    hid[r][c] = gelu_erf_f(v + b1v);
+    const float hval = gelu_erf_f(v + b1v);
+    bool pub = false;
+    if constexpr (PS) pub = two;
+    if (pub) {
+      if (!((deadm >> r) & 1)) st_gran(Buf16(ps.mlp_hid), (uint32_t)(r * HD + j0 + c), ps.tag_out, hval);
+    } else {
+      hid[r][c] = hval;
+    }
+  }
+  if constexpr (PS) {
+    if (two) {
+      ps_stamp(ps, 4);
+      constexpr int EPH = MR * HD / NT, CHK = EPH <= 16 ? EPH : EPH / 2;
+      static_assert(EPH % CHK == 0, "sweep chunks");
+      float hv[EPH];
+      {
+        const Buf16 hgb(ps.mlp_hid);
+        unsigned sweeps = 0;
+        bool bad = false;
+#pragma unroll
+        for (int c0 = 0; c0 < EPH; c0 += CHK) {
+          Gran g[CHK];
+          bool rd[CHK];
+#pragma unroll
+          for (int i = 0; i < CHK; i++) { g[i] = Gran{0u, 0.f}; rd[i] = ((deadm >> ((tid + NT * (c0 + i)) / HD)) & 1) != 0; }
+          while (!bad) {
+#pragma unroll
+            for (int i = 0; i < CHK; i++)
+              if (!rd[i] && g[i].tag != ps.tag_out) g[i] = ld_gran(hgb, (uint32_t)(tid + NT * (c0 + i)), 0u);
+            bool ok = true;
+#pragma unroll
+            for (int i = 0; i < CHK; i++) ok &= rd[i] || g[i].tag == ps.tag_out;
+            if (ok) break;
+            if (ps_sweep_retry(sweeps, ps)) { *ps.lds_flag = 0; bad = true; }
+          }
+#pragma unroll
+          for (int i = 0; i < CHK; i++) hv[c0 + i] = rd[i] ? 0.f : g[i].v;
+        }
+      }
+      using ML = MlpLds<MR, DPL, REC>;
+      static_assert(offsetof(ML, hid) == offsetof(ML, red) + sizeof(ML::red) && offsetof(ML, obuf) == offsetof(ML, hid) + sizeof(ML::hid) &&
+                    sizeof(ML::red) + sizeof(ML::hid) + sizeof(ML::obuf) >= sizeof(float) * MR * HD, "hidden rows in red .. obuf");
+      float* hall = &red[0][0][0];
+      __syncthreads();
+#pragma unroll
+      for (int i = 0; i < EPH; i++) hall[tid + NT * i] = hv[i];
+      __syncthreads();
+      if (!ps_sweeps_ok(ps)) return false;
+      float o2[MR][4];
+#pragma unroll
+      for (int r = 0; r < MR; r++) { o2[r][0] = o2[r][1] = o2[r][2] = o2[r][3] = 0.f; }
+#pragma unroll
+      for (int r = 0; r < MR; r++) {
+        if ((deadm >> r) & 1) continue;
+#pragma unroll
+        for (int i4 = 0; i4 < RPG; i4 += 4) {
+          const float4 h4 = *reinterpret_cast<const float4*>(&hall[r * HD + ch2 * RPG + i4]);
+          const float hq[4] = {h4.x, h4.y, h4.z, h4.w};
+#pragma unroll
+          for (int i = 0; i < 4; i++) {
+            const float hvv = hq[i];
+            o2[r][0] += hvv * w2[i4 + i].x; o2[r][1] += hvv * w2[i4 + i].y; o2[r][2] += hvv * w2[i4 + i].z; o2[r][3] += hvv * w2[i4 + i].w;
+          }
+        }
+      }
+      float* pbuf = &hs[0][0];
+      const bool g0 = (tid >> 2) < NCH && ((tid >> 2) % G) == 0;
+      const int jsl = (tid >> 2) / G;
+#pragma unroll
+      for (int r = 0; r < MR; r++) {
+        if ((deadm >> r) & 1) continue;
+        float s4[4] = {o2[r][0], o2[r][1], o2[r][2], o2[r][3]};
+#pragma unroll
+        for (int g2 = 1; g2 < G; g2++)
+#pragma unroll
+          for (int k = 0; k < 4; k++) s4[k] += lane_get(o2[r][k], (lane + 4 * g2) & 63);
+        if (g0) *reinterpret_cast<float4*>(&pbuf[(r * NB2 + jsl) * CB + cq * 4]) = make_float4(s4[0], s4[1], s4[2], s4[3]);
+      }
+      __syncthreads();
+      if (tid < MR * CB) {
+        const int r = tid >> 4, c = tid & (CB - 1);
+        if (r < n_rows && !((deadm >> r) & 1)) {
+          float accp = b2v;
+#pragma unroll
+          for (int j = 0; j < NB2; j++) accp += pbuf[(r * NB2 + j) * CB + c];
+          st_gran(Buf16(a.g_x_out), (uint32_t)(r * d + jblk * CB + c), ps.tag_out, xown + accp);
+        }
+      }
+      ps_stamp(ps, 5);
+      return true;
+    }
   }
   __syncthreads();
   WB_STAMP(3);
+  if constexpr (PS) ps_stamp(ps, 4);
   float o[MR][4];
 #pragma unroll
   for (int r = 0; r < MR; r++) { o[r][0] = o[r][1] = o[r][2] = o[r][3] = 0.f; }
@@ -638,6 +750,7 @@
       }
     }
   }
+  if constexpr (PS) ps_stamp(ps, 5);
   WB_STAMP(4);
   WB_STAMP_FLUSH(a, 5);
   return true;
@@ -752,7 +865,7 @@
       const Buf16 xgb(a.g_x_in), pgb(a.g_pend);
       const uint32_t pvo = (uint32_t)(r * d + c);
       const int iplane = a.S * d;
-      if (a.KSp > 0) ps_nap<2>();
+      if (a.KSp > 0 || ps.x_late) ps_nap<2>();
       constexpr int FP = 4 * DPL;
       float accp = a.KSp > 0 ? gld(a.pbias + c) : 0.f;
       unsigned sweeps = 0;
@@ -1168,7 +1281,9 @@
       const Buf16 xgb(a.g_x_in), pgb(a.g_pend);
       const uint32_t pvo = (uint32_t)(r * d + c);
       const int iplane = a.S * d;
-      if (ps.cross_early) ps_nap<WB_PS_CROSS0_NAP>(); else ps_nap<4>();
+      if (ps.cross_early) ps_nap<WB_PS_CROSS0_NAP>();
+      else if (ps.x_late) { ps_nap<2>(); __builtin_amdgcn_s_sleep(32); }
+      else ps_nap<4>();
       constexpr int FP = 8;
       float v = 0.f, accp = gld(a.pbias + c);
       unsigned sweeps = 0;
diff --git a/whisper-burn_amd/csrc/decode_persist.hip b/whisper-burn_amd/csrc/decode_persist.hip
--- a/whisper-burn_amd/csrc/decode_persist.hip
+++ b/whisper-burn_amd/csrc/decode_persist.hip
@@ -70,6 +70,7 @@
 template <int MR, int DPL>
 struct LogitsLds {
   alignas(16) float xs[MR][64 * DPL];
+  alignas(16) float xn[MR][64 * DPL];
   alignas(16) float red[8][MR][PS_CT];
   float tilev[MR][PS_CT];
 };
@@ -85,6 +86,10 @@
   auto& xs = sm.xs; auto& red = sm.red; auto& tilev = sm.tilev;
   const int tid = role_tid<true>(), lane = tid & 63, wave = tid >> 6;
   const int hh = lane >> 5, c4 = (lane & 31) * 4;
+  const bool own_ln = a.mlp2 != 0;
+  const int ln_col = 2 * wave * NR + (lane < 2 * NR ? lane : 0);
+  float g_own = 0.f, b_own = 0.f;
+  if (own_ln) { g_own = gld(a.ln_g + ln_col); b_own = gld(a.ln_b + ln_col); }
   const Buf16 etb(a.Et);
   auto load_tile = [&](float4 (&w)[NR], int tile) {
     const int n0 = tile * CT;
@@ -114,7 +119,7 @@
 #pragma unroll
     for (int r = 0; r < MR; r++)
       if (r >= ps.n_rows || ld_i<true>(ps.dead + min(r, ps.n_rows - 1)) != 0) deadm |= 1 << r;
-    const Buf16 xgb(a.g_xn);
+    const Buf16 xgb(own_ln ? a.x_fin : a.g_xn);
     float v[EPT];
     unsigned sweeps = 0;
     for (;;) {
@@ -142,6 +147,20 @@
   if (!ps_sweeps_ok(ps)) return false;
   ps_stamp(ps, 3);
   if (forced) return true;
+  const float (*xg)[d] = xs;
+#if !defined(WB_PS_DRY)
+  if (own_ln) {
+#pragma unroll
+    for (int r = 0; r < MR; r++) {
+      if ((deadm >> r) & 1) continue;
+      float mean, denom;
+      ln_stats_lds<DPL>(xs[r], d, lane, a.ln_eps, a.ln_inside, mean, denom);
+      if (lane < 2 * NR) sm.xn[r][ln_col] = (xs[r][ln_col] - mean) / denom * g_own + b_own;
+    }
+    __builtin_amdgcn_wave_barrier();
+    xg = sm.xn;
+  }
+#endif
 #if defined(WB_PS_DRY)
   for (int t = 0; t < n_t; t++)
     if (wave < MR && !((deadm >> wave) & 1)) {
@@ -166,7 +185,7 @@
       if ((deadm >> r) & 1) continue;
 #pragma unroll
       for (int i4 = 0; i4 < NR; i4 += 4) {
-        const float4 xv = *reinterpret_cast<const float4*>(&xs[r][(2 * wave + hh) * NR + i4]);
+        const float4 xv = *reinterpret_cast<const float4*>(&xg[r][(2 * wave + hh) * NR + i4]);
         acc[r][0] += xv.x * w[i4].x; acc[r][1] += xv.x * w[i4].y; acc[r][2] += xv.x * w[i4].z; acc[r][3] += xv.x * w[i4].w;
         acc[r][0] += xv.y * w[i4 + 1].x; acc[r][1] += xv.y * w[i4 + 1].y; acc[r][2] += xv.y * w[i4 + 1].z; acc[r][3] += xv.y * w[i4 + 1].w;
         acc[r][0] += xv.z * w[i4 + 2].x; acc[r][1] += xv.z * w[i4 + 2].y; acc[r][2] += xv.z * w[i4 + 2].z; acc[r][3] += xv.z * w[i4 + 2].w;
@@ -350,7 +369,8 @@
       const unsigned tag_l = a.tag_base + 2u + 3u * (unsigned)(e * NL + (role.kind <= PSR_MLP ? role.layer : NL - 1));
       const bool pick_e = a.pick != 0 && e >= 1 && e - 1 >= a.n_forced && ps.step < a.Lmax;
       if (role.kind == PSR_ATTN) {
-        const AttnFusedArgs la = a.layers[role.layer].attn;
+        AttnFusedArgs la = a.layers[role.layer].attn;
+        if (a.mlp2) { la.KSp = 0; ps.x_late = role.layer > 0; }
         if (role.layer == 0) { ps.ctr_index = C_X + role.b; ps.target = (unsigned)e; }
         else { ps.ctr_index = C_CROSS + role.layer - 1; ps.target = (unsigned)(e + 1) * H * R; }
         ps.ctr = cptr(ps.ctr_index);
@@ -371,6 +391,7 @@
         ps.ctr = cptr(ps.ctr_index);
         ps.tag_out = tag_l + 1u; ps.tag_in = tag_l;
         ps.cross_early = role.layer == 0 && pick_e;
+        ps.x_late = a.mlp2 != 0 && role.layer > 0;
         ok = dec_cross_body<DPL, true, NP, RS>(la, role.a, role.b, ps, lds.cross, i == res_i ? res_buf : nullptr);
         out = C_CROSS + role.layer;
       } else if (role.kind == PSR_MLP) {
@@ -378,6 +399,10 @@
         ps.ctr_index = C_ATTN + role.layer * S; ps.target = (unsigned)(e + 1) * H; ps.n_ctr = R;
         ps.ctr = cptr(ps.ctr_index);
         ps.tag_out = tag_l + 2u; ps.tag_in = tag_l + 1u;
+        if (a.mlp2) {
+          ps.mlp_hid = a.g_hid;
+          ps.mlp_b2 = a.layers[role.layer].mlp_b2;
+        }
         ok = dec_mlp_body<MR, DPL, false, true>(la, role.a, ps, lds.mlp);
         out = C_MLP + role.layer;
       } else if (role.kind == PSR_FINLN) {
@@ -425,6 +450,43 @@
   if (threadIdx.x == 0) *out_id = ps_sweeps_ok(ps) ? tok : -1;
 }
 
+template <int DPL>
+__global__ __launch_bounds__(PS_NT) void ps_mlp2_test_kernel(PsMlp2TestArgs t) {
+  __shared__ MlpLds<4, DPL, false> sm;
+  __shared__ int flag;
+  PsStep ps;
+  ps.ctl = t.ctl; ps.step = -1; ps.lds_flag = &flag;
+  ps.ctr = reinterpret_cast<const unsigned*>(t.ctl + HX_HDR); ps.target = 0u;
+  ps.n_rows = t.n_rows; ps.dead = t.dead;
+  ps.tag_in = t.tag_in; ps.tag_out = t.tag_in + 1u;
+  ps.mlp_hid = t.g_hid; ps.mlp_b2 = t.b2;
+  dec_mlp_body<4, DPL, false, true>(t.a, blockIdx.x, ps, sm);
+}
+
+template <int DPL>
+struct PsLogitsTestLds { union { FinLnLds<DPL> finln; LogitsLds<4, DPL> logits; }; };
+struct PsLogitsTestArgs { PersistArgs a; unsigned tag; int n_t; };
+template <int DPL>
+__global__ __launch_bounds__(PS_NT) void ps_logits_test_kernel(PsLogitsTestArgs t) {
+  const PersistArgs& a = t.a;
+  const unsigned tag = t.tag;
+  const int n_t = t.n_t;
+  __shared__ PsLogitsTestLds<DPL> sm;
+  __shared__ int flag;
+  PsStep ps;
+  ps.ctl = a.ctl; ps.step = -1; ps.lds_flag = &flag;
+  ps.ctr = reinterpret_cast<const unsigned*>(a.ctl + HX_HDR); ps.target = 0u;
+  ps.n_rows = a.n_rows; ps.dead = a.dead;
+  ps.tag_in = tag; ps.tag_out = tag;
+  if (blockIdx.x == 0) {
+    if (a.mlp2 == 0)
+      for (int r = 0; r < a.n_rows; r++)
+        if (!ps_finln_role<DPL>(a, r, ps, sm.finln)) return;
+    return;
+  }
+  ps_logits_role<4, DPL>(a, 0, n_t, ps, false, 0, sm.logits);
+}
+
 template <int DPL, int MR, int NP>
 int max_blocks_per_cu() {
   int nb = 0;
@@ -493,6 +555,23 @@
   hipLaunchKernelGGL(ps_pick_test_kernel, dim3(1), dim3(PS_NT), 0, st, rec, n_tiles, tag, ctl, out_id);
 }
 
+int launch_ps_mlp2_test(hipStream_t st, const PsMlp2TestArgs& t) {
+  if ((t.a.d != 128 && t.a.d != 384) || t.n_rows < 1 || t.n_rows > 4 || t.n_rows > t.a.S) return -1;
+  const dim3 g(4 * t.a.d / 64), b(PS_NT);
+  hipError_t e;
+  if (t.a.d == 128) e = WB_LAUNCH_COOP((ps_mlp2_test_kernel<2>), g, b, 0, st, t);
+  else e = WB_LAUNCH_COOP((ps_mlp2_test_kernel<6>), g, b, 0, st, t);
+  return e == hipSuccess ? 0 : -1;
+}
+
+int launch_ps_logits_test(hipStream_t st, const PersistArgs& a, unsigned tag, int n_t) {
+  if ((a.d != 128 && a.d != 384) || a.n_rows < 1 || a.n_rows > 4 || a.n_rows > a.S || n_t < 1 || n_t > 2 || n_t > a.n_tiles) return -1;
+  const PsLogitsTestArgs t{a, tag, n_t};
+  const dim3 g(2), b(PS_NT);
+  const hipError_t e = a.d == 128 ? WB_LAUNCH_COOP((ps_logits_test_kernel<2>), g, b, 0, st, t) : WB_LAUNCH_COOP((ps_logits_test_kernel<6>), g, b, 0, st, t);
+  return e == hipSuccess ? 0 : -1;
+}
+
 int launch_dec_persist(hipStream_t st, const PersistArgs& a, int grid) {
   const dim3 g(grid), b(PS_NT);
   const bool big = a.n_rows > 4;
diff --git a/whisper-burn_amd/csrc/session.h b/whisper-burn_amd/csrc/session.h
--- a/whisper-burn_amd/csrc/session.h
+++ b/whisper-burn_amd/csrc/session.h
@@ -46,7 +46,7 @@
   wb::DevMem x, h, att, Pqkv, Po, Pq, P1, P2, Pa, Pc, carec, ca, logits, tstats, row_stats, mask, lp_tmp, gctl, gtok, hm;
   int sk_qkv = 0, sk_o = 0, sk_1 = 0, sk_2 = 0;
   wb::DevMem ps_layers, ps_roles, ps_ctl, ps_dead, ps_tstats, ps_stamps;
-  wb::DevMem ps_gx, ps_gpa, ps_gpc, ps_gp2, ps_gxn;
+  wb::DevMem ps_gx, ps_gpa, ps_gpc, ps_gp2, ps_gxn, ps_ghid;
   unsigned ps_launches = 0;
   int ps_grid = -1;
   std::vector<uint64_t> ps_setup_key;
diff --git a/whisper-burn_amd/csrc/switches.h b/whisper-burn_amd/csrc/switches.h
--- a/whisper-burn_amd/csrc/switches.h
+++ b/whisper-burn_amd/csrc/switches.h
@@ -46,6 +46,7 @@
   X(persist_setup, "WHISPER_HIP_PERSIST_SETUP", STR, nullptr, "persistent kernel: launch setup cached on the session (on); 0: built per call; log: on + report; 0log: both") \
   X(persist_deal, "WHISPER_HIP_PERSIST_DEAL", STR, nullptr, "persistent kernel: merge / final-LN roles kept off the first-layer attention blocks (on); legacy: the least loaded blocks; log: on + report") \
   X(persist_pick, "WHISPER_HIP_PERSIST_PICK", STR, nullptr, "persistent kernel: first-layer self-attention picks the next token from the tile records itself (on); merge: it waits for the merge role's row") \
+  X(persist_mlp, "WHISPER_HIP_PERSIST_MLP", STR, nullptr, "persistent kernel: the MLP role publishes finished residual columns and the logits roles apply the final LayerNorm (on); planes: 4 d / 64 partial planes per layer and a final-LN role") \
   X(persist_inject_fail, "WHISPER_HIP_PERSIST_INJECT_FAIL", STR, nullptr, "test hook: \"launch\" = the cooperative launch is refused")
 
 #define WB_SW_DECL(fn, name, kind, dflt, what) bool fn();
```

New measurement: 2643 x real-time, median of 6. 1.3% higher.
